# yzhang511/multi_modal_foundation_model

Hardware: AMD Instinct MI355X
Metric: pretrain samples/sec (T=100 bins/modality, d_model=256, 5+5 layers, spike+behaviour masked pretraining step) (higher is better)
Workload: dtype bf16; 1 GPU; BASELINE.json configs[1]: 1 session, ap(668 neurons)+behaviour(2), d_model=256, heads=8, mlp=512, 5 enc + 5 dec layers, T=100 (L=200 tokens), dropout 0.4/0.2, AdamW+OneCycleLR, mixed objectives; per_gpu_batch=1024, global_batch=1024, seq_len=200, parallelism=dp1

## Files before the change

include/mmfm.h:

```cpp
#ifndef MMFM_H
#define MMFM_H
#include <stdint.h>
#ifdef __cplusplus
extern "C" {
#endif

#define MMFM_VERSION 401
#define MMFM_F32 0
#define MMFM_BF16 1
#define MMFM_NULL_BIAS 1
#define MMFM_EMBED_OPTS 1
#define MMFM_MLP_GELU 0
#define MMFM_MLP_RELU 1
#define MMFM_MLP_SIGMOID 2
#define MMFM_MLP_GELU_TANH 3

typedef void* mmfm_stream;

typedef struct {
    const void* state;
    uint32_t site;
    float p;
} mmfm_dropout;

int mmfm_version(void);
const char* mmfm_last_error(void);
int mmfm_device_check(int device);
int mmfm_rng_seed(void* state, uint64_t seed, mmfm_stream stream);
int mmfm_rng_advance(void* state, mmfm_stream stream);

typedef struct {
    int dtype;
    int c_f32;
    const void* A;
    const void* B;
    void* C;
    int M, N, K;
    int lda, ldb, ldc;
    int a_kcontig, b_kcontig;
    int splits, kchunk;
    int64_t slab_stride;
    const float* bias;
    void* pre_out;
    int act;
    float act_scale;
    const void* gradmul_pre;
    mmfm_dropout drop;
    const void* residual;
    int ldr;
    float* colsum;
} mmfm_gemm_desc;
int mmfm_gemm(const mmfm_gemm_desc* d, mmfm_stream stream);
int mmfm_gemm_pair(const mmfm_gemm_desc* a, const mmfm_gemm_desc* b, mmfm_stream stream);

int mmfm_gemm_dw_tiles(int M, int N, int K);
int mmfm_reduce_slabs(float* dst, const float* src, int64_t n, int nslabs, int64_t slab_stride,
                      int accumulate, mmfm_stream stream);
typedef struct {
    float* dst;
    const float* src;
    int64_t n, slab_stride;
    int32_t nslabs, accumulate, chunk0, pad_;
} mmfm_reduce_entry;
int mmfm_reduce_slabs_multi(const mmfm_reduce_entry* table, int count, int total_chunks, mmfm_stream stream);
int64_t mmfm_colsum_workspace(int64_t R, int N);
int mmfm_colsum(int dtype, const void* x, int64_t R, int N, int ld, float* out, int accumulate,
                void* workspace, int64_t workspace_bytes, mmfm_stream stream);

int mmfm_layernorm_fwd(int dtype, const void* x, const float* gamma, const float* beta, void* y,
                       float* mean, float* rstd, int64_t R, int H, float eps,
                       int destitch_L, int destitch_T, mmfm_stream stream);
int64_t mmfm_layernorm_bwd_workspace(int64_t R, int H);
int mmfm_layernorm_bwd(int dtype, const void* dy, const void* x, const float* mean, const float* rstd,
                       const float* gamma, const void* dres, void* dx, float* dgamma, float* dbeta,
                       int accumulate, int64_t R, int H, int destitch_L, int destitch_T,
                       void* workspace, int64_t workspace_bytes, mmfm_stream stream);

int mmfm_scalenorm_fwd(int dtype, const void* x, const float* g, void* y, float* rinv, int64_t R, int H, float eps,
                       mmfm_stream stream);
int64_t mmfm_scalenorm_bwd_workspace(int64_t R, int H);
int mmfm_scalenorm_bwd(int dtype, const void* dy, const void* x, const float* rinv, const float* g, const void* dres, void* dx,
                       float* dg, int accumulate, int64_t R, int H, void* workspace, int64_t workspace_bytes,
                       mmfm_stream stream);

#define MMFM_ATTN_DIAG 1
#define MMFM_ATTN_CAUSAL 2
#define MMFM_ATTN_SEP 4
typedef struct {
    int dtype;
    int B, heads, Lq, Lk, dh;
    const void* q; const void* k; const void* v;
    int ldq, ldk, ldv;
    void* o; int ldo;
    float* lse;
    const uint8_t* keypad;
    const uint8_t* mod_id;
    int flags;
    float scale;
    mmfm_dropout drop_p, drop_o;
    const void* d_o; int lddo;
    void* dq; void* dk; void* dv;
    int lddq, lddk, lddv;
    void* keepbits;
} mmfm_attn_desc;
int mmfm_attn_fwd(const mmfm_attn_desc* d, mmfm_stream stream);
int mmfm_attn_bwd(const mmfm_attn_desc* d, mmfm_stream stream);
int64_t mmfm_attn_keepbits_bytes(int B, int heads, int Lq, int Lk);
float mmfm_attn_keep_prob(float p);

int mmfm_mask_prep(int B, int T, int M, const int64_t* const* mask_src, const int64_t* mask_stride,
                   const int64_t* attn, const int64_t* channels, uint8_t* tokmask, uint8_t* keypad,
                   uint8_t* keep0, uint8_t* mod_id, int64_t* count, mmfm_stream stream);

int mmfm_stitch_fwd(int dtype, const void* tok, const float* mod_emb_row, const float* pos_emb,
                    const int64_t* ts, const uint8_t* keep0, void* x, void* emb,
                    int B, int T, int L, int m, int H, int max_F, mmfm_stream stream);
int64_t mmfm_stitch_bwd_workspace(int dtype, int B, int T, int L, int H, int max_F);
int mmfm_stitch_bwd(int dtype, const void* dx, const void* dextra, const int64_t* ts, const uint8_t* keep0,
                    mmfm_dropout drop, void* d_tok, float* d_mod_row, float* d_pos, int acc_mod, int acc_pos,
                    int B, int T, int L, int m, int H, int max_F,
                    void* workspace, int64_t workspace_bytes, mmfm_stream stream);

int mmfm_collate_csr(int B, int max_T, int max_N, float pad_value, const uint8_t* data, const int32_t* indices,
                     const int64_t* indptr, const int64_t* indptr_off, const int64_t* nnz_off, const int32_t* T_b,
                     const int32_t* N_b, float* out, int64_t* time_mask, int64_t* space_mask, mmfm_stream stream);

#define MMFM_LOSS_KINDS 1
#define MMFM_LOSS_POISSON_LOG 0
#define MMFM_LOSS_MSE 1
#define MMFM_LOSS_POISSON_RATE 2
#define MMFM_LOSS_L1 3
#define MMFM_LOSS_SMOOTH_L1 4
#define MMFM_LOSS_HUBER 5
#define MMFM_LOSS_BCE_LOGITS 6
#define MMFM_LOSS_FULL 1
int64_t mmfm_masked_loss_workspace(int64_t R, int N);
int mmfm_masked_loss_fwd(int dtype, int kind, const void* pred, const float* target, const uint8_t* rowmask,
                         int mask_ld, int T, int64_t R, int N, float* loss_sum,
                         void* workspace, int64_t workspace_bytes, mmfm_stream stream);
int mmfm_masked_loss_kind_fwd(int dtype, int kind, float param, int flags, const void* pred, const float* target,
                              const uint8_t* rowmask, int mask_ld, int T, int64_t R, int N, float* loss_sum,
                              void* workspace, int64_t workspace_bytes, mmfm_stream stream);
int mmfm_loss_finalize(const float* loss_sum, const int64_t* count, int M, float* loss, float* inv_n,
                       mmfm_stream stream);
int mmfm_masked_loss_bwd(int dtype, int kind, const void* pred, const float* target, const uint8_t* rowmask,
                         int mask_ld, int T, int64_t R, int N, const float* grad_out, const float* inv_n,
                         void* dpred, mmfm_stream stream);
int mmfm_masked_loss_kind_bwd(int dtype, int kind, float param, int flags, const void* pred, const float* target,
                              const uint8_t* rowmask, int mask_ld, int T, int64_t R, int N, const float* grad_out,
                              const float* inv_n, void* dpred, mmfm_stream stream);

int mmfm_dropout_apply(int dtype, const void* src, void* dst, int64_t R, int N, mmfm_dropout drop,
                       mmfm_stream stream);
int mmfm_cast_f32_to_bf16(const float* src, void* dst, int64_t n, mmfm_stream stream);

int mmfm_adamw_step(float* p, const float* g, float* m, float* v, void* p_bf16, int64_t n,
                    const float* hyper, mmfm_stream stream);

int mmfm_r2_series(const float* gt, const int64_t* gt_strides, const float* pred, const int64_t* pred_strides,
                   int G, int S, int C, float* out, mmfm_stream stream);
int64_t mmfm_bits_per_spike_workspace(int64_t R, int N);
int mmfm_bits_per_spike(const float* rates, const float* spikes, int64_t R, int N, float* out,
                        void* workspace, int64_t workspace_bytes, mmfm_stream stream);
int64_t mmfm_bits_per_spike_neurons_workspace(int64_t R, int N);
int mmfm_bits_per_spike_neurons(const float* rates, const float* spikes, int64_t R, int N, float* out,
                                void* workspace, int64_t workspace_bytes, mmfm_stream stream);


typedef struct {
    const float* W;
    const float* gamma;
    const float* beta;
    const float* bias;
    void* Wp;
// ... 64 lines not shown
```

multi_modal_foundation_model_amd/_lib.py:

```python
from __future__ import annotations

import ctypes as C
import os
import re

import torch

_HERE = os.path.dirname(os.path.abspath(__file__))
LIB_PATH = os.environ.get("MMFM_LIB") or os.path.join(_HERE, "libmmfm_hip.so")
HEADER_PATH = os.path.join(os.path.dirname(_HERE), "include", "mmfm.h")

F32, BF16 = 0, 1
ATTN_DIAG, ATTN_CAUSAL, ATTN_SEP = 1, 2, 4
ACT_NONE, ACT_GELU, ACT_SOFTSIGN, ACT_GELU_GRAD, ACT_SOFTSIGN_GRAD, ACT_SOFTSIGN_GRAD_OUT = 0, 1, 2, 3, 4, 5
ACT_RELU, ACT_RELU_GRAD, ACT_SIGMOID, ACT_SIGMOID_GRAD, ACT_GELU_TANH, ACT_GELU_TANH_GRAD = 6, 7, 8, 9, 10, 11
(ACT_EMB_IDENTITY, ACT_EMB_IDENTITY_GRAD, ACT_EMB_RELU, ACT_EMB_RELU_GRAD, ACT_EMB_GELU, ACT_EMB_GELU_GRAD, ACT_EMB_SILU, ACT_EMB_SILU_GRAD,
 ACT_EMB_QUICK_GELU, ACT_EMB_QUICK_GELU_GRAD, ACT_EMB_GELU_TANH, ACT_EMB_GELU_TANH_GRAD, ACT_EMB_TANH, ACT_EMB_TANH_GRAD) = range(12, 26)
MLP_GELU, MLP_RELU, MLP_SIGMOID, MLP_GELU_TANH = 0, 1, 2, 3
LOSS_POISSON_LOG, LOSS_MSE, LOSS_POISSON_RATE, LOSS_L1, LOSS_SMOOTH_L1, LOSS_HUBER, LOSS_BCE_LOGITS = range(7)
LOSS_FULL = 1


class MmfmError(RuntimeError):
    pass


class Dropout(C.Structure):
    _fields_ = [("state", C.c_void_p), ("site", C.c_uint32), ("p", C.c_float)]


NO_DROP = Dropout(None, 0, 0.0)


class GemmDesc(C.Structure):
    _fields_ = [("dtype", C.c_int), ("c_f32", C.c_int), ("A", C.c_void_p), ("B", C.c_void_p), ("C", C.c_void_p),
                ("M", C.c_int), ("N", C.c_int), ("K", C.c_int), ("lda", C.c_int), ("ldb", C.c_int), ("ldc", C.c_int),
                ("a_kcontig", C.c_int), ("b_kcontig", C.c_int), ("splits", C.c_int), ("kchunk", C.c_int),
                ("slab_stride", C.c_int64), ("bias", C.c_void_p), ("pre_out", C.c_void_p), ("act", C.c_int),
                ("act_scale", C.c_float), ("gradmul_pre", C.c_void_p), ("drop", Dropout), ("residual", C.c_void_p),
                ("ldr", C.c_int), ("colsum", C.c_void_p)]


class AttnDesc(C.Structure):
    _fields_ = [("dtype", C.c_int), ("B", C.c_int), ("heads", C.c_int), ("Lq", C.c_int), ("Lk", C.c_int), ("dh", C.c_int),
                ("q", C.c_void_p), ("k", C.c_void_p), ("v", C.c_void_p), ("ldq", C.c_int), ("ldk", C.c_int),
                ("ldv", C.c_int), ("o", C.c_void_p), ("ldo", C.c_int), ("lse", C.c_void_p), ("keypad", C.c_void_p),
                ("mod_id", C.c_void_p), ("flags", C.c_int), ("scale", C.c_float), ("drop_p", Dropout),
                ("drop_o", Dropout), ("d_o", C.c_void_p), ("lddo", C.c_int), ("dq", C.c_void_p), ("dk", C.c_void_p),
                ("dv", C.c_void_p), ("lddq", C.c_int), ("lddk", C.c_int), ("lddv", C.c_int), ("keepbits", C.c_void_p)]


class PrepEntry(C.Structure):
    _fields_ = [("W", C.c_void_p), ("gamma", C.c_void_p), ("beta", C.c_void_p), ("bias", C.c_void_p), ("Wp", C.c_void_p),
                ("WpT", C.c_void_p), ("bp", C.c_void_p), ("N", C.c_int), ("K", C.c_int), ("tile0", C.c_int), ("scalar_gain", C.c_int),
                ("WpP", C.c_void_p), ("WpTP", C.c_void_p)]


class ReduceEntry(C.Structure):
    _fields_ = [("dst", C.c_void_p), ("src", C.c_void_p), ("n", C.c_int64), ("slab_stride", C.c_int64), ("nslabs", C.c_int32),
                ("accumulate", C.c_int32), ("chunk0", C.c_int32), ("pad_", C.c_int32)]


class RowGemmDesc(C.Structure):
    _fields_ = [("R", C.c_int64), ("K", C.c_int), ("N", C.c_int), ("x", C.c_void_p), ("ldx", C.c_int), ("w", C.c_void_p),
                ("ldw", C.c_int), ("bias", C.c_void_p), ("ln", C.c_int), ("eps", C.c_float), ("xhat", C.c_void_p),
                ("rstd", C.c_void_p), ("residual", C.c_void_p), ("ldr", C.c_int), ("y", C.c_void_p), ("ldy", C.c_int),
                ("stream_out", C.c_int), ("rotate", C.c_int), ("ln_bwd", C.c_int), ("bwd_xhat", C.c_void_p), ("bwd_rstd", C.c_void_p)]


class MlpDesc(C.Structure):
    _fields_ = [("R", C.c_int64), ("x", C.c_void_p), ("ldx", C.c_int), ("eps", C.c_float), ("w_up", C.c_void_p),
                ("b_up", C.c_void_p), ("w_down", C.c_void_p), ("b_down", C.c_void_p), ("drop", Dropout), ("y", C.c_void_p),
                ("ldy", C.c_int), ("xhat", C.c_void_p), ("rstd", C.c_void_p), ("dy", C.c_void_p), ("lddy", C.c_int),
                ("w_down_t", C.c_void_p), ("w_up_t", C.c_void_p), ("t1", C.c_void_p), ("g", C.c_void_p), ("du", C.c_void_p),
                ("dx", C.c_void_p), ("lddx", C.c_int), ("rotate", C.c_int), ("scalenorm", C.c_int),
                ("act", C.c_int), ("act_beta", C.c_float)]


_vp, _i, _i64, _f = C.c_void_p, C.c_int, C.c_int64, C.c_float
_PROTOS = {
    "mmfm_version": (C.c_int, []),
    "mmfm_last_error": (C.c_char_p, []),
    "mmfm_device_check": (C.c_int, [_i]),
    "mmfm_rng_seed": (C.c_int, [_vp, C.c_uint64, _vp]),
    "mmfm_rng_advance": (C.c_int, [_vp, _vp]),
    "mmfm_gemm": (C.c_int, [C.POINTER(GemmDesc), _vp]),
    "mmfm_gemm_pair": (C.c_int, [_vp, _vp, _vp]),
    "mmfm_gemm_dw_tiles": (C.c_int, [_i, _i, _i]),
    "mmfm_reduce_slabs": (C.c_int, [_vp, _vp, _i64, _i, _i64, _i, _vp]),
    "mmfm_reduce_slabs_multi": (C.c_int, [_vp, _i, _i, _vp]),
    "mmfm_colsum_workspace": (C.c_int64, [_i64, _i]),
    "mmfm_colsum": (C.c_int, [_i, _vp, _i64, _i, _i, _vp, _i, _vp, _i64, _vp]),
    "mmfm_layernorm_fwd": (C.c_int, [_i, _vp, _vp, _vp, _vp, _vp, _vp, _i64, _i, _f, _i, _i, _vp]),
    "mmfm_layernorm_bwd_workspace": (C.c_int64, [_i64, _i]),
    "mmfm_layernorm_bwd": (C.c_int, [_i, _vp, _vp, _vp, _vp, _vp, _vp, _vp, _vp, _vp, _i, _i64, _i, _i, _i, _vp, _i64, _vp]),
    "mmfm_scalenorm_fwd": (C.c_int, [_i, _vp, _vp, _vp, _vp, _i64, _i, _f, _vp]),
    "mmfm_scalenorm_bwd_workspace": (C.c_int64, [_i64, _i]),
    "mmfm_scalenorm_bwd": (C.c_int, [_i, _vp, _vp, _vp, _vp, _vp, _vp, _vp, _i, _i64, _i, _vp, _i64, _vp]),
    "mmfm_attn_fwd": (C.c_int, [C.POINTER(AttnDesc), _vp]),
    "mmfm_attn_bwd": (C.c_int, [C.POINTER(AttnDesc), _vp]),
    "mmfm_attn_keepbits_bytes": (C.c_int64, [_i, _i, _i, _i]),
    "mmfm_attn_keep_prob": (C.c_float, [_f]),
    "mmfm_mask_prep": (C.c_int, [_i, _i, _i, C.POINTER(_vp), C.POINTER(_i64), _vp, C.POINTER(_i64), _vp, _vp, _vp, _vp, _vp, _vp]),
    "mmfm_collate_csr": (C.c_int, [_i, _i, _i, _f, _vp, _vp, _vp, _vp, _vp, _vp, _vp, _vp, _vp, _vp, _vp]),
    "mmfm_stitch_fwd": (C.c_int, [_i, _vp, _vp, _vp, _vp, _vp, _vp, _vp, _i, _i, _i, _i, _i, _i, _vp]),
    "mmfm_stitch_bwd_workspace": (C.c_int64, [_i, _i, _i, _i, _i, _i]),
    "mmfm_stitch_bwd": (C.c_int, [_i, _vp, _vp, _vp, _vp, Dropout, _vp, _vp, _vp, _i, _i, _i, _i, _i, _i, _i, _i, _vp, _i64, _vp]),
    "mmfm_masked_loss_workspace": (C.c_int64, [_i64, _i]),
    "mmfm_masked_loss_fwd": (C.c_int, [_i, _i, _vp, _vp, _vp, _i, _i, _i64, _i, _vp, _vp, _i64, _vp]),
    "mmfm_masked_loss_kind_fwd": (C.c_int, [_i, _i, _f, _i, _vp, _vp, _vp, _i, _i, _i64, _i, _vp, _vp, _i64, _vp]),
    "mmfm_loss_finalize": (C.c_int, [_vp, _vp, _i, _vp, _vp, _vp]),
    "mmfm_masked_loss_bwd": (C.c_int, [_i, _i, _vp, _vp, _vp, _i, _i, _i64, _i, _vp, _vp, _vp, _vp]),
    "mmfm_masked_loss_kind_bwd": (C.c_int, [_i, _i, _f, _i, _vp, _vp, _vp, _i, _i, _i64, _i, _vp, _vp, _vp, _vp]),
    "mmfm_dropout_apply": (C.c_int, [_i, _vp, _vp, _i64, _i, Dropout, _vp]),
    "mmfm_cast_f32_to_bf16": (C.c_int, [_vp, _vp, _i64, _vp]),
    "mmfm_adamw_step": (C.c_int, [_vp, _vp, _vp, _vp, _vp, _i64, _vp, _vp]),
    "mmfm_prep_weights": (C.c_int, [_vp, _i, _i, _vp]),
    "mmfm_rowgemm": (C.c_int, [C.POINTER(RowGemmDesc), _vp]),
    "mmfm_mlp_fwd": (C.c_int, [C.POINTER(MlpDesc), _vp]),
    "mmfm_mlp_bwd": (C.c_int, [C.POINTER(MlpDesc), _vp]),
    "mmfm_ln_linear_grad_workspace": (C.c_int64, [_i]),
    "mmfm_ln_linear_grad": (C.c_int, [_vp, _vp, _vp, _vp, _i, _i, _vp, _vp, _vp, _vp, _i, _vp, _i64, _vp]),
    "mmfm_sn_linear_grad": (C.c_int, [_vp, _vp, _vp, _i, _i, _vp, _vp, _vp, _i, _vp, _i64, _vp]),
    "mmfm_r2_series": (C.c_int, [_vp, C.POINTER(_i64), _vp, C.POINTER(_i64), _i, _i, _i, _vp, _vp]),
    "mmfm_bits_per_spike_workspace": (C.c_int64, [_i64, _i]),
    "mmfm_bits_per_spike": (C.c_int, [_vp, _vp, _i64, _i, _vp, _vp, _i64, _vp]),
    "mmfm_bits_per_spike_neurons_workspace": (C.c_int64, [_i64, _i]),
    "mmfm_bits_per_spike_neurons": (C.c_int, [_vp, _vp, _i64, _i, _vp, _vp, _i64, _vp]),
    "mmfm_mt19937_jump": (C.c_int, [_vp, C.POINTER(C.c_int32), C.c_uint64]),
    "mmfm_mt19937_jump_reset": (C.c_int, []),
}

_lib = None


def header_symbols():
    with open(HEADER_PATH) as f:
        src = f.read()
    src = re.sub(r"/\*.*?\*/", "", src, flags=re.S)
    return sorted(set(re.findall(r"\b(mmfm_[a-z0-9_]+)\s*\(", src)))


def lib():
    global _lib
    if _lib is None:
        if not os.path.exists(LIB_PATH):
            raise ImportError(f"{LIB_PATH} is missing: the HIP extension is not built and there is no CPU "
                              "fallback.  Run `python -c 'import __graft_entry__ as g; g.build()'`.")
        l = C.CDLL(LIB_PATH)
        for name, (res, args) in _PROTOS.items():
            fn = getattr(l, name)
            fn.restype, fn.argtypes = res, args
        _lib = l
    return _lib


def check(rc, what=""):
    if rc != 0:
# ... 2 lines not shown
```

multi_modal_foundation_model_amd/csrc/common.h:

```cpp
#pragma once
#include <hip/hip_runtime.h>
#include <stdint.h>
#include <stdio.h>
#include <stdarg.h>
#include <math.h>

#include "../../include/mmfm.h"

typedef __attribute__((ext_vector_type(16))) float f32x16;
typedef __attribute__((ext_vector_type(4))) float f32x4;
typedef __attribute__((ext_vector_type(8))) short bf16x8;
typedef __bf16 bf16_t;

int mmfm_set_error(int code, const char* fmt, ...);

#define MMFM_REQUIRE(cond, ...)                      \
    do {                                             \
        if (!(cond)) return mmfm_set_error(-1, __VA_ARGS__); \
    } while (0)

#define MMFM_LAUNCH_CHECK(name)                                                         \
    do {                                                                                \
        hipError_t e__ = hipGetLastError();                                             \
        if (e__ != hipSuccess)                                                          \
            return mmfm_set_error((int)e__, "%s: launch failed: %s", name, hipGetErrorString(e__)); \
    } while (0)

int mmfm_lds_opt_in(const void* kern, size_t bytes, const char* what);

static inline int cdiv(long a, long b) { return (int)((a + b - 1) / b); }

__device__ __forceinline__ float bf2f(uint16_t v) { return __uint_as_float(((uint32_t)v) << 16); }
__device__ __forceinline__ uint16_t f2bf(float f) {
    bf16_t b = (bf16_t)f;
    return *reinterpret_cast<uint16_t*>(&b);
}

typedef __attribute__((ext_vector_type(4))) unsigned int mmfm_u32x4;
typedef __attribute__((ext_vector_type(2))) unsigned int mmfm_u32x2;
typedef __attribute__((ext_vector_type(4))) float mmfm_f32x4;
__device__ __forceinline__ void st_stream(uint4* p, uint4 v) {
    __builtin_nontemporal_store(__builtin_bit_cast(mmfm_u32x4, v), reinterpret_cast<mmfm_u32x4*>(p));
}
__device__ __forceinline__ void st_stream(uint2* p, uint2 v) {
    __builtin_nontemporal_store(__builtin_bit_cast(mmfm_u32x2, v), reinterpret_cast<mmfm_u32x2*>(p));
}
__device__ __forceinline__ void st_stream(float4* p, float4 v) {
    __builtin_nontemporal_store(__builtin_bit_cast(mmfm_f32x4, v), reinterpret_cast<mmfm_f32x4*>(p));
}

template <typename T> struct io;
template <> struct io<float> {
    static __device__ __forceinline__ float ld(const float* p) { return *p; }
    static __device__ __forceinline__ void st(float* p, float v) { *p = v; }
    static __device__ __forceinline__ float4 ld4(const float* p) { return *reinterpret_cast<const float4*>(p); }
    static __device__ __forceinline__ void st4(float* p, float4 v) { *reinterpret_cast<float4*>(p) = v; }
    static __device__ __forceinline__ void st4s(float* p, float4 v) { st_stream(reinterpret_cast<float4*>(p), v); }
};
template <> struct io<uint16_t> {
    static __device__ __forceinline__ float ld(const uint16_t* p) { return bf2f(*p); }
    static __device__ __forceinline__ void st(uint16_t* p, float v) { *p = f2bf(v); }
    static __device__ __forceinline__ float4 ld4(const uint16_t* p) {
        uint2 u = *reinterpret_cast<const uint2*>(p);
        return make_float4(__uint_as_float(u.x << 16), __uint_as_float(u.x & 0xffff0000u),
                           __uint_as_float(u.y << 16), __uint_as_float(u.y & 0xffff0000u));
    }
    static __device__ __forceinline__ void st4(uint16_t* p, float4 v) {
        uint2 u;
        u.x = (uint32_t)f2bf(v.x) | ((uint32_t)f2bf(v.y) << 16);
        u.y = (uint32_t)f2bf(v.z) | ((uint32_t)f2bf(v.w) << 16);
        *reinterpret_cast<uint2*>(p) = u;
    }
    static __device__ __forceinline__ void st4s(uint16_t* p, float4 v) {
        uint2 u;
        u.x = (uint32_t)f2bf(v.x) | ((uint32_t)f2bf(v.y) << 16);
        u.y = (uint32_t)f2bf(v.z) | ((uint32_t)f2bf(v.w) << 16);
        st_stream(reinterpret_cast<uint2*>(p), u);
    }
};

__device__ __forceinline__ uint32_t mix32(uint32_t x) {
    x ^= x >> 16; x *= 0x7feb352dU; x ^= x >> 15; x *= 0x846ca68bU; x ^= x >> 16;
    return x;
// ... 289 lines not shown
```

multi_modal_foundation_model_amd/csrc/gemm.hip:

```cpp
#include "common.h"

namespace {

constexpr int BM = 128, BN = 128, BK = 32;
constexpr int LDT = 132;
constexpr int NTHREADS = 256;

template <bool KC>
__device__ __forceinline__ void g2r(float4 (&r)[4], const float* __restrict__ base, int ld, int row0, int k0,
                                    int rows, int kend, bool vec, int t) {
    if (KC) {
        const int kq = t & 7, r0 = t >> 3;
        const int k = k0 + 4 * kq;
#pragma unroll
        for (int p = 0; p < 4; ++p) {
            const int row = row0 + r0 + 32 * p;
            float4 v = make_float4(0.f, 0.f, 0.f, 0.f);
            if (row < rows && k < kend) {
                const float* src = base + (size_t)row * ld + k;
                if (vec && k + 3 < kend) {
                    v = *reinterpret_cast<const float4*>(src);
                } else {
                    v.x = src[0];
                    if (k + 1 < kend) v.y = src[1];
// ... 218 lines not shown
    }
}

template <typename T>
__global__ __launch_bounds__(256) void colsum_kernel(const T* __restrict__ x, int64_t R, int N, int ld, float* __restrict__ part,
                                                     int64_t rows_per) {
    __shared__ float red[4][64];
    const int c = blockIdx.x * 64 + (threadIdx.x & 63), rl = threadIdx.x >> 6;
    const int64_t r0 = (int64_t)blockIdx.y * rows_per, r1 = min(R, r0 + rows_per);
    float s = 0.f;
    if (c < N)
        for (int64_t r = r0 + rl; r < r1; r += 4) s += io<T>::ld(x + (size_t)r * ld + c);
    red[rl][threadIdx.x & 63] = s;
    __syncthreads();
    if (rl == 0 && c < N)
        part[(size_t)blockIdx.y * N + c] = red[0][threadIdx.x] + red[1][threadIdx.x] + red[2][threadIdx.x] + red[3][threadIdx.x];
}

template <typename T>
__global__ __launch_bounds__(256) void colsum4_kernel(const T* __restrict__ x, int64_t R, int N, int ld, float* __restrict__ part,
                                                      int64_t rows_per) {
    __shared__ float4 red[4][64];
    const int lane = threadIdx.x & 63, wave = threadIdx.x >> 6;
    const int c = blockIdx.x * 256 + lane * 4;
    const int64_t r0 = (int64_t)blockIdx.y * rows_per, r1 = min(R, r0 + rows_per);
    float4 s = make_float4(0.f, 0.f, 0.f, 0.f);
    if (c < N) {
        int64_t r = r0 + wave;
        for (; r + 12 < r1; r += 16) {
            const float4 a = io<T>::ld4(x + (size_t)r * ld + c), b = io<T>::ld4(x + (size_t)(r + 4) * ld + c);
            const float4 e = io<T>::ld4(x + (size_t)(r + 8) * ld + c), f = io<T>::ld4(x + (size_t)(r + 12) * ld + c);
            s.x += (a.x + b.x) + (e.x + f.x); s.y += (a.y + b.y) + (e.y + f.y);
            s.z += (a.z + b.z) + (e.z + f.z); s.w += (a.w + b.w) + (e.w + f.w);
        }
        for (; r < r1; r += 4) {
            const float4 a = io<T>::ld4(x + (size_t)r * ld + c);
            s.x += a.x; s.y += a.y; s.z += a.z; s.w += a.w;
        }
    }
    red[wave][lane] = s;
    __syncthreads();
    if (wave == 0 && c < N) {
        float4 o;
        o.x = red[0][lane].x + red[1][lane].x + red[2][lane].x + red[3][lane].x;
        o.y = red[0][lane].y + red[1][lane].y + red[2][lane].y + red[3][lane].y;
        o.z = red[0][lane].z + red[1][lane].z + red[2][lane].z + red[3][lane].z;
        o.w = red[0][lane].w + red[1][lane].w + red[2][lane].w + red[3][lane].w;
        *reinterpret_cast<float4*>(part + (size_t)blockIdx.y * N + c) = o;
    }
}

}

int mmfm_gemm_bf16_launch(const mmfm_gemm_desc* d, hipStream_t st);

static int gemm_check(const mmfm_gemm_desc* dp, mmfm_gemm_desc& d) {
    MMFM_REQUIRE(dp != nullptr, "mmfm_gemm: null descriptor");
    d = *dp;
    MMFM_REQUIRE(d.dtype == MMFM_F32 || d.dtype == MMFM_BF16, "mmfm_gemm: bad dtype %d", d.dtype);
    MMFM_REQUIRE(d.M > 0 && d.N > 0 && d.K > 0, "mmfm_gemm: bad shape M=%d N=%d K=%d", d.M, d.N, d.K);
    MMFM_REQUIRE(d.A && d.B && d.C, "mmfm_gemm: null operand");
    MMFM_REQUIRE(d.lda >= (d.a_kcontig ? d.K : d.M), "mmfm_gemm: lda %d too small", d.lda);
    MMFM_REQUIRE(d.ldb >= (d.b_kcontig ? d.K : d.N), "mmfm_gemm: ldb %d too small", d.ldb);
    MMFM_REQUIRE(d.ldc >= d.N, "mmfm_gemm: ldc %d < N %d", d.ldc, d.N);
    MMFM_REQUIRE(!(d.a_kcontig == 0 && d.b_kcontig == 1), "mmfm_gemm: layout (A row-contig, B k-contig) is not built");
    MMFM_REQUIRE(d.act >= 0 && d.act <= kActEmbedLast, "mmfm_gemm: bad act %d", d.act);
    const bool grad_act = (d.act >= 3 && d.act <= 5) || (d.act >= 7 && (d.act & 1));
    MMFM_REQUIRE(!d.gradmul_pre || grad_act,
                 "mmfm_gemm: gradmul_pre needs a gradient act (3 gelu', 4 softsign', 5 softsign' from the output, 7 relu', 9 sigmoid-gate', 11 tanh-gelu', "
                 "the embedder's 13 identity', 15 relu', 17 gelu', 19 silu', 21 quick_gelu', 23 tanh-gelu', 25 tanh')");
    MMFM_REQUIRE(d.gradmul_pre || !grad_act || d.act == kActEmbedIdentityGrad, "mmfm_gemm: act %d needs gradmul_pre", d.act);
    if (d.splits <= 1) {
        d.splits = 1;
        d.kchunk = d.K;
    } else {
        MMFM_REQUIRE(d.kchunk > 0 && d.kchunk % 64 == 0, "mmfm_gemm: kchunk %d must be a positive multiple of 64", d.kchunk);
        MMFM_REQUIRE((int64_t)d.splits * d.kchunk >= d.K, "mmfm_gemm: splits*kchunk < K");
        MMFM_REQUIRE(d.slab_stride >= (int64_t)d.M * d.ldc, "mmfm_gemm: slab_stride too small");
        MMFM_REQUIRE(!d.bias && !d.pre_out && !d.act && !d.residual && d.drop.p <= 0.f,
                     "mmfm_gemm: split-K writes raw partials, no epilogue");
    }
    MMFM_REQUIRE(!d.residual || d.ldr >= d.N, "mmfm_gemm: ldr too small");
    MMFM_REQUIRE(!d.colsum || (d.dtype == MMFM_BF16 && d.a_kcontig == 0), "mmfm_gemm: colsum needs dtype bf16 and a_kcontig == 0");
    return 0;
}

int mmfm_gemm_dw_pair_launch(const mmfm_gemm_desc* a, const mmfm_gemm_desc* b, hipStream_t st);

extern "C" int mmfm_gemm(const mmfm_gemm_desc* dp, mmfm_stream stream) {
    mmfm_gemm_desc d;
    if (int rc = gemm_check(dp, d)) return rc;
    hipStream_t st = (hipStream_t)stream;
    if (d.dtype == MMFM_BF16) return mmfm_gemm_bf16_launch(&d, st);

    const int tiles = cdiv(d.M, BM) * cdiv(d.N, BN);
    const int vecA = (d.lda % 4 == 0) && ((uintptr_t)d.A % 16 == 0);
    const int vecB = (d.ldb % 4 == 0) && ((uintptr_t)d.B % 16 == 0);
    dim3 grid(tiles, d.splits), block(NTHREADS);
#define F32_LAUNCH(AKV)                                                                                            \
    if (d.a_kcontig && d.b_kcontig) hipLaunchKernelGGL((gemm_f32_kernel<true, true, AKV>), grid, block, 0, st, d, vecA, vecB);        \
    else if (d.a_kcontig && !d.b_kcontig) hipLaunchKernelGGL((gemm_f32_kernel<true, false, AKV>), grid, block, 0, st, d, vecA, vecB); \
    else hipLaunchKernelGGL((gemm_f32_kernel<false, false, AKV>), grid, block, 0, st, d, vecA, vecB);
    switch (gemm_act_kind(d.act)) {
    case MMFM_MLP_RELU: { F32_LAUNCH(MMFM_MLP_RELU) } break;
    case MMFM_MLP_SIGMOID: { F32_LAUNCH(MMFM_MLP_SIGMOID) } break;
    case MMFM_MLP_GELU_TANH: { F32_LAUNCH(MMFM_MLP_GELU_TANH) } break;
    case kActEmbed: { F32_LAUNCH(kActEmbed) } break;
    default: { F32_LAUNCH(0) }
    }
#undef F32_LAUNCH
    MMFM_LAUNCH_CHECK("mmfm_gemm(f32)");
    return 0;
}

extern "C" int mmfm_gemm_pair(const mmfm_gemm_desc* ap, const mmfm_gemm_desc* bp, mmfm_stream stream) {
    mmfm_gemm_desc a, b;
    if (int rc = gemm_check(ap, a)) return rc;
    if (int rc = gemm_check(bp, b)) return rc;
    hipStream_t st = (hipStream_t)stream;
    if (a.dtype == MMFM_BF16 && b.dtype == MMFM_BF16) {
        const int rc = mmfm_gemm_dw_pair_launch(&a, &b, st);
        if (rc != -1000) return rc;
    }
    if (int rc = mmfm_gemm(ap, stream)) return rc;
    return mmfm_gemm(bp, stream);
}

__global__ __launch_bounds__(256) void reduce_slabs_multi_kernel(const mmfm_reduce_entry* __restrict__ tab, int count) {
    int lo = 0, hi = count - 1;
    const int b = blockIdx.x;
    while (lo < hi) {
        const int mid = (lo + hi + 1) >> 1;
        if (tab[mid].chunk0 <= b) lo = mid; else hi = mid - 1;
    }
    const mmfm_reduce_entry e = tab[lo];
    const int64_t i = (int64_t)(b - e.chunk0) * 256 + threadIdx.x;
    if (i >= e.n) return;
    float s = e.accumulate ? e.dst[i] : 0.f;
    for (int k = 0; k < e.nslabs; ++k) s += e.src[(size_t)k * e.slab_stride + i];
    e.dst[i] = s;
}

extern "C" int mmfm_reduce_slabs_multi(const mmfm_reduce_entry* table, int count, int total_chunks, mmfm_stream stream) {
    MMFM_REQUIRE(table && count > 0 && total_chunks > 0, "mmfm_reduce_slabs_multi: bad arguments");
    hipLaunchKernelGGL(reduce_slabs_multi_kernel, dim3(total_chunks), dim3(256), 0, (hipStream_t)stream, table, count);
    MMFM_LAUNCH_CHECK("mmfm_reduce_slabs_multi");
    return 0;
}

extern "C" int mmfm_reduce_slabs(float* dst, const float* src_c, int64_t n, int nslabs, int64_t slab_stride,
                                 int accumulate, mmfm_stream stream) {
    MMFM_REQUIRE(dst && src_c && n > 0 && nslabs > 0 && slab_stride >= n, "mmfm_reduce_slabs: bad arguments");
    float* src = const_cast<float*>(src_c);
    hipStream_t st = (hipStream_t)stream;
    const bool vec = (n % 4 == 0) && (slab_stride % 4 == 0) && ((uintptr_t)dst % 16 == 0) && ((uintptr_t)src % 16 == 0);
    if (!vec) {
        const int blocks = (int)std::min<int64_t>(2048, (n + 255) / 256);
        hipLaunchKernelGGL(reduce_slabs_kernel, dim3(blocks), dim3(256), 0, st, dst, src, n, nslabs, slab_stride, accumulate);
        MMFM_LAUNCH_CHECK("mmfm_reduce_slabs");
        return 0;
    }
    const int chunks = (int)((n + 255) / 256);
    int group = nslabs;
    if (nslabs >= 16 && chunks < 512) {
        const int want = std::min(nslabs / 4, std::max(1, 512 / chunks));
// ... 46 lines not shown
```

multi_modal_foundation_model_amd/csrc/gemm_bf16.hip:

```cpp
#include "common.h"
#include <stdlib.h>
#include <algorithm>

namespace {

constexpr int BM = 128, BN = 128;
constexpr int NTHREADS = 256;
template <int BK> struct Geo {
    static constexpr int KC_LD = BK + 8;
    static constexpr int TILE_BYTES = 128 * KC_LD * 2;
    static constexpr int NP = BK / 16;
};

typedef __attribute__((ext_vector_type(8))) __bf16 bf16x8v;
typedef __attribute__((ext_vector_type(4))) short s16x4;
typedef __attribute__((address_space(3))) s16x4 lds_s16x4;

__device__ __forceinline__ uint4 load8(const uint16_t* __restrict__ src, int nvalid, int align) {
    uint4 v = make_uint4(0u, 0u, 0u, 0u);
    if (nvalid >= 8 && align == 8) return *reinterpret_cast<const uint4*>(src);
    if (nvalid >= 8 && align == 4) {
        const uint2 a = *reinterpret_cast<const uint2*>(src), b = *reinterpret_cast<const uint2*>(src + 4);
        return make_uint4(a.x, a.y, b.x, b.y);
    }
// ... 16 lines not shown
        for (int p = 0; p < NP; ++p) {
            const int row = row0 + r0 + RPP * p;
            r[p] = (row < rows) ? load8(base + (size_t)row * ld + k, kend - k, align) : make_uint4(0u, 0u, 0u, 0u);
        }
    } else {
        const int cq = t & 15, kk0 = t >> 4, col = row0 + 8 * cq;
#pragma unroll
        for (int p = 0; p < NP; ++p) {
            const int k = k0 + kk0 + 16 * p;
            r[p] = (k < kend) ? load8(base + (size_t)k * ld + col, rows - col, align) : make_uint4(0u, 0u, 0u, 0u);
        }
    }
}

template <bool RC, int BK>
__device__ __forceinline__ void r2s(char* __restrict__ S, const uint4 (&r)[BK / 16], int t) {
    constexpr int NP = BK / 16, LPR = BK / 8, RPP = 256 / LPR, KC_LD = Geo<BK>::KC_LD;
    if (!RC) {
        const int kq = t % LPR, r0 = t / LPR;
#pragma unroll
        for (int p = 0; p < NP; ++p) *reinterpret_cast<uint4*>(S + (r0 + RPP * p) * (KC_LD * 2) + kq * 16) = r[p];
    } else {
        const int cq = t & 15, kk0 = t >> 4;
#pragma unroll
        for (int p = 0; p < NP; ++p) {
            const int kk = kk0 + 16 * p;
            *reinterpret_cast<uint4*>(S + kk * 256 + ((cq * 16) ^ ((kk & 3) << 6))) = r[p];
        }
    }
}

template <bool RC, int BK>
__device__ __forceinline__ bf16x8v frag(const char* __restrict__ S, int rowbase, int ks, int lane) {
    if (!RC) {
        const int r = lane & 31, h = lane >> 5;
        const uint4 v = *reinterpret_cast<const uint4*>(S + (rowbase + r) * (Geo<BK>::KC_LD * 2) + ks * 32 + h * 16);
        return __builtin_bit_cast(bf16x8v, v);
    } else {
        const int g = lane >> 4, li = lane & 15, q = li >> 2, p = li & 3;
        const int col = rowbase + 16 * (g & 1) + 4 * p;
        const int kb = ks * 16 + 8 * (g >> 1);
        const int off0 = (kb + q) * 256 + ((col * 2) ^ (q << 6));
        const int off1 = (kb + 4 + q) * 256 + ((col * 2) ^ (q << 6));
        const s16x4 lo = __builtin_amdgcn_ds_read_tr16_b64_v4i16((lds_s16x4*)(S + off0));
        const s16x4 hi = __builtin_amdgcn_ds_read_tr16_b64_v4i16((lds_s16x4*)(S + off1));
        typedef __attribute__((ext_vector_type(8))) short s16x8;
        s16x8 v;
        v[0] = lo[0]; v[1] = lo[1]; v[2] = lo[2]; v[3] = lo[3]; v[4] = hi[0]; v[5] = hi[1]; v[6] = hi[2]; v[7] = hi[3];
        return __builtin_bit_cast(bf16x8v, v);
    }
}

template <typename TO, int AK = 0, int EF = 0>
__device__ __forceinline__ void epilogue_store(const mmfm_gemm_desc& d, const Drop& dr, float v, int m, int n) {
    typedef io<uint16_t> I16;
    constexpr int AKM = AK == kActEmbed ? 0 : AK;
    if (d.bias) v += d.bias[n];
    if (d.pre_out) I16::st(reinterpret_cast<uint16_t*>(d.pre_out) + (size_t)m * d.ldc + n, v);
    if constexpr (AK == kActEmbed) {
        if (!(d.act & 1)) v = embed_act1<true, EF>(v) * d.act_scale;
        else if (EF == 0) v *= d.act_scale;
        else v = embed_mul_grad1<true, EF>(v, I16::ld(reinterpret_cast<const uint16_t*>(d.gradmul_pre) + (size_t)m * d.ldc + n)) * d.act_scale;
        v = dr.apply(v, (uint64_t)m * (uint64_t)d.N + (uint64_t)n);
        if (d.residual) v += I16::ld(reinterpret_cast<const uint16_t*>(d.residual) + (size_t)m * d.ldr + n);
        io<TO>::st(reinterpret_cast<TO*>(d.C) + (size_t)m * d.ldc + n, v);
        return;
    }
    if (d.act == 1) v = gelu_poly(v);
    else if (d.act == 2) v = softsign_f(v) * d.act_scale;
    else if (AK && !(d.act & 1)) v = mlp_act1<AKM>(v, d.act_scale);
    if (d.gradmul_pre) {
        const float u = I16::ld(reinterpret_cast<const uint16_t*>(d.gradmul_pre) + (size_t)m * d.ldc + n);
        if (AK == MMFM_MLP_RELU) v = u > 0.f ? v : 0.f;
        else if (AK) v *= mlp_act_grad1<AKM>(u, d.act_scale);
        else v *= (d.act == 3) ? gelu_poly_grad(u) : (d.act == 4 ? softsign_grad(u) : softsign_grad_from_out(u, 1.f / d.act_scale)) * d.act_scale;
    }
    v = dr.apply(v, (uint64_t)m * (uint64_t)d.N + (uint64_t)n);
    if (d.residual) v += I16::ld(reinterpret_cast<const uint16_t*>(d.residual) + (size_t)m * d.ldr + n);
    io<TO>::st(reinterpret_cast<TO*>(d.C) + (size_t)m * d.ldc + n, v);
}

typedef __attribute__((ext_vector_type(8))) __bf16 bf16x8e;
__device__ __forceinline__ bf16x8e pack8f(const float* v) {
    bf16x8e o;
#pragma unroll
    for (int e = 0; e < 8; ++e) o[e] = (__bf16)v[e];
    return o;
}
__device__ __forceinline__ void unpack8(uint4 w, float* u) {
    u[0] = __uint_as_float(w.x << 16); u[1] = __uint_as_float(w.x & 0xffff0000u);
    u[2] = __uint_as_float(w.y << 16); u[3] = __uint_as_float(w.y & 0xffff0000u);
    u[4] = __uint_as_float(w.z << 16); u[5] = __uint_as_float(w.z & 0xffff0000u);
    u[6] = __uint_as_float(w.w << 16); u[7] = __uint_as_float(w.w & 0xffff0000u);
}

__device__ __forceinline__ int xcd_remap(int bid, int nwg) {
    const int q = nwg >> 3, r = nwg & 7, x = bid & 7;
    return (x < r ? x * (q + 1) : r * (q + 1) + (x - r) * q) + (bid >> 3);
}

__device__ __forceinline__ uint4 ldg8(const uint16_t* p, bool a16, bool hi, bool nt) {
    if (a16 && nt) return __builtin_bit_cast(uint4, __builtin_nontemporal_load(reinterpret_cast<const mmfm_u32x4*>(p)));
    if (a16) return *reinterpret_cast<const uint4*>(p);
    const uint2 a = *reinterpret_cast<const uint2*>(p);
    const uint2 b = hi ? *reinterpret_cast<const uint2*>(p + 4) : make_uint2(0u, 0u);
    return make_uint4(a.x, a.y, b.x, b.y);
}
__device__ __forceinline__ void stg8(uint16_t* p, uint4 v, bool a16, bool hi, bool nt) {
    if (nt) {
        if (a16) { st_stream(reinterpret_cast<uint4*>(p), v); return; }
        st_stream(reinterpret_cast<uint2*>(p), make_uint2(v.x, v.y));
        if (hi) st_stream(reinterpret_cast<uint2*>(p + 4), make_uint2(v.z, v.w));
        return;
    }
    if (a16) { *reinterpret_cast<uint4*>(p) = v; return; }
    *reinterpret_cast<uint2*>(p) = make_uint2(v.x, v.y);
    if (hi) *reinterpret_cast<uint2*>(p + 4) = make_uint2(v.z, v.w);
}

template <typename TO, bool EPI_LOADS = true, int AK = 0, int EF = 0>
__device__ __forceinline__ void epilogue_tile(const mmfm_gemm_desc& d, f32x16 (&acc)[2][2], char* smem, int m0, int n0, int z, int vec_epi,
                                              int t, int wm, int wn, int kh, int l31) {
    const bool split = d.splits > 1;
    constexpr int AKM = AK == kActEmbed ? 0 : AK;
    float* Cf = reinterpret_cast<float*>(d.C) + (split ? (size_t)z * d.slab_stride : 0);
    const Drop dr = drop_init(d.drop);
    if (vec_epi & 1) {
        float* stage = reinterpret_cast<float*>(smem);
        constexpr int SLDW = 132;
        constexpr bool BF_OUT = sizeof(TO) == 2;
        const bool bf_path = BF_OUT && !split;
        const bool a16 = !(vec_epi & 2);
        const int col = (t & 15) * 8, n = n0 + col;
        const bool n_ok = n < d.N, hi = n + 8 <= d.N;
        float bs[8];
#pragma unroll
        for (int e = 0; e < 8; ++e) bs[e] = 0.f;
        if (d.bias && n_ok && !split) {
            const float4 b0 = *reinterpret_cast<const float4*>(d.bias + n);
            const float4 b1 = hi ? *reinterpret_cast<const float4*>(d.bias + n + 4) : make_float4(0.f, 0.f, 0.f, 0.f);
            bs[0] = b0.x; bs[1] = b0.y; bs[2] = b0.z; bs[3] = b0.w; bs[4] = b1.x; bs[5] = b1.y; bs[6] = b1.z; bs[7] = b1.w;
        }
#pragma unroll 1
        for (int half = 0; half < 2; ++half) {
            uint4 gu[4], gr[4];
            if (EPI_LOADS && bf_path) {
#pragma unroll
                for (int c = 0; c < 4; ++c) {
                    const int m = m0 + half * 64 + ((t + 256 * c) >> 4);
                    gu[c] = gr[c] = make_uint4(0u, 0u, 0u, 0u);
                    if (m < d.M && n_ok) {
                        if (d.gradmul_pre) gu[c] = ldg8(reinterpret_cast<const uint16_t*>(d.gradmul_pre) + (size_t)m * d.ldc + n, a16, hi, (vec_epi & 32768) != 0);
                        if (d.residual) gr[c] = ldg8(reinterpret_cast<const uint16_t*>(d.residual) + (size_t)m * d.ldr + n, a16, hi, (vec_epi & 32768) != 0);
                    }
                }
            }
            __syncthreads();
            if (wm == half) {
#pragma unroll
                for (int i = 0; i < 2; ++i)
#pragma unroll
                    for (int j = 0; j < 2; ++j)
#pragma unroll
                        for (int r = 0; r < 16; ++r)
                            stage[(i * 32 + (r & 3) + 8 * (r >> 2) + 4 * kh) * SLDW + wn * 64 + j * 32 + l31] = acc[i][j][r];
            }
            __syncthreads();
#pragma unroll
            for (int c = 0; c < 4; ++c) {
                const int row = (t + 256 * c) >> 4;
                const int m = m0 + half * 64 + row;
                if (m >= d.M || !n_ok) continue;
                float v[8];
                const float4 s0 = *reinterpret_cast<const float4*>(stage + row * SLDW + col);
                const float4 s1 = *reinterpret_cast<const float4*>(stage + row * SLDW + col + 4);
                v[0] = s0.x; v[1] = s0.y; v[2] = s0.z; v[3] = s0.w; v[4] = s1.x; v[5] = s1.y; v[6] = s1.z; v[7] = s1.w;
                const size_t off = (size_t)m * d.ldc + n;
#pragma unroll
                for (int e = 0; e < 8; ++e) v[e] += bs[e];
                if (split || !BF_OUT) {
                    float* dst = (split ? Cf : reinterpret_cast<float*>(d.C)) + off;
                    if (vec_epi & 16384) {
                        st_stream(reinterpret_cast<float4*>(dst), make_float4(v[0], v[1], v[2], v[3]));
                        if (hi) st_stream(reinterpret_cast<float4*>(dst + 4), make_float4(v[4], v[5], v[6], v[7]));
                    } else {
                        *reinterpret_cast<float4*>(dst) = make_float4(v[0], v[1], v[2], v[3]);
                        if (hi) *reinterpret_cast<float4*>(dst + 4) = make_float4(v[4], v[5], v[6], v[7]);
                    }
                    continue;
                }
                if (d.pre_out) stg8(reinterpret_cast<uint16_t*>(d.pre_out) + off, __builtin_bit_cast(uint4, pack8f(v)), a16, hi, (vec_epi & 8192) != 0);
                if constexpr (AK == kActEmbed) {
                    if (!(d.act & 1)) embed_act_n<8, EF>(v, d.act_scale);
                    else {
                        float u[8];
                        unpack8(gu[c], u);
                        embed_mul_grad_n<8, EF>(v, u, d.act_scale);
                    }
                } else if (d.act == 1) gelu_n<8>(v);
                else if (d.act == 2) {
#pragma unroll
                    for (int e = 0; e < 8; ++e) v[e] = softsign_f(v[e]) * d.act_scale;
                } else if (AK && !(d.act & 1)) mlp_act_n<AK, 8>(v, d.act_scale);
                if (AK != kActEmbed && EPI_LOADS && d.gradmul_pre) {
                    float u[8];
                    unpack8(gu[c], u);
                    if (d.act == 3) mul_gelu_grad_n<8>(v, u);
                    else if (d.act == 4) {
#pragma unroll
                        for (int e = 0; e < 8; ++e) v[e] *= softsign_grad(u[e]) * d.act_scale;
                    } else if (AK) mul_mlp_act_grad_n<AKM, 8>(v, u, d.act_scale);
                    else {
                        const float inv_s = 1.f / d.act_scale;
#pragma unroll
                        for (int e = 0; e < 8; ++e) v[e] *= softsign_grad_from_out(u[e], inv_s) * d.act_scale;
                    }
                }
                if (dr.on()) {
                    const uint64_t base = (uint64_t)m * (uint64_t)d.N + (uint64_t)n;
#pragma unroll
                    for (int e = 0; e < 8; e += 2) dr.apply2(v[e], v[e + 1], base + e);
                }
                if (EPI_LOADS && d.residual) {
                    float u[8];
                    unpack8(gr[c], u);
#pragma unroll
                    for (int e = 0; e < 8; ++e) v[e] += u[e];
                }
                stg8(reinterpret_cast<uint16_t*>(d.C) + off, __builtin_bit_cast(uint4, pack8f(v)), a16, hi, (vec_epi & 4096) != 0);
            }
        }
        return;
    }
    if (split) {
#pragma unroll
        for (int i = 0; i < 2; ++i)
#pragma unroll
            for (int j = 0; j < 2; ++j)
#pragma unroll
                for (int r = 0; r < 16; ++r) {
                    const int m = m0 + wm * 64 + i * 32 + (r & 3) + 8 * (r >> 2) + 4 * kh;
                    const int n = n0 + wn * 64 + j * 32 + l31;
                    if (m < d.M && n < d.N) Cf[(size_t)m * d.ldc + n] = acc[i][j][r];
                }
        return;
    }
#pragma unroll
    for (int i = 0; i < 2; ++i)
#pragma unroll
        for (int j = 0; j < 2; ++j)
#pragma unroll
            for (int r = 0; r < 16; ++r) {
                const int m = m0 + wm * 64 + i * 32 + (r & 3) + 8 * (r >> 2) + 4 * kh;
                const int n = n0 + wn * 64 + j * 32 + l31;
                if (m < d.M && n < d.N) epilogue_store<TO, AK, EF>(d, dr, acc[i][j][r], m, n);
            }
}

template <bool ARC, bool BRC, typename TO, int BK, bool PERSIST = (sizeof(TO) == 4), int AK = 0>
__global__ __launch_bounds__(NTHREADS, BK == 64 ? 3 : 2) void gemm_bf16_kernel(const mmfm_gemm_desc d, const int alignA, const int alignB,
                                                                              const int vec_epi, const int total_items) {
    constexpr int TILE_BYTES = Geo<BK>::TILE_BYTES;
    __shared__ __attribute__((aligned(16))) char smem[2 * TILE_BYTES];
    char* As = smem;
    char* Bs = smem + TILE_BYTES;
    const int t = threadIdx.x, lane = t & 63, wave = t >> 6;
    const int wm = wave >> 1, wn = wave & 1, kh = lane >> 5, l31 = lane & 31;
    const int tiles_n = (d.N + BN - 1) / BN;
    const int tiles = ((d.M + BM - 1) / BM) * tiles_n;
    const uint16_t* A = reinterpret_cast<const uint16_t*>(d.A);
    const uint16_t* B = reinterpret_cast<const uint16_t*>(d.B);

    auto decode = [&](int w, int& m0, int& n0, int& z, int& kbeg, int& kend) {
        const int item = xcd_remap(w, total_items);
        z = item / tiles;
        const int tile = item - z * tiles;
        m0 = (tile / tiles_n) * BM;
        n0 = (tile % tiles_n) * BN;
        kbeg = z * d.kchunk;
        kend = min(d.K, kbeg + d.kchunk);
    };

    int m0, n0, z, kbeg, kend;
    int w = blockIdx.x;
    if (w >= total_items) return;
    decode(w, m0, n0, z, kbeg, kend);
    uint4 ra[BK / 16], rb[BK / 16];
    g2r<ARC, BK>(ra, A, d.lda, m0, kbeg, d.M, kend, alignA, t);
    g2r<BRC, BK>(rb, B, d.ldb, n0, kbeg, d.N, kend, alignB, t);
    for (;;) {
        f32x16 acc[2][2];
#pragma unroll
        for (int i = 0; i < 2; ++i)
#pragma unroll
            for (int j = 0; j < 2; ++j)
#pragma unroll
                for (int r = 0; r < 16; ++r) acc[i][j][r] = 0.f;
        const bool do_cs = ARC && d.colsum != nullptr && n0 == 0;
        float cs[8];
#pragma unroll
        for (int j = 0; j < 8; ++j) cs[j] = 0.f;
        const int wn_ = w + gridDim.x;
        const bool more = PERSIST && wn_ < total_items;
        int m0n = 0, n0n = 0, zn = 0, kbegn = 0, kendn = 0;
        if (more) decode(wn_, m0n, n0n, zn, kbegn, kendn);
        for (int k0 = kbeg; k0 < kend; k0 += BK) {
            __syncthreads();
            r2s<ARC, BK>(As, ra, t);
            r2s<BRC, BK>(Bs, rb, t);
            __syncthreads();
            {
                if (k0 + BK < kend) {
                    g2r<ARC, BK>(ra, A, d.lda, m0, k0 + BK, d.M, kend, alignA, t);
                    g2r<BRC, BK>(rb, B, d.ldb, n0, k0 + BK, d.N, kend, alignB, t);
                } else if (more) {
                    g2r<ARC, BK>(ra, A, d.lda, m0n, kbegn, d.M, kendn, alignA, t);
                    g2r<BRC, BK>(rb, B, d.ldb, n0n, kbegn, d.N, kendn, alignB, t);
                }
            }
            if (ARC && do_cs) {
                const int cq = t & 15, kk0 = t >> 4;
#pragma unroll
                for (int p = 0; p < BK / 16; ++p) {
                    const int kk = kk0 + 16 * p;
                    float u[8];
                    unpack8(*reinterpret_cast<const uint4*>(As + kk * 256 + ((cq * 16) ^ ((kk & 3) << 6))), u);
#pragma unroll
                    for (int j = 0; j < 8; ++j) cs[j] += u[j];
                }
            }
#pragma unroll
            for (int ks = 0; ks < BK / 16; ++ks) {
                const bf16x8v a0 = frag<ARC, BK>(As, wm * 64, ks, lane), a1 = frag<ARC, BK>(As, wm * 64 + 32, ks, lane);
                const bf16x8v b0 = frag<BRC, BK>(Bs, wn * 64, ks, lane), b1 = frag<BRC, BK>(Bs, wn * 64 + 32, ks, lane);
                acc[0][0] = __builtin_amdgcn_mfma_f32_32x32x16_bf16(a0, b0, acc[0][0], 0, 0, 0);
                acc[0][1] = __builtin_amdgcn_mfma_f32_32x32x16_bf16(a0, b1, acc[0][1], 0, 0, 0);
                acc[1][0] = __builtin_amdgcn_mfma_f32_32x32x16_bf16(a1, b0, acc[1][0], 0, 0, 0);
                acc[1][1] = __builtin_amdgcn_mfma_f32_32x32x16_bf16(a1, b1, acc[1][1], 0, 0, 0);
            }
        }
        if (ARC && do_cs) {
            __syncthreads();
            float* red = reinterpret_cast<float*>(smem);
            float* mine = red + (t >> 4) * 128 + (t & 15) * 8;
            *reinterpret_cast<float4*>(mine) = make_float4(cs[0], cs[1], cs[2], cs[3]);
            *reinterpret_cast<float4*>(mine + 4) = make_float4(cs[4], cs[5], cs[6], cs[7]);
            __syncthreads();
            if (t < 128 && m0 + t < d.M) {
                float sum = 0.f;
#pragma unroll
                for (int i = 0; i < 16; ++i) sum += red[i * 128 + t];
                d.colsum[(d.splits > 1 ? (size_t)z * d.slab_stride : 0) + m0 + t] = sum;
            }
        }
        if constexpr (AK == kActEmbed)
            embed_dispatch(d.act, [&](auto F) {
                epilogue_tile<TO, !(PERSIST && sizeof(TO) == 2), AK, decltype(F)::value>(d, acc, smem, m0, n0, z, vec_epi, t, wm, wn, kh, l31);
            });
        else
            epilogue_tile<TO, !(PERSIST && sizeof(TO) == 2), AK>(d, acc, smem, m0, n0, z, vec_epi, t, wm, wn, kh, l31);
        if (!more) break;
        w = wn_; m0 = m0n; n0 = n0n; z = zn; kbeg = kbegn; kend = kendn;
    }
}

int align_of(const void* p, int ld) {
    if (ld % 8 == 0 && (uintptr_t)p % 16 == 0) return 8;
    if (ld % 4 == 0 && (uintptr_t)p % 8 == 0) return 4;
    return 1;
}

}

int mmfm_gemm_big_launch(const mmfm_gemm_desc* dp, hipStream_t st);
int mmfm_gemm_dw_launch(const mmfm_gemm_desc* dp, hipStream_t st);

int mmfm_gemm_bf16_launch(const mmfm_gemm_desc* dp, hipStream_t st) {
    const mmfm_gemm_desc d = *dp;
    {
        const int rb = mmfm_gemm_big_launch(dp, st);
        if (rb != -1000) return rb;
        const int rw = mmfm_gemm_dw_launch(dp, st);
        if (rw != -1000) return rw;
    }
    MMFM_REQUIRE(d.splits == 1 || d.kchunk % 64 == 0, "mmfm_gemm(bf16): kchunk %d must be a multiple of 64", d.kchunk);
    static const int bk_env = [] { const char* e = getenv("MMFM_GEMM_BK"); return e ? atoi(e) : 0; }();
    const int kspan = d.splits > 1 ? d.kchunk : d.K;
    (void)kspan;
    const int BKsel = bk_env == 128 ? 128 : 64;
    const int tiles = cdiv(d.M, BM) * cdiv(d.N, BN);
    const int aA = align_of(d.A, d.lda), aB = align_of(d.B, d.ldb);
    const int total_items = tiles * d.splits;
    static const int wg_per_cu = [] { const char* e = getenv("MMFM_GEMM_WG_PER_CU"); const int v = e ? atoi(e) : 3; return v > 0 ? v : 3; }();
    const bool f32out = d.c_f32 || d.splits > 1;
    auto al16 = [](const void* p) { return p == nullptr || (uintptr_t)p % 16 == 0; };
    const int vec8 = (d.N % 8 == 0) && (d.ldc % 8 == 0) && al16(d.C) && al16(d.pre_out) && al16(d.gradmul_pre) && al16(d.bias) &&
                     (!d.residual || (d.ldr % 8 == 0 && al16(d.residual))) && (!d.splits || d.splits == 1 || d.slab_stride % 4 == 0);
    auto al8 = [](const void* p) { return p == nullptr || (uintptr_t)p % 8 == 0; };
    const bool f32c = d.c_f32 || d.splits > 1;
    const int vec4 = (d.N % 4 == 0) && (d.ldc % 4 == 0) && (f32c ? al16(d.C) : al8(d.C)) && al8(d.pre_out) && al8(d.gradmul_pre) && al16(d.bias) &&
                     (!d.residual || (d.ldr % 4 == 0 && al8(d.residual))) && (!d.splits || d.splits == 1 || d.slab_stride % 4 == 0);
    const int vec = vec8 ? 1 : (vec4 ? 3 : 0);
    static const int nt_env = [] { const char* e = getenv("MMFM_GEMM_NT"); return e ? atoi(e) : 3; }();
    const int vecf = vec | ((nt_env & 1) ? 4096 : 0) | ((nt_env & 2) ? 8192 : 0) | ((nt_env & 4) ? 16384 : 0) | ((nt_env & 8) ? 32768 : 0);
    static const int persist_bf16 = [] { const char* e = getenv("MMFM_GEMM_PERSIST_BF16"); return e ? atoi(e) : 1; }();
    const int ak = gemm_act_kind(d.act);
    const bool pb = !f32out && !ak && persist_bf16 && !d.gradmul_pre && !d.residual && !d.pre_out && (vec & 1) && d.K <= 768;
    dim3 grid((f32out || pb) ? std::min(total_items, 256 * wg_per_cu) : total_items), block(NTHREADS);
    static const int pad_lds = [] { const char* e = getenv("MMFM_GEMM_PAD_LDS"); return e ? atoi(e) : 0; }();
#define LAUNCH2(ARC, BRC, BKV)                                                                                    \
    if (f32out) hipLaunchKernelGGL((gemm_bf16_kernel<ARC, BRC, float, BKV>), grid, block, pad_lds, st, d, aA, aB, vecf, total_items);  \
    else if (pb) hipLaunchKernelGGL((gemm_bf16_kernel<ARC, BRC, uint16_t, BKV, true>), grid, block, pad_lds, st, d, aA, aB, vecf, total_items); \
    else hipLaunchKernelGGL((gemm_bf16_kernel<ARC, BRC, uint16_t, BKV>), grid, block, pad_lds, st, d, aA, aB, vecf, total_items);
#define LAUNCH_AK(ARC, BRC, AKV)                                                                                  \
    if (f32out) hipLaunchKernelGGL((gemm_bf16_kernel<ARC, BRC, float, 64, true, AKV>), grid, block, pad_lds, st, d, aA, aB, vecf, total_items); \
    else hipLaunchKernelGGL((gemm_bf16_kernel<ARC, BRC, uint16_t, 64, false, AKV>), grid, block, pad_lds, st, d, aA, aB, vecf, total_items);
#define LAUNCH(ARC, BRC)                                                                                          \
    if (ak == MMFM_MLP_RELU) { LAUNCH_AK(ARC, BRC, MMFM_MLP_RELU) }                                                \
    else if (ak == MMFM_MLP_SIGMOID) { LAUNCH_AK(ARC, BRC, MMFM_MLP_SIGMOID) }                                     \
    else if (ak == MMFM_MLP_GELU_TANH) { LAUNCH_AK(ARC, BRC, MMFM_MLP_GELU_TANH) }                                 \
    else if (ak == kActEmbed) { LAUNCH_AK(ARC, BRC, kActEmbed) }                                                   \
    else if (BKsel == 128) { LAUNCH2(ARC, BRC, 128) } else { LAUNCH2(ARC, BRC, 64) }
    if (d.a_kcontig && d.b_kcontig) { LAUNCH(false, false) }
    else if (d.a_kcontig && !d.b_kcontig) { LAUNCH(false, true) }
    else { LAUNCH(true, true) }
#undef LAUNCH
#undef LAUNCH_AK
#undef LAUNCH2
    MMFM_LAUNCH_CHECK("mmfm_gemm(bf16)");
    return 0;
}
```

multi_modal_foundation_model_amd/csrc/gemm_big.hip:

```cpp
#include "rowchain.h"
#include <stdlib.h>
#include <algorithm>

using namespace rowchain;

namespace {

typedef __attribute__((address_space(3))) void lds_void_t;
typedef __attribute__((address_space(1))) const void glb_void_t;

constexpr int TB = 256, BK = 64, NT = 512;
constexpr int TILE_B = TB * BK * 2;
constexpr int STG0 = 4 * TILE_B;
constexpr int LDS_ALL = STG0 + 8 * STG_BYTES;

__device__ __forceinline__ opnd tfrag(const char* tile, int row, int c) {
    return as_opnd(*reinterpret_cast<const uint4*>(tile + row * 128 + ((c ^ ((row >> 1) & 7)) << 4)));
}

__device__ __forceinline__ int xcd_order(int bid, int nwg) {
    const int q = nwg >> 3, r = nwg & 7, x = bid & 7;
    return (x < r ? x * (q + 1) : r * (q + 1) + (x - r) * q) + (bid >> 3);
}

struct BigArgs {
    mmfm_gemm_desc d;
    int tiles_n, ntiles, nk;
    int nt_c, nt_pre;
};

__device__ __forceinline__ void issue_ktile(char* buf, const uint16_t* const (&pa)[4], const uint16_t* const (&pb)[4], int koff, int wave) {
#pragma unroll
    for (int i = 0; i < 4; ++i)
        __builtin_amdgcn_global_load_lds((glb_void_t*)(pa[i] + koff), (lds_void_t*)(buf + (i * 512 + 64 * wave) * 16), 16, 0, 0);
#pragma unroll
    for (int i = 0; i < 4; ++i)
        __builtin_amdgcn_global_load_lds((glb_void_t*)(pb[i] + koff), (lds_void_t*)(buf + TILE_B + (i * 512 + 64 * wave) * 16), 16, 0, 0);
}

#define LDS_READ(dst, addr, off) asm volatile("ds_read_b128 %0, %1 offset:%2" : "=v"(dst) : "v"(addr), "n"(off))
#define LDS_WAIT(n) do { asm volatile("s_waitcnt lgkmcnt(" #n ")" ::: "memory"); __builtin_amdgcn_sched_barrier(0); } while (0)

template <int AK = 0>
__global__ __launch_bounds__(NT, 2) void gemm_big_kernel(const BigArgs a) {
    extern __shared__ __attribute__((aligned(16))) char smem[];
    const mmfm_gemm_desc& d = a.d;
    const int t = threadIdx.x, lane = t & 63, m = lane & 31, h = lane >> 5;
    const int wave = __builtin_amdgcn_readfirstlane(t >> 6);
    const int wnh = wave & 1, wmq = wave >> 1;
    char* stg = smem + STG0 + wave * STG_BYTES;
    const uint16_t* A = reinterpret_cast<const uint16_t*>(d.A);
    const uint16_t* B = reinterpret_cast<const uint16_t*>(d.B);
    const int nk = a.nk;
    const int my_tiles = blockIdx.x < a.ntiles ? (a.ntiles - 1 - (int)blockIdx.x) / (int)gridDim.x + 1 : 0;
    if (my_tiles == 0) return;
    const int G = my_tiles * nk;

    const int ldrow = t >> 3, ldc8 = 8 * ((t & 7) ^ ((t >> 4) & 7));
    const uint16_t* pa[4];
    const uint16_t* pb[4];
    auto set_rows = [&](int it) {
        const int tile = xcd_order((int)blockIdx.x + it * (int)gridDim.x, a.ntiles);
        const int m0 = (tile / a.tiles_n) * TB, n0 = (tile % a.tiles_n) * TB;
#pragma unroll
        for (int i = 0; i < 4; ++i) {
            pa[i] = A + (size_t)min(m0 + 64 * i + ldrow, d.M - 1) * d.lda + ldc8;
            pb[i] = B + (size_t)min(n0 + 64 * i + ldrow, d.N - 1) * d.ldb + ldc8;
        }
    };
    int ld_g = 0, ld_it = 0, ld_kt = 0;
    auto issue_next = [&]() {
        if (ld_g >= G) return false;
        if (ld_kt == 0) set_rows(ld_it);
        issue_ktile(smem + (ld_g & 1) * 2 * TILE_B, pa, pb, ld_kt * BK, wave);
        ++ld_g;
        if (++ld_kt == nk) { ld_kt = 0; ++ld_it; }
        return true;
    };
    issue_next();
    bool tail1 = issue_next();

    const Drop dr = drop_init(d.drop);
    const GBuf Cb = gbuf(d.C, (int64_t)d.M * d.ldc * 2), Pb = gbuf(d.pre_out, (int64_t)d.M * d.ldc * 2);
    const GBuf Gb = gbuf(d.gradmul_pre, (int64_t)d.M * d.ldc * 2), Rb = gbuf(d.residual, (int64_t)d.M * d.ldr * 2);

    const uint32_t lds0 = (uint32_t)(uintptr_t)(__attribute__((address_space(3))) char*)smem;
    const uint32_t sw = (uint32_t)((m >> 1) & 7);
    const uint32_t xrow = lds0 + (uint32_t)(64 * wmq + m) * 128u, wrow = lds0 + (uint32_t)(128 * wnh + m) * 128u;
    uint32_t coff[4];
#pragma unroll
    for (int ks = 0; ks < 4; ++ks) coff[ks] = (((uint32_t)(2 * ks + h)) ^ sw) << 4;

    f32x16 acc[4][2];
    int g = 0;
    for (int it = 0; it < my_tiles; ++it) {
        const int tile = xcd_order((int)blockIdx.x + it * (int)gridDim.x, a.ntiles);
        const int m0 = (tile / a.tiles_n) * TB, n0 = (tile % a.tiles_n) * TB;
#pragma unroll
// ... 83 lines not shown
                else if (d.act == 2) {
#pragma unroll
                    for (int e = 0; e < 2; ++e)
#pragma unroll
                        for (int r = 0; r < 16; ++r) {
                            const float v = acc[2 * ip + e][j][r];
                            acc[2 * ip + e][j][r] = v * __builtin_amdgcn_rcpf(1.f + fabsf(v)) * d.act_scale;
                        }
                } else if (AK && !(d.act & 1)) {
#pragma unroll
                    for (int e = 0; e < 2; ++e) {
                        float v[16];
#pragma unroll
                        for (int r = 0; r < 16; ++r) v[r] = acc[2 * ip + e][j][r];
                        mlp_act_n<AK, 16>(v, d.act_scale);
#pragma unroll
                        for (int r = 0; r < 16; ++r) acc[2 * ip + e][j][r] = v[r];
                    }
                } else if (d.gradmul_pre) {
                    const Lines L = fetch_lines(Gb, wrow0, ldcb, (uint32_t)ncol0 * 2u, lane);
                    stage_lines(stg, L, lane);
#pragma unroll
                    for (int e = 0; e < 2; ++e) {
                        const f32x16 u = unstage_tile(stg, e, m, h);
                        f32x16& v = acc[2 * ip + e][j];
                        if (AK) {
                            float uu[16], vv[16];
#pragma unroll
                            for (int r = 0; r < 16; ++r) { uu[r] = u[r]; vv[r] = v[r]; }
                            mul_mlp_act_grad_n<AK, 16>(vv, uu, d.act_scale);
#pragma unroll
                            for (int r = 0; r < 16; ++r) v[r] = vv[r];
                        } else if (d.act == 3) {
#pragma unroll
                            for (int r = 0; r < 16; r += 2) {
                                mmfm_f32x2 uu; uu.x = u[r]; uu.y = u[r + 1];
                                uu = gelu_grad2(uu);
                                v[r] *= uu.x; v[r + 1] *= uu.y;
                            }
                        } else if (d.act == 4) {
#pragma unroll
                            for (int r = 0; r < 16; ++r) {
                                const float rd = __builtin_amdgcn_rcpf(1.f + fabsf(u[r]));
                                v[r] *= rd * rd * d.act_scale;
                            }
                        } else {
                            const float inv_s = 1.f / d.act_scale;
#pragma unroll
                            for (int r = 0; r < 16; ++r) v[r] *= softsign_grad_from_out(u[r], inv_s) * d.act_scale;
                        }
                    }
                }
                if (dr.on()) {
#pragma unroll
                    for (int e = 0; e < 2; ++e)
#pragma unroll
                        for (int r = 0; r < 16; r += 2) {
                            float v0 = acc[2 * ip + e][j][r], v1 = acc[2 * ip + e][j][r + 1];
                            dr.apply2(v0, v1, (uint64_t)row * (uint64_t)d.N + (uint64_t)(ncol0 + 32 * e + 8 * (r >> 2) + 4 * h + (r & 3)));
                            acc[2 * ip + e][j][r] = v0; acc[2 * ip + e][j][r + 1] = v1;
                        }
                }
                if (d.residual) {
                    const Lines L = fetch_lines(Rb, wrow0, ldrb, (uint32_t)ncol0 * 2u, lane);
                    stage_lines(stg, L, lane);
#pragma unroll
                    for (int e = 0; e < 2; ++e) {
                        const f32x16 u = unstage_tile(stg, e, m, h);
#pragma unroll
                        for (int r = 0; r < 16; ++r) acc[2 * ip + e][j][r] += u[r];
                    }
                }
                stage_tile(stg, 0, m, h, acc[2 * ip][j]);
                stage_tile(stg, 1, m, h, acc[2 * ip + 1][j]);
                if (a.nt_c) flush_lines<true>(stg, Cb, wrow0, ldcb, (uint32_t)ncol0 * 2u, lane, nchunk);
                else flush_lines<false>(stg, Cb, wrow0, ldcb, (uint32_t)ncol0 * 2u, lane, nchunk);
            }
        }
        tail1 = false;
    }
}

}

int mmfm_gemm_big_launch(const mmfm_gemm_desc* dp, hipStream_t st) {
    const mmfm_gemm_desc& d = *dp;
    static const int on = [] { const char* e = getenv("MMFM_GEMM_BIG"); return e ? atoi(e) : 1; }();
    static const int kmin = [] { const char* e = getenv("MMFM_GEMM_BIG_KMIN"); return e ? atoi(e) : 512; }();
    if (!on || d.dtype != MMFM_BF16 || d.c_f32 || d.splits > 1 || !d.a_kcontig || !d.b_kcontig || d.colsum) return -1000;
    if (d.K % BK || d.K < kmin || d.N < 128 || d.M < 1024 || d.N % 8) return -1000;
    const char* mt = getenv("MMFM_GEMM_BIG_MIN_TILES");
    if (cdiv(d.M, TB) * cdiv(d.N, TB) < (mt ? atoi(mt) : 96)) return -1000;
    auto al16 = [](const void* p) { return p == nullptr || (uintptr_t)p % 16 == 0; };
    if (d.lda % 8 || d.ldb % 8 || d.ldc % 8 || (d.residual && d.ldr % 8) || !al16(d.A) || !al16(d.B) || !al16(d.C) || !al16(d.pre_out) ||
        !al16(d.gradmul_pre) || !al16(d.residual) || !al16(d.bias))
        return -1000;
    if ((int64_t)d.M * std::max(d.ldc, d.ldr) * 2 >= (int64_t)1 << 31) return -1000;
    const int ak = gemm_act_kind(d.act);
    const void* kern = ak == MMFM_MLP_RELU ? reinterpret_cast<const void*>(gemm_big_kernel<MMFM_MLP_RELU>)
                     : ak == MMFM_MLP_SIGMOID ? reinterpret_cast<const void*>(gemm_big_kernel<MMFM_MLP_SIGMOID>)
                     : ak == MMFM_MLP_GELU_TANH ? reinterpret_cast<const void*>(gemm_big_kernel<MMFM_MLP_GELU_TANH>)
                     : ak == kActEmbed ? reinterpret_cast<const void*>(gemm_big_kernel<kActEmbed>)
                     : reinterpret_cast<const void*>(gemm_big_kernel<0>);
    if (int rc = mmfm_lds_opt_in(kern, LDS_ALL, "mmfm_gemm(bf16, 256 tile)")) return rc;
    static const int nt_env = [] { const char* e = getenv("MMFM_GEMM_NT"); return e ? atoi(e) : 3; }();
    BigArgs a;
    a.d = d;
    a.tiles_n = cdiv(d.N, TB);
    a.ntiles = cdiv(d.M, TB) * a.tiles_n;
    a.nk = d.K / BK;
    a.nt_c = nt_env & 1;
    a.nt_pre = (nt_env >> 1) & 1;
    if (ak == MMFM_MLP_RELU) hipLaunchKernelGGL(gemm_big_kernel<MMFM_MLP_RELU>, dim3(std::min(a.ntiles, 256)), dim3(NT), LDS_ALL, st, a);
    else if (ak == MMFM_MLP_SIGMOID) hipLaunchKernelGGL(gemm_big_kernel<MMFM_MLP_SIGMOID>, dim3(std::min(a.ntiles, 256)), dim3(NT), LDS_ALL, st, a);
    else if (ak == MMFM_MLP_GELU_TANH) hipLaunchKernelGGL(gemm_big_kernel<MMFM_MLP_GELU_TANH>, dim3(std::min(a.ntiles, 256)), dim3(NT), LDS_ALL, st, a);
    else if (ak == kActEmbed) hipLaunchKernelGGL(gemm_big_kernel<kActEmbed>, dim3(std::min(a.ntiles, 256)), dim3(NT), LDS_ALL, st, a);
    else hipLaunchKernelGGL(gemm_big_kernel<0>, dim3(std::min(a.ntiles, 256)), dim3(NT), LDS_ALL, st, a);
    MMFM_LAUNCH_CHECK("mmfm_gemm(bf16, 256 tile)");
    return 0;
}
```

multi_modal_foundation_model_amd/csrc/gemm_dw.hip:

```cpp
#include "common.h"
#include <stdlib.h>
#include <algorithm>

namespace {

typedef __attribute__((address_space(3))) void lds_void_t;
typedef __attribute__((ext_vector_type(8))) __bf16 opnd;
typedef __attribute__((ext_vector_type(2))) unsigned int u32x2;
typedef __attribute__((ext_vector_type(4))) unsigned int u32x4;

constexpr int TM = 128, DNT = 256;
constexpr uint32_t OOB = 0x80000000u;

#ifndef MMFM_DW_LDS_KB
#define MMFM_DW_LDS_KB 160
#endif
template <int TN, int BK> struct Geo {
    static constexpr int OPA = BK * TM * 2, OPB = BK * TN * 2, STB = OPA + OPB;
    static constexpr int NST = (MMFM_DW_LDS_KB * 1024) / STB < 8 ? (MMFM_DW_LDS_KB * 1024) / STB : 8;
    static_assert(NST >= 3, "ring needs three stages");
    static constexpr int LDS = NST * STB;
    static constexpr int NA = BK / 16;
    static constexpr int NB = NA * (TN / TM);
    static constexpr int NJ = TN / 64;
};

struct DwArgs {
    mmfm_gemm_desc d;
    int tiles_n, ntiles, items;
};

__device__ __forceinline__ int xcd_order(int bid, int nwg) {
    const int q = nwg >> 3, r = nwg & 7, x = bid & 7;
    return (x < r ? x * (q + 1) : r * (q + 1) + (x - r) * q) + (bid >> 3);
}

__device__ __forceinline__ opnd mk_opnd(u32x2 lo, u32x2 hi) {
    u32x4 v;
    v[0] = lo[0]; v[1] = lo[1]; v[2] = hi[0]; v[3] = hi[1];
    return __builtin_bit_cast(opnd, v);
}

#define TR_READ(dst, addr, off) asm volatile("ds_read_b64_tr_b16 %0, %1 offset:%2" : "=v"(dst) : "v"(addr), "n"(off))
#define LDS_WAIT0 do { asm volatile("s_waitcnt lgkmcnt(0)" ::: "memory"); __builtin_amdgcn_sched_barrier(0); } while (0)
template <int N> __device__ __forceinline__ void vm_wait() { asm volatile("s_waitcnt vmcnt(%0)" :: "n"(N) : "memory"); }

struct DwPair {
    DwArgs a, b;
    int first;
};

template <int TN, int BK>
__global__ __launch_bounds__(DNT) void gemm_dw_kernel(const DwPair pr) {
    const bool second = pr.first > 0 && (int)blockIdx.x >= pr.first;
    const DwArgs& a = second ? pr.b : pr.a;
    const int w0 = second ? (int)blockIdx.x - pr.first : (int)blockIdx.x;
    const int wstep = pr.first > 0 ? (1 << 30) : (int)gridDim.x;
    typedef Geo<TN, BK> G;
    constexpr int NLW = 4;
    constexpr int NST = G::NST, NJ = G::NJ, RBB = TN * 2;
    extern __shared__ __attribute__((aligned(16))) char smem[];
    const mmfm_gemm_desc& d = a.d;
    const int t = threadIdx.x, lane = t & 63;
    const int wave = __builtin_amdgcn_readfirstlane(t >> 6);
    const int wm = wave >> 1, wn = wave & 1;
    const uint32_t ldaB = (uint32_t)d.lda * 2u, ldbB = (uint32_t)d.ldb * 2u;
    const __amdgpu_buffer_rsrc_t rsA = __builtin_amdgcn_make_buffer_rsrc(const_cast<void*>(d.A), 0, (int)((int64_t)d.K * ldaB), 0x00020000);
    const __amdgpu_buffer_rsrc_t rsB = __builtin_amdgcn_make_buffer_rsrc(const_cast<void*>(d.B), 0, (int)((int64_t)d.K * ldbB), 0x00020000);

    const int dkA = lane >> 4, dcA = (lane & 15) ^ (dkA << 2);
    constexpr int PPR = TN / 8, RPI = 64 / PPR;
    const int dkB = lane / PPR;
    const int dcB = (lane % PPR) ^ ((((RPI * wave) & 3) + dkB) << 2);
    const int g = lane >> 4, li = lane & 15, q = li >> 2, p = li & 3;
    const uint32_t lds0 = (uint32_t)(uintptr_t)(__attribute__((address_space(3))) char*)smem;
    uint32_t ra[2], rb[NJ];
#pragma unroll
    for (int i = 0; i < 2; ++i) ra[i] = lds0 + (uint32_t)((8 * (g >> 1) + q) * 256 + (((128 * wm + 64 * i) ^ (q << 6)) + 32 * (g & 1) + 8 * p));
#pragma unroll
    for (int j = 0; j < NJ; ++j)
        rb[j] = lds0 + (uint32_t)(G::OPA + (8 * (g >> 1) + q) * RBB + (((TN * wn + 64 * j) ^ (q << 6)) + 32 * (g & 1) + 8 * p));
    u32x4 ones4;
    ones4[0] = ones4[1] = ones4[2] = ones4[3] = 0x3F803F80u;
    const opnd ones = __builtin_bit_cast(opnd, ones4);

    for (int w = w0; w < a.items; w += wstep) {
        const int item = xcd_order(w, a.items);
        const int z = item / a.ntiles, tile = item - z * a.ntiles;
        const int m0 = (tile / a.tiles_n) * TM, n0 = (tile % a.tiles_n) * TN;
        const int kbeg = d.splits > 1 ? z * d.kchunk : 0;
        const int kend = d.splits > 1 ? min(d.K, kbeg + d.kchunk) : d.K;
        const int nk = (kend - kbeg + BK - 1) / BK;
        const bool do_cs = d.colsum != nullptr && n0 == 0 && wn == 0;

        const uint32_t srcA = (m0 + 8 * dcA < d.M) ? (uint32_t)dkA * ldaB + (uint32_t)(m0 + 8 * dcA) * 2u : OOB;
        const uint32_t srcB = (n0 + 8 * dcB < d.N) ? (uint32_t)dkB * ldbB + (uint32_t)(n0 + 8 * dcB) * 2u : OOB;
        auto issue = [&](int kt) {
            char* buf = smem + (kt % NST) * G::STB;
            const bool live = kt < nk;
            const uint32_t k0 = (uint32_t)(kbeg + kt * BK);
#pragma unroll
            for (int j = 0; j < G::NA; ++j) {
                const uint32_t kr = k0 + (uint32_t)(4 * (NLW * j + wave));
                const uint32_t va = live ? srcA + kr * ldaB : OOB;
                __builtin_amdgcn_raw_ptr_buffer_load_lds(rsA, (lds_void_t*)(buf + (NLW * j + wave) * 1024), 16, (int)va, 0, 0, 0);
            }
#pragma unroll
            for (int j = 0; j < G::NB; ++j) {
                const uint32_t kr = k0 + (uint32_t)(RPI * (NLW * j + wave));
                const uint32_t vb = live ? srcB + kr * ldbB : OOB;
                __builtin_amdgcn_raw_ptr_buffer_load_lds(rsB, (lds_void_t*)(buf + G::OPA + (NLW * j + wave) * 1024), 16, (int)vb, 0, 0, 0);
            }
        };
#pragma unroll
        for (int s = 0; s < NST - 1; ++s) issue(s);
// ... 46 lines not shown
            LDS_WAIT0;
            if (BK == 64) {
                READ_SET(0, 2)
                MMA_SET(1)
                LDS_WAIT0;
                READ_SET(1, 3)
                MMA_SET(0)
                LDS_WAIT0;
            }
            MMA_SET(1)
#undef READ_SET
#undef MMA_SET
        }
        asm volatile("s_waitcnt vmcnt(0)" ::: "memory");
        __builtin_amdgcn_s_barrier();

        float* Cf = reinterpret_cast<float*>(d.C) + (d.splits > 1 ? (size_t)z * d.slab_stride : 0);
        const int h = lane >> 5, l31 = lane & 31;
#pragma unroll
        for (int i = 0; i < 2; ++i)
#pragma unroll
            for (int j = 0; j < NJ; ++j) {
                const int n = n0 + (TN / 2) * wn + 32 * j + l31;
#pragma unroll
                for (int r = 0; r < 16; ++r) {
                    const int m = m0 + 64 * wm + 32 * i + (r & 3) + 8 * (r >> 2) + 4 * h;
                    if (m < d.M && n < d.N) Cf[(size_t)m * d.ldc + n] = acc[i][j][r];
                }
            }
        if (do_cs && l31 == 0) {
            float* csum = d.colsum + (d.splits > 1 ? (size_t)z * d.slab_stride : 0);
#pragma unroll
            for (int i = 0; i < 2; ++i)
#pragma unroll
                for (int r = 0; r < 16; ++r) {
                    const int m = m0 + 64 * wm + 32 * i + (r & 3) + 8 * (r >> 2) + 4 * h;
                    if (m < d.M) csum[m] = cs[i][r];
                }
        }
    }
}

template <int TN>
DwArgs make_args(const mmfm_gemm_desc& d) {
    DwArgs a;
    a.d = d;
    a.tiles_n = cdiv(d.N, TN);
    a.ntiles = cdiv(d.M, TM) * a.tiles_n;
    a.items = a.ntiles * std::max(1, d.splits);
    return a;
}

template <int TN, int BK>
int launch(const mmfm_gemm_desc& d, const mmfm_gemm_desc* d2, hipStream_t st) {
    typedef Geo<TN, BK> G;
    if (int rc = mmfm_lds_opt_in(reinterpret_cast<const void*>(gemm_dw_kernel<TN, BK>), G::LDS, "mmfm_gemm(bf16, dW stream)")) return rc;
    DwPair p;
    p.a = make_args<TN>(d);
    p.b = p.a;
    p.first = 0;
    int grid = std::min(p.a.items, 256);
    if (d2) {
        p.b = make_args<TN>(*d2);
        p.first = p.a.items;
        grid = p.a.items + p.b.items;
    }
    hipLaunchKernelGGL((gemm_dw_kernel<TN, BK>), dim3(grid), dim3(DNT), G::LDS, st, p);
    MMFM_LAUNCH_CHECK("mmfm_gemm(bf16, dW stream)");
    return 0;
}

}

static bool dw_wide(int N, int K) {
    static const int tn_env = [] { const char* e = getenv("MMFM_GEMM_DW_TN"); return e ? atoi(e) : 0; }();
    if (tn_env == 128 || N <= 128) return false;
    return tn_env == 256 || K >= 32768;
}

extern "C" int mmfm_gemm_dw_tiles(int M, int N, int K) { return cdiv(M, TM) * cdiv(N, dw_wide(N, K) ? 256 : 128); }

static bool dw_eligible(const mmfm_gemm_desc& d) {
    static const int on = [] { const char* e = getenv("MMFM_GEMM_DW"); return e ? atoi(e) : 1; }();
    const bool f32out = d.c_f32 || d.splits > 1;
    if (!on || d.dtype != MMFM_BF16 || !f32out || d.a_kcontig || d.b_kcontig) return false;
    if (d.bias || d.pre_out || d.gradmul_pre || d.residual || d.act || (d.drop.p > 0.f)) return false;
    if (d.lda % 8 || d.ldb % 8 || d.lda < (d.M + 7) / 8 * 8 || d.ldb < (d.N + 7) / 8 * 8 || ((uintptr_t)d.A & 15) || ((uintptr_t)d.B & 15) || ((uintptr_t)d.C & 3)) return false;
    if (d.splits > 1 && (d.kchunk % 64 || d.kchunk <= 0)) return false;
    if (((int64_t)d.K + 9 * 64) * std::max(d.lda, d.ldb) * 2 >= (int64_t)1 << 31) return false;
    return true;
}

int mmfm_gemm_dw_launch(const mmfm_gemm_desc* dp, hipStream_t st) {
    const mmfm_gemm_desc& d = *dp;
    if (!dw_eligible(d)) return -1000;
    return dw_wide(d.N, d.K) ? launch<256, 32>(d, nullptr, st) : launch<128, 32>(d, nullptr, st);
}

int mmfm_gemm_dw_pair_launch(const mmfm_gemm_desc* ap, const mmfm_gemm_desc* bp, hipStream_t st) {
    const mmfm_gemm_desc &a = *ap, &b = *bp;
    if (!dw_eligible(a) || !dw_eligible(b)) return -1000;
    const bool wide = dw_wide(a.N, a.K);
    if (wide != dw_wide(b.N, b.K)) return -1000;
    const int ia = mmfm_gemm_dw_tiles(a.M, a.N, a.K) * std::max(1, a.splits), ib = mmfm_gemm_dw_tiles(b.M, b.N, b.K) * std::max(1, b.splits);
    if (ia % 8 || ia + ib > 512) return -1000;
    return wide ? launch<256, 32>(a, &b, st) : launch<128, 32>(a, &b, st);
}
```

multi_modal_foundation_model_amd/csrc/stitch.hip:

```cpp
#include "common.h"
#include <algorithm>

namespace {

constexpr int MAXM = 8;
struct MaskSrc {
    const int64_t* p[MAXM];
    int64_t stride[MAXM];
    int64_t channels[MAXM];
};

__global__ void mask_prep_kernel(MaskSrc src, const int64_t* __restrict__ attn, int B, int T, int M, uint8_t* __restrict__ tokmask,
                                 uint8_t* __restrict__ keypad, uint8_t* __restrict__ keep0, uint8_t* __restrict__ mod_id,
                                 unsigned long long* __restrict__ count) {
    const int L = M * T;
    unsigned long long local[MAXM];
#pragma unroll
    for (int m = 0; m < MAXM; ++m) local[m] = 0;
    for (int64_t idx = (int64_t)blockIdx.x * blockDim.x + threadIdx.x; idx < (int64_t)B * L; idx += (int64_t)gridDim.x * blockDim.x) {
        const int b = (int)(idx / L), l = (int)(idx % L), m = l / T, t = l % T;
        const int64_t a = attn[(size_t)b * T + t];
        const int64_t v = src.p[m][((size_t)b * T + t) * src.stride[m]] & a;
        tokmask[idx] = (uint8_t)(v != 0);
        keypad[idx] = (uint8_t)(a != 0);
        if (b == 0) {
            keep0[l] = (uint8_t)(v != 1);
            mod_id[l] = (uint8_t)m;
        }
#pragma unroll
        for (int mm = 0; mm < MAXM; ++mm)
            if (mm == m) local[mm] += (unsigned long long)v * (unsigned long long)src.channels[mm];
    }
#pragma unroll
    for (int m = 0; m < MAXM; ++m) {
        if (m < M) {
            unsigned long long s = local[m];
            for (int o = 32; o > 0; o >>= 1) s += __shfl_xor(s, o);
            if ((threadIdx.x & 63) == 0 && s) atomicAdd(&count[m], s);
        }
    }
}

__global__ void zero_u64_kernel(unsigned long long* p, int n) {
    if ((int)threadIdx.x < n) p[threadIdx.x] = 0ull;
}

template <typename T>
__global__ __launch_bounds__(256) void stitch_fwd_kernel(const T* __restrict__ tok, const float* __restrict__ mod_row,
                                                         const float* __restrict__ pos, const int64_t* __restrict__ ts,
                                                         const uint8_t* __restrict__ keep0, T* __restrict__ x, T* __restrict__ emb,
                                                         int B, int Tn, int L, int m, int H, int max_F) {
    const int C4 = H / 4;
    const int64_t total = (int64_t)B * Tn * C4;
    for (int64_t idx = (int64_t)blockIdx.x * blockDim.x + threadIdx.x; idx < total; idx += (int64_t)gridDim.x * blockDim.x) {
        const int64_t r = idx / C4;
        const int c = (int)(idx % C4) * 4;
        const int b = (int)(r / Tn), t = (int)(r % Tn);
        const int l = m * Tn + t;
        const float4 mr = *reinterpret_cast<const float4*>(mod_row + c);
        float4 e = mr;
        if (pos) {
            const int tsv = (int)min((int64_t)(max_F - 1), max((int64_t)0, ts[r]));
            const float4 pr = *reinterpret_cast<const float4*>(pos + (size_t)tsv * H + c);
            e = make_float4(mr.x + pr.x, mr.y + pr.y, mr.z + pr.z, mr.w + pr.w);
        }
        const size_t o = ((size_t)b * L + l) * H + c;
        if (emb) io<T>::st4(emb + o, e);
        if (keep0[l]) {
            const float4 tv = io<T>::ld4(tok + (size_t)r * H + c);
            e.x += tv.x; e.y += tv.y; e.z += tv.z; e.w += tv.w;
        }
        io<T>::st4(x + o, e);
    }
}

template <typename T, bool POS>
__global__ void stitch_bwd_kernel(const T* __restrict__ dx, const T* __restrict__ dextra, const int64_t* __restrict__ ts,
                                  const uint8_t* __restrict__ keep0, mmfm_dropout dropa, T* __restrict__ d_tok,
                                  float* __restrict__ part, int B, int Tn, int L, int m, int H, int max_F, int bper) {
    extern __shared__ __attribute__((aligned(16))) float tab[];
    const int CW = blockDim.x, j = threadIdx.x, col = blockIdx.x * CW + j;
    const Drop dr = drop_init(dropa);
    for (int f = 0; f < max_F; ++f) tab[f * CW + j] = 0.f;
    float macc = 0.f;
    const int b0 = blockIdx.y * bper, b1 = min(B, b0 + bper);
    for (int b = b0; b < b1; ++b) {
        for (int t = 0; t < Tn; ++t) {
            const int l = m * Tn + t;
            const size_t o = ((size_t)b * L + l) * H + col;
            const float g = io<T>::ld(dx + o);
            float e = g;
            if (dextra) e += io<T>::ld(dextra + o);
            const int64_t r = (int64_t)b * Tn + t;
            if (POS) {
                const int tsv = (int)min((int64_t)(max_F - 1), max((int64_t)0, ts[r]));
                tab[tsv * CW + j] += e;
            }
            macc += e;
            if (d_tok) io<T>::st(d_tok + (size_t)r * H + col, keep0[l] ? dr.apply(g, (uint64_t)r * H + col) : 0.f);
        }
    }
    float* out = part + (size_t)blockIdx.y * (max_F + 1) * H;
    for (int f = 0; f < max_F; ++f) out[(size_t)f * H + col] = tab[f * CW + j];
    out[(size_t)max_F * H + col] = macc;
}

__global__ __launch_bounds__(256) void onehot_kernel(const int64_t* __restrict__ ts, uint16_t* __restrict__ oh, int B, int Tn, int L, int m,
                                                     int max_F, int ohc) {
    const int cpr = ohc / 8;
    const int64_t total = (int64_t)B * L * cpr;
    for (int64_t idx = (int64_t)blockIdx.x * blockDim.x + threadIdx.x; idx < total; idx += (int64_t)gridDim.x * blockDim.x) {
        const int64_t row = idx / cpr;
        const int c0 = (int)(idx % cpr) * 8;
        const int b = (int)(row / L), l = (int)(row % L), t = l - m * Tn;
        uint32_t w[4] = {0u, 0u, 0u, 0u};
        if (t >= 0 && t < Tn) {
            const int tsv = (int)min((int64_t)(max_F - 1), max((int64_t)0, ts[(int64_t)b * Tn + t]));
#pragma unroll
            for (int j = 0; j < 8; ++j)
                if (c0 + j == tsv || c0 + j == max_F) w[j >> 1] |= 0x3F80u << (16 * (j & 1));
        }
        *reinterpret_cast<uint4*>(oh + row * ohc + c0) = make_uint4(w[0], w[1], w[2], w[3]);
    }
}

__global__ __launch_bounds__(256) void stitch_modsum_kernel(const uint16_t* __restrict__ dx, const uint16_t* __restrict__ dextra,
                                                            float* __restrict__ part, int B, int Tn, int L, int m, int H, int bper) {
    __shared__ float4 red[4][64];
    const int lane = threadIdx.x & 63, rl = threadIdx.x >> 6;
    const int c = blockIdx.x * 256 + lane * 4;
    const int b0 = blockIdx.y * bper, b1 = min(B, b0 + bper);
    float4 acc = make_float4(0.f, 0.f, 0.f, 0.f);
    if (c < H) {
        for (int64_t r = (int64_t)b0 * Tn + rl; r < (int64_t)b1 * Tn; r += 4) {
            const size_t o = ((size_t)(r / Tn) * L + (size_t)m * Tn + (size_t)(r % Tn)) * H + c;
            float4 e = io<uint16_t>::ld4(dx + o);
            if (dextra) {
                const float4 x = io<uint16_t>::ld4(dextra + o);
                e.x += x.x; e.y += x.y; e.z += x.z; e.w += x.w;
            }
            acc.x += e.x; acc.y += e.y; acc.z += e.z; acc.w += e.w;
        }
    }
    red[rl][lane] = acc;
    __syncthreads();
    if (rl == 0 && c < H) {
        float4 o;
        o.x = (red[0][lane].x + red[1][lane].x) + (red[2][lane].x + red[3][lane].x);
        o.y = (red[0][lane].y + red[1][lane].y) + (red[2][lane].y + red[3][lane].y);
        o.z = (red[0][lane].z + red[1][lane].z) + (red[2][lane].z + red[3][lane].z);
        o.w = (red[0][lane].w + red[1][lane].w) + (red[2][lane].w + red[3][lane].w);
        *reinterpret_cast<float4*>(part + (size_t)blockIdx.y * H + c) = o;
    }
}

__global__ __launch_bounds__(256) void stitch_dtok_kernel(const uint16_t* __restrict__ dx, const uint8_t* __restrict__ keep0, mmfm_dropout dropa,
                                                          uint16_t* __restrict__ d_tok, int B, int Tn, int L, int m, int H) {
    const Drop dr = drop_init(dropa);
    const int C8 = H / 8;
    const int64_t total = (int64_t)B * Tn * C8;
    for (int64_t idx = (int64_t)blockIdx.x * blockDim.x + threadIdx.x; idx < total; idx += (int64_t)gridDim.x * blockDim.x) {
        const int64_t r = idx / C8;
        const int c = (int)(idx % C8) * 8;
        const int b = (int)(r / Tn), l = m * Tn + (int)(r % Tn);
        uint4 o = make_uint4(0u, 0u, 0u, 0u);
        if (keep0[l]) {
            const uint4 g = *reinterpret_cast<const uint4*>(dx + ((size_t)b * L + l) * H + c);
            if (dr.on()) {
                const uint32_t gw[4] = {g.x, g.y, g.z, g.w};
                uint32_t ow[4];
#pragma unroll
                for (int j = 0; j < 4; ++j) {
                    const float v0 = dr.apply(__uint_as_float(gw[j] << 16), (uint64_t)r * H + c + 2 * j);
                    const float v1 = dr.apply(__uint_as_float(gw[j] & 0xffff0000u), (uint64_t)r * H + c + 2 * j + 1);
                    ow[j] = (uint32_t)f2bf(v0) | ((uint32_t)f2bf(v1) << 16);
                }
                o = make_uint4(ow[0], ow[1], ow[2], ow[3]);
            } else {
                o = g;
            }
        }
        *reinterpret_cast<uint4*>(d_tok + (size_t)r * H + c) = o;
    }
}

struct CollateArgs {
    const uint8_t* data;
    const int32_t* indices;
    const int64_t* indptr;
    const int64_t* indptr_off;
    const int64_t* nnz_off;
    const int32_t* T_b;
    const int32_t* N_b;
};
__global__ __launch_bounds__(256) void collate_csr_kernel(CollateArgs a, int B, int max_T, int max_N, float pad, float* __restrict__ out,
                                                          int64_t* __restrict__ tmask, int64_t* __restrict__ smask) {
    const int lane = threadIdx.x & 63, wave = threadIdx.x >> 6;
    for (int64_t row = (int64_t)blockIdx.x * 4 + wave; row < (int64_t)B * max_T; row += (int64_t)gridDim.x * 4) {
        const int b = (int)(row / max_T), t = (int)(row % max_T);
        const int Tb = a.T_b[b], Nb = a.N_b[b];
        const bool live = t < Tb;
        const int nvalid = min(Nb, max_N);
        float* o = out + row * max_N;
        for (int n = lane; n < max_N; n += 64) o[n] = (live && n < nvalid) ? 0.f : pad;
        if (lane == 0) tmask[row] = live ? 1 : 0;
        if (t == 0)
            for (int n = lane; n < max_N; n += 64) smask[(size_t)b * max_N + n] = n < nvalid ? 1 : 0;
        if (!live) continue;
        __threadfence_block();
        __builtin_amdgcn_wave_barrier();
        const int64_t* ip = a.indptr + a.indptr_off[b];
        const int64_t z0 = ip[t], z1 = ip[t + 1], base = a.nnz_off[b];
        for (int64_t z = z0 + lane; z < z1; z += 64) {
            const int col = a.indices[base + z];
            if (col >= 0 && col < nvalid) atomicAdd(o + col, (float)a.data[base + z]);
        }
    }
}

int pick_cw(int H, int max_F) {
    for (int cw : {256, 128, 64, 32, 16, 8, 4})
        if (H % cw == 0 && (size_t)max_F * cw * 4 <= 60 * 1024) return cw;
    return 0;
}
int stitch_chunks(int B, int H, int cw) { return std::max(1, std::min(B, 512 / std::max(1, H / cw))); }
struct OhGeo { int ohc, S, kchunk; int64_t oh_bytes, slab; };
OhGeo oh_geo(int B, int L, int H, int max_F) {
    OhGeo g;
    g.ohc = (max_F + 1 + 7) & ~7;
    const int64_t K = (int64_t)B * L;
    const int tiles = ((max_F + 1 + 127) / 128) * ((H + 127) / 128);
    int S = (int)std::max<int64_t>(1, std::min<int64_t>(K / 512, (512 + tiles - 1) / tiles));
    g.kchunk = (int)(((K + S - 1) / S + 63) / 64 * 64);
    g.S = (int)((K + g.kchunk - 1) / g.kchunk);
    g.oh_bytes = ((int64_t)K * g.ohc * 2 + 255) / 256 * 256;
    g.slab = (int64_t)(max_F + 1) * H;
    return g;
}
bool oh_path(int dtype, int H) { return dtype == MMFM_BF16 && H % 8 == 0; }

}

extern "C" int mmfm_reduce_slabs(float*, const float*, int64_t, int, int64_t, int, mmfm_stream);
int mmfm_gemm_bf16_launch(const mmfm_gemm_desc* dp, hipStream_t st);

extern "C" int mmfm_mask_prep(int B, int T, int M, const int64_t* const* mask_src, const int64_t* mask_stride,
                              const int64_t* attn, const int64_t* channels, uint8_t* tokmask, uint8_t* keypad,
                              uint8_t* keep0, uint8_t* mod_id, int64_t* count, mmfm_stream stream) {
    MMFM_REQUIRE(B > 0 && T > 0 && M > 0 && M <= MAXM, "mmfm_mask_prep: bad shape B=%d T=%d M=%d (M <= %d)", B, T, M, MAXM);
    MMFM_REQUIRE(mask_src && mask_stride && attn && channels && tokmask && keypad && keep0 && mod_id && count, "mmfm_mask_prep: null pointer");
    MMFM_REQUIRE(M * T <= 65535, "mmfm_mask_prep: sequence too long");
    MaskSrc src;
    for (int m = 0; m < MAXM; ++m) {
        src.p[m] = m < M ? mask_src[m] : nullptr;
        src.stride[m] = m < M ? mask_stride[m] : 0;
        src.channels[m] = m < M ? channels[m] : 0;
        MMFM_REQUIRE(m >= M || (src.p[m] && src.stride[m] > 0), "mmfm_mask_prep: modality %d has no mask source", m);
    }
    hipStream_t st = (hipStream_t)stream;
    hipLaunchKernelGGL(zero_u64_kernel, dim3(1), dim3(64), 0, st, (unsigned long long*)count, M);
    MMFM_LAUNCH_CHECK("mmfm_mask_prep(zero)");
    const int64_t n = (int64_t)B * M * T;
    hipLaunchKernelGGL(mask_prep_kernel, dim3((int)std::min<int64_t>(256, (n + 255) / 256)), dim3(256), 0, st, src, attn, B, T, M,
                       tokmask, keypad, keep0, mod_id, (unsigned long long*)count);
    MMFM_LAUNCH_CHECK("mmfm_mask_prep");
    return 0;
}

extern "C" int mmfm_collate_csr(int B, int max_T, int max_N, float pad_value, const uint8_t* data, const int32_t* indices,
                                const int64_t* indptr, const int64_t* indptr_off, const int64_t* nnz_off, const int32_t* T_b,
                                const int32_t* N_b, float* out, int64_t* time_mask, int64_t* space_mask, mmfm_stream stream) {
    MMFM_REQUIRE(B > 0 && max_T > 0 && max_N > 0, "mmfm_collate_csr: bad shape");
    MMFM_REQUIRE(indptr && indptr_off && nnz_off && T_b && N_b && out && time_mask && space_mask, "mmfm_collate_csr: null pointer");
    CollateArgs a{data, indices, indptr, indptr_off, nnz_off, T_b, N_b};
    const int64_t rows = (int64_t)B * max_T;
    hipLaunchKernelGGL(collate_csr_kernel, dim3((int)std::min<int64_t>(4096, (rows + 3) / 4)), dim3(256), 0, (hipStream_t)stream, a, B, max_T,
                       max_N, pad_value, out, time_mask, space_mask);
    MMFM_LAUNCH_CHECK("mmfm_collate_csr");
    return 0;
}

extern "C" int mmfm_stitch_fwd(int dtype, const void* tok, const float* mod_emb_row, const float* pos_emb, const int64_t* ts,
                               const uint8_t* keep0, void* x, void* emb, int B, int T, int L, int m, int H, int max_F, mmfm_stream stream) {
    MMFM_REQUIRE(tok && mod_emb_row && (ts || !pos_emb) && keep0 && x, "mmfm_stitch_fwd: null pointer");
    MMFM_REQUIRE(B > 0 && T > 0 && H > 0 && H % 4 == 0 && m >= 0 && (m + 1) * T <= L && max_F > 0, "mmfm_stitch_fwd: bad shape");
    const int64_t n = (int64_t)B * T * (H / 4);
    dim3 grid((int)std::min<int64_t>(4096, (n + 255) / 256)), block(256);
    hipStream_t st = (hipStream_t)stream;
    if (dtype == MMFM_F32)
        hipLaunchKernelGGL(stitch_fwd_kernel<float>, grid, block, 0, st, (const float*)tok, mod_emb_row, pos_emb, ts, keep0, (float*)x, (float*)emb, B, T, L, m, H, max_F);
    else if (dtype == MMFM_BF16)
        hipLaunchKernelGGL(stitch_fwd_kernel<uint16_t>, grid, block, 0, st, (const uint16_t*)tok, mod_emb_row, pos_emb, ts, keep0, (uint16_t*)x, (uint16_t*)emb, B, T, L, m, H, max_F);
    else
        return mmfm_set_error(-1, "mmfm_stitch_fwd: bad dtype %d", dtype);
    MMFM_LAUNCH_CHECK("mmfm_stitch_fwd");
    return 0;
}

extern "C" int64_t mmfm_stitch_bwd_workspace(int dtype, int B, int T, int L, int H, int max_F) {
    (void)T;
    if (oh_path(dtype, H)) {
        const OhGeo g = oh_geo(B, L, H, max_F);
        return g.oh_bytes + 2 * (int64_t)g.S * g.slab * (int64_t)sizeof(float);
    }
    const int cw = pick_cw(H, max_F);
    if (!cw) return -1;
    return (int64_t)stitch_chunks(B, H, cw) * (max_F + 1) * H * sizeof(float);
}

extern "C" int mmfm_stitch_bwd(int dtype, const void* dx, const void* dextra, const int64_t* ts, const uint8_t* keep0,
                               mmfm_dropout drop, void* d_tok, float* d_mod_row, float* d_pos, int acc_mod, int acc_pos, int B, int T,
                               int L, int m, int H, int max_F, void* workspace, int64_t workspace_bytes, mmfm_stream stream) {
    MMFM_REQUIRE(dx && (ts || !d_pos) && keep0 && d_mod_row, "mmfm_stitch_bwd: null pointer");
    MMFM_REQUIRE(B > 0 && T > 0 && H > 0 && max_F > 0 && m >= 0 && (m + 1) * T <= L, "mmfm_stitch_bwd: bad shape");
    if (oh_path(dtype, H)) {
        const OhGeo g = oh_geo(B, L, H, max_F);
        MMFM_REQUIRE(workspace && workspace_bytes >= mmfm_stitch_bwd_workspace(dtype, B, T, L, H, max_F), "mmfm_stitch_bwd: workspace too small");
        MMFM_REQUIRE((uintptr_t)dx % 16 == 0 && (!dextra || (uintptr_t)dextra % 16 == 0) && (!d_tok || (uintptr_t)d_tok % 16 == 0) &&
                     (uintptr_t)workspace % 16 == 0, "mmfm_stitch_bwd: bf16 tensors must be 16-byte aligned");
        hipStream_t st = (hipStream_t)stream;
        if (!d_pos) {
            const int64_t room = mmfm_stitch_bwd_workspace(dtype, B, T, L, H, max_F) / ((int64_t)H * (int64_t)sizeof(float));
            const int S = (int)std::max<int64_t>(1, std::min<int64_t>(std::min<int64_t>(B, 256), room));
            const int bper = (B + S - 1) / S, nsl = (B + bper - 1) / bper;
            if (d_tok) {
                const int64_t n = (int64_t)B * T * (H / 8);
                hipLaunchKernelGGL(stitch_dtok_kernel, dim3((int)std::min<int64_t>(4096, (n + 255) / 256)), dim3(256), 0, st, (const uint16_t*)dx, keep0,
                                   drop, (uint16_t*)d_tok, B, T, L, m, H);
            }
            hipLaunchKernelGGL(stitch_modsum_kernel, dim3(cdiv(H, 256), nsl), dim3(256), 0, st, (const uint16_t*)dx, (const uint16_t*)dextra,
                               (float*)workspace, B, T, L, m, H, bper);
            MMFM_LAUNCH_CHECK("mmfm_stitch_bwd(column sum)");
            return mmfm_reduce_slabs(d_mod_row, (const float*)workspace, H, nsl, H, acc_mod, stream);
        }
        uint16_t* oh = reinterpret_cast<uint16_t*>(workspace);
        float* slabs = reinterpret_cast<float*>(reinterpret_cast<char*>(workspace) + g.oh_bytes);
        const int64_t nch = (int64_t)B * L * (g.ohc / 8);
        hipLaunchKernelGGL(onehot_kernel, dim3((int)std::min<int64_t>(4096, (nch + 255) / 256)), dim3(256), 0, st, ts, oh, B, T, L, m, max_F, g.ohc);
        if (d_tok) {
            const int64_t n = (int64_t)B * T * (H / 8);
            hipLaunchKernelGGL(stitch_dtok_kernel, dim3((int)std::min<int64_t>(4096, (n + 255) / 256)), dim3(256), 0, st, (const uint16_t*)dx, keep0,
                               drop, (uint16_t*)d_tok, B, T, L, m, H);
        }
        MMFM_LAUNCH_CHECK("mmfm_stitch_bwd(one-hot)");
        mmfm_gemm_desc gd = {};
        gd.dtype = MMFM_BF16; gd.c_f32 = 1;
        gd.A = oh; gd.lda = g.ohc; gd.a_kcontig = 0;
        gd.ldb = H; gd.b_kcontig = 0;
        gd.M = max_F + 1; gd.N = H; gd.K = B * L; gd.ldc = H;
        gd.splits = g.S; gd.kchunk = g.kchunk; gd.slab_stride = g.slab;
        gd.act_scale = 1.f;
        int nsl = 0;
        for (const void* src : {dx, dextra}) {
            if (!src) continue;
            gd.B = src;
            gd.C = slabs + (int64_t)nsl * g.slab;
            if (int rc = mmfm_gemm_bf16_launch(&gd, st)) return rc;
            nsl += g.S;
        }
        if (int rc = mmfm_reduce_slabs(d_pos, slabs, (int64_t)max_F * H, nsl, g.slab, acc_pos, stream)) return rc;
        return mmfm_reduce_slabs(d_mod_row, slabs + (int64_t)max_F * H, H, nsl, g.slab, acc_mod, stream);
    }
    const int cw = pick_cw(H, max_F);
    MMFM_REQUIRE(cw > 0, "mmfm_stitch_bwd: no column slab fits LDS for H=%d max_F=%d", H, max_F);
    const int nch = stitch_chunks(B, H, cw);
    MMFM_REQUIRE(workspace && workspace_bytes >= mmfm_stitch_bwd_workspace(dtype, B, T, L, H, max_F), "mmfm_stitch_bwd: workspace too small");
    const int bper = (B + nch - 1) / nch;
    dim3 grid(H / cw, nch), block(cw);
    const size_t lds = (size_t)max_F * cw * sizeof(float);
    hipStream_t st = (hipStream_t)stream;
    MMFM_REQUIRE(dtype == MMFM_F32 || dtype == MMFM_BF16, "mmfm_stitch_bwd: bad dtype %d", dtype);
    if (!d_pos) {
        if (dtype == MMFM_F32)
            hipLaunchKernelGGL((stitch_bwd_kernel<float, false>), grid, block, 0, st, (const float*)dx, (const float*)dextra, ts, keep0, drop,
                               (float*)d_tok, (float*)workspace, B, T, L, m, H, 0, bper);
        else
            hipLaunchKernelGGL((stitch_bwd_kernel<uint16_t, false>), grid, block, 0, st, (const uint16_t*)dx, (const uint16_t*)dextra, ts, keep0, drop,
                               (uint16_t*)d_tok, (float*)workspace, B, T, L, m, H, 0, bper);
        MMFM_LAUNCH_CHECK("mmfm_stitch_bwd(no table)");
        return mmfm_reduce_slabs(d_mod_row, (const float*)workspace, H, nch, H, acc_mod, stream);
    }
    if (dtype == MMFM_F32)
        hipLaunchKernelGGL((stitch_bwd_kernel<float, true>), grid, block, lds, st, (const float*)dx, (const float*)dextra, ts, keep0, drop, (float*)d_tok,
                           (float*)workspace, B, T, L, m, H, max_F, bper);
    else
        hipLaunchKernelGGL((stitch_bwd_kernel<uint16_t, true>), grid, block, lds, st, (const uint16_t*)dx, (const uint16_t*)dextra, ts, keep0, drop,
                           (uint16_t*)d_tok, (float*)workspace, B, T, L, m, H, max_F, bper);
    MMFM_LAUNCH_CHECK("mmfm_stitch_bwd");
    const int64_t stride = (int64_t)(max_F + 1) * H;
    if (int rc = mmfm_reduce_slabs(d_pos, (const float*)workspace, (int64_t)max_F * H, nch, stride, acc_pos, stream)) return rc;
    return mmfm_reduce_slabs(d_mod_row, (const float*)workspace + (size_t)max_F * H, H, nch, stride, acc_mod, stream);
}
```

multi_modal_foundation_model_amd/ops.py:

```python
from __future__ import annotations

import ctypes as C

import torch

from . import _lib as L


def _stream():
    return torch.cuda.current_stream().cuda_stream


def run_plan(plan, stream=None):
    st = _stream() if stream is None else stream
    for fn, args, _keep in plan:
        rc = fn(*args, st)
        if rc:
            L.check(rc, fn.__name__)


def _emit(plan, fn, args, keep=()):
    if plan is None:
        L.check(fn(*args, _stream()), fn.__name__)
    else:
        plan.append((fn, args, keep))


def P(t):
    return None if t is None else t.data_ptr()


def dt(t):
    if t.dtype == torch.float32:
        return L.F32
    if t.dtype == torch.bfloat16:
        return L.BF16
    raise TypeError(f"unsupported dtype {t.dtype}")


def dropout(state, site, p):
    if state is None or p <= 0:
        return L.NO_DROP
    return L.Dropout(state.data_ptr(), site, float(p))


def gemm_desc(A, B, Cout, M, N, K, *, lda, ldb, ldc, a_kcontig=1, b_kcontig=1, bias=None, pre_out=None, act=0,
              act_scale=1.0, gradmul_pre=None, drop=None, residual=None, ldr=0, splits=1, kchunk=0, slab_stride=0,
              dtype=None, c_f32=0, colsum=None):
    d = L.GemmDesc()
    d.dtype = dt(A) if dtype is None else dtype
    d.c_f32 = c_f32
    d.A, d.B, d.C = P(A), P(B), P(Cout)
    d.M, d.N, d.K, d.lda, d.ldb, d.ldc = M, N, K, lda, ldb, ldc
    d.a_kcontig, d.b_kcontig = a_kcontig, b_kcontig
    d.splits, d.kchunk, d.slab_stride = splits, kchunk, slab_stride
    d.bias, d.pre_out, d.act, d.act_scale, d.gradmul_pre = P(bias), P(pre_out), act, act_scale, P(gradmul_pre)
    d.drop = drop if drop is not None else L.NO_DROP
    d.residual, d.ldr = P(residual), ldr
    d.colsum = colsum if isinstance(colsum, int) else P(colsum)
    return d


def gemm(A, B, Cout, M, N, K, *, plan=None, **kw):
    d = gemm_desc(A, B, Cout, M, N, K, **kw)
    _emit(plan, L.lib().mmfm_gemm, (C.byref(d),), keep=(d,))


def gemm_pair(da, db, plan=None):
    _emit(plan, L.lib().mmfm_gemm_pair, (C.byref(da), C.byref(db)), keep=(da, db))


def reduce_slabs(dst, src, n, nslabs, stride, accumulate=False, plan=None):
    _emit(plan, L.lib().mmfm_reduce_slabs, (P(dst), P(src), n, nslabs, stride, int(accumulate)))


def reduce_slabs_multi(items, device, plan=None):
    import numpy as np
    arr = (L.ReduceEntry * len(items))()
    chunk0 = 0
    for a, (dst, src, n, nslabs, stride, acc) in zip(arr, items):
        a.dst, a.src, a.n, a.slab_stride, a.nslabs, a.accumulate, a.chunk0 = P(dst), P(src), n, stride, nslabs, int(acc), chunk0
        chunk0 += (n + 255) // 256
    table = torch.from_numpy(np.frombuffer(bytes(arr), dtype=np.uint8).copy()).to(device)
    _emit(plan, L.lib().mmfm_reduce_slabs_multi, (P(table), len(items), chunk0), keep=(table,))


def colsum(x, R, N, ld, out, ws, accumulate=False, plan=None):
    _emit(plan, L.lib().mmfm_colsum, (dt(x), P(x), R, N, ld, P(out), int(accumulate), P(ws), ws.numel() * ws.element_size()))


def layernorm_fwd(x, gamma, beta, y, mean, rstd, R, H, eps=1e-5, ds_L=0, ds_T=0, plan=None):
    _emit(plan, L.lib().mmfm_layernorm_fwd, (dt(x), P(x), P(gamma), P(beta), P(y), P(mean), P(rstd), R, H, eps, ds_L, ds_T))


def layernorm_bwd(dy, x, mean, rstd, gamma, dres, dx, dgamma, dbeta, R, H, ws, accumulate=False, ds_L=0, ds_T=0, plan=None):
    _emit(plan, L.lib().mmfm_layernorm_bwd, (dt(x), P(dy), P(x), P(mean), P(rstd), P(gamma), P(dres), P(dx), P(dgamma),
                                             P(dbeta), int(accumulate), R, H, ds_L, ds_T, P(ws), ws.numel() * ws.element_size()))


def scalenorm_fwd(x, g, y, rinv, R, H, eps=1e-5, plan=None):
    _emit(plan, L.lib().mmfm_scalenorm_fwd, (dt(x), P(x), P(g), P(y), P(rinv), R, H, eps))


def scalenorm_bwd_workspace(R, H):
    return int(L.lib().mmfm_scalenorm_bwd_workspace(R, H))


def scalenorm_bwd(dy, x, rinv, g, dres, dx, dg, R, H, ws, accumulate=False, plan=None):
    _emit(plan, L.lib().mmfm_scalenorm_bwd, (dt(x), P(dy), P(x), P(rinv), P(g), P(dres), P(dx), P(dg), int(accumulate), R, H, P(ws),
                                             ws.numel() * ws.element_size()))


def attn_desc(dtype, B, heads, Lq, Lk, dh, q, k, v, ldq, ldk, ldv, o, ldo, lse, keypad, mod_id, flags, scale,
              drop_p=None, drop_o=None, d_o=None, lddo=0, dq=None, dk=None, dv=None, lddq=0, lddk=0, lddv=0, keepbits=None):
    d = L.AttnDesc()
    d.dtype, d.B, d.heads, d.Lq, d.Lk, d.dh = dtype, B, heads, Lq, Lk, dh
    d.q, d.k, d.v, d.ldq, d.ldk, d.ldv = q, k, v, ldq, ldk, ldv
    d.o, d.ldo, d.lse, d.keypad, d.mod_id, d.flags, d.scale = o, ldo, P(lse), P(keypad), P(mod_id), flags, scale
    d.drop_p = drop_p if drop_p is not None else L.NO_DROP
    d.drop_o = drop_o if drop_o is not None else L.NO_DROP
    d.d_o, d.lddo, d.dq, d.dk, d.dv, d.lddq, d.lddk, d.lddv = d_o, lddo, dq, dk, dv, lddq, lddk, lddv
    d.keepbits = P(keepbits)
    return d


def attn_keepbits_bytes(B, heads, Lq, Lk):
    return int(L.lib().mmfm_attn_keepbits_bytes(B, heads, Lq, Lk))


def attn_keep_prob(p):
    return float(L.lib().mmfm_attn_keep_prob(float(p)))


def attn_fwd(desc, plan=None):
    _emit(plan, L.lib().mmfm_attn_fwd, (C.byref(desc),), keep=(desc,))


def attn_bwd(desc, plan=None):
    _emit(plan, L.lib().mmfm_attn_bwd, (C.byref(desc),), keep=(desc,))


def mask_prep(B, T, masks, strides, attn, channels, tokmask, keypad, keep0, mod_id, count, plan=None):
    M = len(masks)
    src = (C.c_void_p * M)(*[m.data_ptr() for m in masks])
    st = (C.c_int64 * M)(*strides)
    ch = (C.c_int64 * M)(*channels)
    _emit(plan, L.lib().mmfm_mask_prep, (B, T, M, src, st, P(attn), ch, P(tokmask), P(keypad), P(keep0), P(mod_id), P(count)),
          keep=(src, st, ch))


def stitch_fwd(tok, mod_row, pos, ts, keep0, x, emb, B, T, Lseq, m, H, max_F, plan=None):
    _emit(plan, L.lib().mmfm_stitch_fwd, (dt(tok), P(tok), P(mod_row), P(pos), P(ts), P(keep0), P(x), P(emb), B, T, Lseq, m, H, max_F))


def stitch_bwd(dx, dextra, ts, keep0, drop, d_tok, d_mod_row, d_pos, acc_mod, acc_pos, B, T, Lseq, m, H, max_F, ws, plan=None):
    _emit(plan, L.lib().mmfm_stitch_bwd, (dt(dx), P(dx), P(dextra), P(ts), P(keep0), drop if drop is not None else L.NO_DROP,
                                          P(d_tok), P(d_mod_row), P(d_pos), int(acc_mod), int(acc_pos), B, T, Lseq, m, H, max_F, P(ws),
                                          ws.numel() * ws.element_size()))


def masked_loss_fwd(kind, pred, target, rowmask, mask_ld, T, R, N, loss_sum, ws, plan=None):
    _emit(plan, L.lib().mmfm_masked_loss_fwd, (dt(pred), kind, P(pred), P(target), P(rowmask), mask_ld, T, R, N, P(loss_sum), P(ws),
                                               ws.numel() * ws.element_size()))


def masked_loss_kind_fwd(kind, param, flags, pred, target, rowmask, mask_ld, T, R, N, loss_sum, ws, plan=None):
    _emit(plan, L.lib().mmfm_masked_loss_kind_fwd, (dt(pred), kind, float(param), flags, P(pred), P(target), P(rowmask), mask_ld, T, R, N,
                                                    P(loss_sum), P(ws), ws.numel() * ws.element_size()))


def loss_finalize(loss_sum, count, M, loss, inv_n, plan=None):
    _emit(plan, L.lib().mmfm_loss_finalize, (P(loss_sum), P(count), M, P(loss), P(inv_n)))


def masked_loss_bwd(kind, pred, target, rowmask, mask_ld, T, R, N, grad_out, inv_n, dpred, plan=None):
    _emit(plan, L.lib().mmfm_masked_loss_bwd, (dt(pred), kind, P(pred), P(target), P(rowmask), mask_ld, T, R, N, P(grad_out), P(inv_n), P(dpred)))


def masked_loss_kind_bwd(kind, param, flags, pred, target, rowmask, mask_ld, T, R, N, grad_out, inv_n, dpred, plan=None):
    _emit(plan, L.lib().mmfm_masked_loss_kind_bwd, (dt(pred), kind, float(param), flags, P(pred), P(target), P(rowmask), mask_ld, T, R, N,
                                                    P(grad_out), P(inv_n), P(dpred)))


def dropout_apply(src, dst, R, N, drop, plan=None):
    _emit(plan, L.lib().mmfm_dropout_apply, (dt(src), P(src), P(dst), R, N, drop))


def cast_bf16(src, dst, n, plan=None):
    _emit(plan, L.lib().mmfm_cast_f32_to_bf16, (P(src), P(dst), n))


def adamw_step(p, g, m, v, p_bf16, n, hyper, plan=None):
    _emit(plan, L.lib().mmfm_adamw_step, (P(p), P(g), P(m), P(v), P(p_bf16), n, P(hyper)))


def rng_seed(state, seed, plan=None):
    _emit(plan, L.lib().mmfm_rng_seed, (P(state), int(seed) & (2 ** 64 - 1)))


def rng_advance(state, plan=None):
    _emit(plan, L.lib().mmfm_rng_advance, (P(state),))


def collate_csr(B, max_T, max_N, pad_value, data, indices, indptr, indptr_off, nnz_off, T_b, N_b, out, tmask, smask, plan=None):
    _emit(plan, L.lib().mmfm_collate_csr, (B, max_T, max_N, float(pad_value), P(data), P(indices), P(indptr), P(indptr_off), P(nnz_off),
# ... 125 lines not shown
```

multi_modal_foundation_model_amd/plan.py:

```python
from __future__ import annotations

import functools
import math
import os
from collections import namedtuple

import torch

from . import _lib as L
from . import ops as K


def _align(n, a=8):
    return (n + a - 1) // a * a


Switches = namedtuple("Switches", "fused gemm_big gemm_dw batch_reduce dw_pair attn_keepbits mlp_bwd_split")


def read_switches() -> Switches:
    env, on = os.environ, lambda k: os.environ.get(k, "1") != "0"
    return Switches(fused=int(env["MMFM_FUSED"]) if "MMFM_FUSED" in env else None, gemm_big=on("MMFM_GEMM_BIG"), gemm_dw=on("MMFM_GEMM_DW"),
                    batch_reduce=on("MMFM_BATCH_REDUCE"), dw_pair=on("MMFM_DW_PAIR"), attn_keepbits=on("MMFM_ATTN_KEEPBITS"),
                    mlp_bwd_split=env.get("MMFM_MLP_BWD_SPLIT", "1") == "1")


class Side:
    def __init__(self, sc, training):
        self.heads, self.I, self.act, self.scale, self.mult, self.max_F = sc.heads, sc.inter, sc.act, sc.embed_scale, sc.mult, sc.max_F
        self.dp, self.dpe = (sc.dropout, sc.embed_dropout) if training else (0.0, 0.0)
        self.act_fwd, self.act_grad = K.GEMM_ACTS[sc.act[0]]
        self.emb_act, self.pos = sc.embed_act, sc.embed_pos
        self.emb_fwd, self.emb_grad = K.embed_act(sc.embed_act)
        self.use_keep = self.F_MLP = False


class PlanBuilder:
    def __init__(self, engine, B, T, training, grad=True):
        e, c = self.e, self.c = engine, engine.cfg
        self.B, self.T, self.training, self.grad = B, T, bool(training), bool(grad)
        self.sw = read_switches()
        self.mods_of = {side: c.side_mods(side) for side in ("encoder", "decoder")}
        self.H, self.M = c.hidden, len(self.mods_of["encoder"])
        if len(self.mods_of["decoder"]) != self.M:
            raise RuntimeError(f"engine: the encoder's sequence has {self.M * T} tokens ({self.M} modalities x {T}), the decoder's "
                               f"{len(self.mods_of['decoder']) * T}: cross-attention needs the two lengths equal")
        self.Lq, self.R, self.BT = self.M * T, B * self.M * T, B * T
        self.split_masks = [m for m, _, _ in self.mods_of["encoder"]] != [m for m, _, _ in self.mods_of["decoder"]]
        self.staged = sorted({m for side in self.mods_of.values() for m, _, _ in side})
        self.sides = {side: Side(c.side(side), training) for side in ("encoder", "decoder")}
        self.Imax, self.mult_max = max(sd.I for sd in self.sides.values()), max(sd.mult for sd in self.sides.values())
        self.code, self.es, self.buf, self.b = e.code, 4 if e.dtype == "fp32" else 2, e._buf, e.b
        self.enc_flags = L.ATTN_DIAG
        self.dec_flags = (L.ATTN_CAUSAL if c.causal_mask else 0) | (L.ATTN_SEP if c.sep_mask else 0)
        self.fwd, self.bwd, self.cur = [], [], []
        self.pend: list = []
        self.late_lng: list = []
        self.slabm_off = 0
        self.deferred: list = []
        self.used_wt: list = []
        self.stream_in = {}

    def embed_saved(self, sd):
        if sd.emb_fwd == L.ACT_EMB_IDENTITY:
            return None
        if sd.emb_fwd == L.ACT_SOFTSIGN and self.code == L.BF16:
            return "a"
        return "z"

    def mk(self, side, name):
        return "dec/" + name if self.split_masks and side == "decoder" else name

    def side(self, name):
        return self.sides["encoder" if name.startswith("enc") else "decoder"]

    @staticmethod
    def rows(t, R, N):
        return t if tuple(t.shape) == (R, N) else t.view(-1)[:R * N].view(R, N)

    def build(self):
        self.workspaces()
        self.forward()
        plan = dict(fwd=self.fwd, bwd=None, B=self.B, T=self.T, training=self.training, M=self.M, R=self.R, BT=self.BT,
                    runs=dict(fwd=0, bwd=0), graphs={}, b=self.b, count=self.mk("decoder", "count"))
        if self.grad:
            self.backward()
            plan.update(bwd=self.bwd, fused=self.fm, use_keep=any(sd.use_keep for sd in self.sides.values()))
        return plan

    def workspaces(self):
        e, c, buf, sw = self.e, self.c, self.buf, self.sw
        B, T, H, R, BT, Lq, M = self.B, self.T, self.H, self.R, self.BT, self.Lq, self.M
        f32, i64, u8 = torch.float32, torch.int64, torch.uint8
        dec = {m for m, _, _ in self.mods_of["decoder"]}
        chans = [c.mods[m][1] for m in self.staged]
        for m in self.staged:
            n = c.mods[m][1]
            buf(f"in/{m}", (BT, _align(n, 8)), zero=True); buf(f"mask/{m}", (B, T), i64)
            if m in dec:
                buf(f"tgt/{m}", (BT, n), f32)
        buf("ts", (B, T), i64); buf("attn", (B, T), i64); buf("loss_sum", (M,), f32)
        for pre in ("", "dec/") if self.split_masks else ("",):
            buf(pre + "tokmask", (B, Lq), u8); buf(pre + "keypad", (B, Lq), u8)
            buf(pre + "keep0", (Lq,), u8); buf(pre + "mod_id", (Lq,), u8); buf(pre + "count", (M,), i64)
        max_slab = 1
        for n in chans:
            for mult in sorted({sd.mult for sd in self.sides.values()}):
                for (mm, nn, ldn) in ((n * mult, n, _align(n, 8)), (H, n * mult, None), (n, H, None)):
                    max_slab = max(max_slab, e._dw_split(mm, nn, BT, ldn=ldn, sw=sw)[0] * _align(mm * nn + mm))
        for l in e.linears:
            max_slab = max(max_slab, e._dw_split(l.N, l.K, R, sw=sw)[0] * _align(l.N * l.K + l.N))
        self.slab = buf("ws/slab", (max_slab,), f32)
        self.slab2 = buf("ws/slab2", (max_slab,), f32)
        self.batch_red = R <= 8192 and sw.batch_reduce
        if self.batch_red:
            seg_max = max(end - s0 for _, s0, end in e.layout.segments)
            self.slabm = buf("ws/slabm", (max(1, min(R // 256, 15)) * (seg_max + 128 * 64),), f32)
        maxN = max([3 * H, self.Imax] + [n * self.mult_max for n in chans])
        buf("ws/col", (max(1, L.lib().mmfm_colsum_workspace(R, maxN) // 4),), f32)
        buf("ws/ln", (max(1, L.lib().mmfm_layernorm_bwd_workspace(R, H) // 4),), f32)
        buf("ws/stitch", (max(1, max(L.lib().mmfm_stitch_bwd_workspace(self.code, B, T, Lq, H, sd.max_F) for sd in self.sides.values()) // 4),), f32)
        buf("ws/loss", (max(1, L.lib().mmfm_masked_loss_workspace(BT, 1) // 4),), f32)
        self.pair_ok = self.code == L.BF16 and not self.batch_red and sw.dw_pair and sw.gemm_dw
        fm = self.fm = e._fused_mask(R, sw)
        self.F_QKV, self.F_LNL, self.F_OUT = bool(fm & 1), bool(fm & 2), bool(fm & 8)
        for name, sd in self.sides.items():
            sd.use_keep = self.code == L.BF16 and sd.dp > 0 and self.grad and sw.attn_keepbits
            sd.F_MLP = e.fused_mlp(name, fm)
        self.prep = e._build_prep() if fm else None
        if fm:
            K.prep_weights(self.prep["table"], self.prep["n"], self.prep["tiles"], plan=self.fwd)
            self.gdb = buf("ws/gdb", (max(_align(l.N * l.K + l.N) for l in e.linears if l.norm),), f32)
            if "ws/lng" not in self.b:
                self.b["ws/lng"] = K.ln_linear_grad_workspace(H, e.device)

    def slab_region(self, S, stride):
        o = self.slabm_off
        self.slabm_off = o + S * stride
        if self.slabm_off > self.slabm.numel():
            raise RuntimeError(f"engine: ws/slabm holds {self.slabm.numel()} floats, the plan's slab regions need {self.slabm_off}")
        return self.slabm[o:o + S * stride]

    def lin(self, plan, X, wname, Y, Mr, N, Kd, ldx=None, **kw):
        K.gemm(X, self.e.W(wname + ".weight"), Y, Mr, N, Kd, lda=ldx or Kd, ldb=Kd, ldc=N, bias=self.e.Pb(wname), dtype=self.code, plan=plan, **kw)

    def wgrad(self, plan, dY, X, dst, N, Kd, Mr, nb, S, kchunk, what, ldx=None, colsum=None, slab=None, paired=False):
        n = N * Kd + nb
        if S == 1 and not paired:
            out, cs, split, red = dst, colsum if colsum is not None else (dst.data_ptr() + 4 * N * Kd if nb else None), {}, None
        else:
            stride = _align(n) if nb else n
            out = self.slab_region(S, stride) if self.batch_red else slab
            if S * stride > out.numel():
                raise RuntimeError(f"engine: {what}: {S} slabs x {stride} floats exceed the {out.numel()}-float slab workspace")
            cs = out.data_ptr() + 4 * N * Kd if nb else None
            split, red = dict(splits=S, kchunk=kchunk, slab_stride=stride), (dst, out, n, S, stride)
        emit = K.gemm_desc if paired else functools.partial(K.gemm, plan=plan)
        d = emit(dY, X, out, N, Kd, Mr, lda=N, ldb=ldx or Kd, ldc=Kd, a_kcontig=0, b_kcontig=0, dtype=self.code, c_f32=1, colsum=cs, **split)
        if paired:
            return d, red
        if red is not None:
            self.reduce(plan, red)

    def reduce(self, plan, red):
        if self.batch_red:
            self.pend.append(red + (False,))
        else:
            K.reduce_slabs(*red, plan=plan)

    def pair_splits(self, Na, Ka, Nb, Kb, Mr):
        ta, tb = L.lib().mmfm_gemm_dw_tiles(Na, Ka, Mr), L.lib().mmfm_gemm_dw_tiles(Nb, Kb, Mr)
        ia = 256 * (Na + Ka) / (Na + Ka + Nb + Kb)
        Sa = max(1, int(ia) // ta)
        while Sa > 1 and (ta * Sa) % 8:
            Sa -= 1
        Sb = max(1, (256 - ta * Sa) // tb)
        out = []
        for S in (Sa, Sb):
            kchunk = _align(-(-Mr // max(1, min(S, Mr // 512))), 64)
            out += [-(-Mr // kchunk), kchunk]
        return out

    def flush_deferred(self, plan):
        if self.deferred:
            a = self.deferred.pop()
            self.dlin(plan, a["dY"], a["X"], a["wname"], a["Mr"], a["N"], a["Kd"])

    def dlin(self, plan, dY, X, wname, Mr, N, Kd, dX=None, ldx=None, defer=False, **kw):
        e, code = self.e, self.code
        S, kchunk = e._dw_split(N, Kd, Mr, ldn=ldx, sw=self.sw)
        gw, gb = e.Gv(wname + ".weight"), e.Gb(wname)
        fused = code == L.BF16 and gb is not None
        adjacent = fused and gb.data_ptr() == gw.data_ptr() + 4 * N * Kd
        if defer and self.pair_ok and S > 1 and (adjacent or gb is None) and dX is None and ldx in (None, Kd):
            self.flush_deferred(plan)
            self.deferred.append(dict(dY=dY, X=X, wname=wname, Mr=Mr, N=N, Kd=Kd, nb=N if gb is not None else 0))
            return
        self.wgrad(plan, dY, X, gw, N, Kd, Mr, N if adjacent and S > 1 else 0, S, kchunk, wname, ldx=ldx, colsum=gb if fused else None, slab=self.slab)
        if gb is not None and (not fused or (S > 1 and not adjacent)):
            K.colsum(dY, Mr, N, N, gb, self.b["ws/col"], plan=plan)
        if dX is not None:
            wT = e._w_transposed(wname, N, Kd, Mr, sw=self.sw) if code == L.BF16 else None
            if wT is not None:
                self.used_wt.append(wname)
                K.gemm(dY, wT, dX, Mr, Kd, N, lda=N, ldb=N, ldc=Kd, b_kcontig=1, dtype=code, plan=plan, **kw)
            else:
                K.gemm(dY, e.W(wname + ".weight"), dX, Mr, Kd, N, lda=N, ldb=Kd, ldc=Kd, b_kcontig=0, dtype=code, plan=plan, **kw)

    def lin_norm_grad(self, plan, Gdb, wname, lnname, N):
        e, H, ws = self.e, self.H, self.b["ws/lng"]
        if e.is_sn(lnname):
            K.sn_linear_grad(Gdb, e.Pf(wname + ".weight"), e.Pf(lnname + ".scale"), N, H, e.Gv(wname + ".weight"),
                             e.Gb(wname), e.Gv(lnname + ".scale"), ws, plan=plan)
            return
        K.ln_linear_grad(Gdb, e.Pf(wname + ".weight"), e.Pf(lnname + ".weight"), e.Pf(lnname + ".bias"), N, H,
                         e.Gv(wname + ".weight"), e.Gb(wname), e.Gv(lnname + ".weight"), e.Gv(lnname + ".bias"), ws, plan=plan)

    def dlin_ln(self, plan, dYt, tag, wname, lnname, N):
        H, R, deferred = self.H, self.R, self.deferred
        S, kchunk = self.e._dw_split(N, H, R, sw=self.sw)
        xh = self.b[tag + "/xh"]
        nb = N if (self.e.Gb(wname) is not None or not self.e.is_sn(lnname)) else 0
        if deferred and S > 1 and deferred[-1]["Mr"] == R:
            a = deferred.pop()
            Sa, kca, Sb, kcb = self.pair_splits(a["N"], a["Kd"], N, H, R)
            da, ra = self.wgrad(plan, a["dY"], a["X"], self.e.Gv(a["wname"] + ".weight"), a["N"], a["Kd"], R, a["nb"], Sa, kca, a["wname"],
                                slab=self.slab2, paired=True)
            db_, rb = self.wgrad(plan, dYt, xh, self.gdb, N, H, R, nb, Sb, kcb, wname, slab=self.slab, paired=True)
            K.gemm_pair(da, db_, plan=plan)
            self.reduce(plan, ra)
            self.reduce(plan, rb)
        elif self.batch_red and S > 1:
            g_site = self.buf(f"ws/gdb/{len(self.late_lng)}", (self.gdb.numel(),), torch.float32)
            self.wgrad(plan, dYt, xh, g_site, N, H, R, nb, S, kchunk, wname)
            self.late_lng.append((g_site, wname, lnname, N))
            return
        else:
            self.wgrad(plan, dYt, xh, self.gdb, N, H, R, nb, S, kchunk, wname, slab=self.slab)
        self.lin_norm_grad(plan, self.gdb, wname, lnname, N)

    def ln_f(self, plan, X, name, Y, tag, **kw):
        e, R, H, f32 = self.e, self.R, self.H, torch.float32
        if e.is_sn(name):
            K.scalenorm_fwd(X, e.Pf(name + ".scale"), Y, self.buf(tag + "/rstd", (R,), f32), R, H, plan=plan)
            return
        K.layernorm_fwd(X, e.Pf(name + ".weight"), e.Pf(name + ".bias"), Y, self.buf(tag + "/mean", (R,), f32),
                        self.buf(tag + "/rstd", (R,), f32), R, H, plan=plan, **kw)

    def ln_b(self, plan, dY, X, name, tag, dres, dX, **kw):
        e, b, R, H = self.e, self.b, self.R, self.H
        if e.is_sn(name):
            K.scalenorm_bwd(dY, X, b[tag + "/rstd"], e.Pf(name + ".scale"), dres, dX, e.Gv(name + ".scale"), R, H, b["ws/ln"], plan=plan)
            return
        K.layernorm_bwd(dY, X, b[tag + "/mean"], b[tag + "/rstd"], e.Pf(name + ".weight"), dres, dX,
                        e.Gv(name + ".weight"), e.Gv(name + ".bias"), R, H, b["ws/ln"], plan=plan, **kw)

    def ln_lin(self, plan, Xin, lnname, wname, Yout, N, tag, residual=None, alias=None):
        b, R, H = self.b, self.R, self.H
        pw = self.prep["v"][wname]
        xh = rs = None
# ... 24 lines not shown
    def loss(self, plan, mod, two_kind, kind_fn, *args):
        c = self.c
        kind, param, flags = c.loss_kind[mod], float(c.loss_param.get(mod, 0.0)), int(c.loss_flags.get(mod, 0))
        if kind in (L.LOSS_POISSON_LOG, L.LOSS_MSE) and flags == 0:
            two_kind(kind, *args, plan=plan)
        else:
            kind_fn(kind, param, flags, *args, plan=plan)

    def out_proj(self, plan, a, wname, Xres, Xout):
        R, H = self.R, self.H
        if self.F_OUT:
            K.rowgemm(a, self.e.W(wname + ".weight"), Xout, R, H, H, bias=self.e.Pb(wname), residual=Xres, ldr=H, plan=plan)
        else:
            self.lin(plan, a, wname, Xout, R, H, H, residual=Xres, ldr=H)

    def self_block(self, plan, X, p, tag, flags):
        buf, R, H = self.buf, self.R, self.H
        qkv, a, Xa = buf(tag + "/qkv", (R, 3 * H)), buf(tag + "/a", (R, H)), buf(tag + "/xa", (R, H))
        if self.F_QKV:
            self.ln_lin(plan, X, p + ".ln1", p + ".attn.qkv", qkv, 3 * H, tag + "/ln1")
        else:
            self.ln_f(plan, X, p + ".ln1", buf(tag + "/h1", (R, H)), tag + "/ln1")
            self.lin(plan, self.b[tag + "/h1"], p + ".attn.qkv", qkv, R, 3 * H, H)
        K.attn_fwd(self.attn_desc(tag + "/sa", qkv, 3 * H, qkv, 3 * H, H, 2 * H, a, flags), plan=plan)
        self.out_proj(plan, a, p + ".attn.out_proj", X, Xa)
        return Xa

    def mlp_block(self, plan, X, p, tag):
        e, buf, R, H, f32, sd = self.e, self.buf, self.R, self.H, torch.float32, self.side(p)
        I, dp = sd.I, sd.dp
        Xb = buf(tag + "/xb", (R, H))
        if sd.F_MLP:
            pu = self.prep["v"][p + ".mlp.up_proj"]
            d_ = K.mlp_desc(R, x=X, w_up=pu["Wp"], b_up=pu["bp"], w_down=self.prep["v"][p + ".mlp.down_proj"]["WpP"],
                            b_down=e.Pb(p + ".mlp.down_proj"), drop=e._drop(tag + "/mlpdrop", dp), y=Xb,
                            xhat=buf(tag + "/ln2/xh", (R, H)) if self.grad else None,
                            rstd=buf(tag + "/ln2/rs", (R,), f32) if self.grad else None, scalenorm=e.is_sn(p + ".ln2"),
                            act=sd.act[0], act_beta=sd.act[1])
            K.mlp_fwd(d_, plan=plan)
            return Xb
        h, u, g = buf(tag + "/h2", (R, H)), buf(tag + "/u", (R, I)), buf(tag + "/g", (R, I))
        self.ln_f(plan, X, p + ".ln2", h, tag + "/ln2")
        self.lin(plan, h, p + ".mlp.up_proj", g, R, I, H, pre_out=u, act=sd.act_fwd, act_scale=sd.act[1])
        self.lin(plan, g, p + ".mlp.down_proj", Xb, R, H, I, drop=e._drop(tag + "/mlpdrop", dp), residual=X, ldr=H)
        return Xb

    def forward(self):
        e, c, b, buf, fwd = self.e, self.c, self.b, self.buf, self.fwd
        B, T, H, R, BT, Lq, M = self.B, self.T, self.H, self.R, self.BT, self.Lq, self.M
        mk = self.mk
        for side in ("encoder", "decoder") if self.split_masks else ("encoder",):
            K.mask_prep(B, T, [b[f"mask/{m}"] for m, _, _ in self.mods_of[side]], [1] * M, b["attn"], [n for _, _, n in self.mods_of[side]],
                        b[mk(side, "tokmask")], b[mk(side, "keypad")], b[mk(side, "keep0")], b[mk(side, "mod_id")], b[mk(side, "count")], plan=fwd)
        tok_tmp = buf("tok_tmp", (BT, H))
        x_enc, emb_enc, x_dec = buf("x_enc", (R, H)), buf("emb_enc", (R, H)), buf("x_dec", (R, H))
        for side, xs, es_ in (("encoder", x_enc, emb_enc), ("decoder", x_dec, None)):
            sd = self.sides[side]
            for slot, (m, mod, n) in enumerate(self.mods_of[side]):
                p = f"{side}_embeddings.{mod}.embedder"
                n2 = n * sd.mult
                a = buf(f"{side}/a/{m}", (BT, n2))
                z = buf(f"{side}/z/{m}", (BT, n2)) if self.embed_saved(sd) == "z" else None
                self.lin(fwd, b[f"in/{m}"], p + ".token_embed", a, BT, n2, n, ldx=_align(n, 8), pre_out=z, act=sd.emb_fwd, act_scale=sd.scale)
                self.lin(fwd, a, p + ".projection", tok_tmp, BT, H, n2, drop=e._drop(f"{side}/embdrop/{m}", sd.dpe))
                mod_row = e.Pf(f"{c.mod_emb_owner(side, mod)}_embeddings.{mod}.embedder.mod_emb.weight")[m]
                pos = e.Pf(p + ".pos_embed.weight") if sd.pos else None
                K.stitch_fwd(tok_tmp, mod_row, pos, b["ts"], b[mk(side, "keep0")], xs, es_, B, T, Lq, slot, H, sd.max_F, plan=fwd)
        X = x_enc
        for i in range(c.n_enc):
            p, tag = f"encoder.{i}", f"enc{i}"
            self.stream_in[tag] = X
            X = self.mlp_block(fwd, self.self_block(fwd, X, p, tag, self.enc_flags), p, tag)
        self.enc_last = X
        enc_out, context = buf("enc_out", (R, H)), buf("context", (R, H))
        if self.F_LNL:
            self.ln_lin(fwd, X, "encoder_norm", "decoder_proj_context", context, H, "encnorm", residual=emb_enc)
        else:
            self.ln_f(fwd, X, "encoder_norm", enc_out, "encnorm")
            self.lin(fwd, enc_out, "decoder_proj_context", context, R, H, H, residual=emb_enc, ldr=H)
        Y = x_dec
        for i in range(c.n_dec):
            p, tag = f"decoder.{i}", f"dec{i}"
            self.stream_in[tag] = Y
            Ya = self.self_block(fwd, Y, p, tag, self.dec_flags)
            qc, kvc, a2, Yb = buf(tag + "/qc", (R, H)), buf(tag + "/kvc", (R, 2 * H)), buf(tag + "/a2", (R, H)), buf(tag + "/yb", (R, H))
            if self.F_LNL:
                self.ln_lin(fwd, Ya, p + ".query_norm", p + ".cross_attn.query", qc, H, tag + "/qn")
                self.ln_lin(fwd, context, p + ".context_norm", p + ".cross_attn.kv", kvc, 2 * H, tag + "/cn", alias=None if i == 0 else "dec0/cn")
            else:
                hq, hc = buf(tag + "/hq", (R, H)), buf(tag + "/hc", (R, H))
                self.ln_f(fwd, Ya, p + ".query_norm", hq, tag + "/qn")
                self.ln_f(fwd, context, p + ".context_norm", hc, tag + "/cn")
                self.lin(fwd, hq, p + ".cross_attn.query", qc, R, H, H)
                self.lin(fwd, hc, p + ".cross_attn.kv", kvc, R, 2 * H, H)
            K.attn_fwd(self.attn_desc(tag + "/xa", qc, H, kvc, 2 * H, 0, H, a2, self.enc_flags), plan=fwd)
            self.out_proj(fwd, a2, p + ".cross_attn.out_proj", Ya, Yb)
            Y = self.mlp_block(fwd, Yb, p, tag)
        self.dec_last = Y
        ydec = buf("ydec", (R, H))
        self.ln_f(fwd, Y, "decoder_norm", ydec, "decnorm", ds_L=Lq, ds_T=T)
        tokmask = b[mk("decoder", "tokmask")]
        for j, (m, mod, n) in enumerate(self.mods_of["decoder"]):
            pred = buf(f"pred/{m}", (BT, n))
            self.lin(fwd, ydec[j * BT:(j + 1) * BT], f"decoder_embeddings.{mod}.out", pred, BT, n, H)
            self.loss(fwd, mod, K.masked_loss_fwd, K.masked_loss_kind_fwd, pred, b[f"tgt/{m}"], tokmask[:, j * T:], Lq, T, BT, n,
                      b["loss_sum"][j:j + 1], b["ws/loss"])
        K.loss_finalize(b["loss_sum"], b[mk("decoder", "count")], M, b["loss"], b["inv_n"], plan=fwd)

    def close_segment(self, name):
        if self.pend:
            K.reduce_slabs_multi(list(self.pend), self.e.device, plan=self.cur)
            self.pend.clear()
        for g_site, wname, lnname, N in self.late_lng:
            self.lin_norm_grad(self.cur, g_site, wname, lnname, N)
        self.late_lng.clear()
        self.slabm_off = 0
        self.bwd.append((name, self.cur))
        self.cur = []

    def mlp_back(self, plan, dS, p, tag, X_in):
# ... 42 lines not shown
    def self_back(self, plan, dS, p, tag, flags):
        b, H = self.b, self.H
        self.out_proj_back(plan, dS, b[tag + "/a"], p + ".attn.out_proj")
        qkv, dqkv = b[tag + "/qkv"], b["d/qkv"]
        K.attn_bwd(self.attn_desc(tag + "/sa", qkv, 3 * H, qkv, 3 * H, H, 2 * H, b[tag + "/a"], flags, d_o=b["d/t2"], dq=dqkv, dkv=dqkv,
                                  lddq=3 * H, lddkv=3 * H, dkoff=H, dvoff=2 * H), plan=plan)
        self.norm_lin_back(plan, self.F_QKV, dqkv, 3 * H, tag + "/ln1", p + ".attn.qkv", p + ".ln1", tag + "/h1", self.stream_in[tag], dS, dS)

    def cross_back(self, plan, dY, p, tag, dctx_in):
        b, H, dqc, dkvc = self.b, self.H, self.b["d/qc"], self.b["d/kvc"]
        self.out_proj_back(plan, dY, b[tag + "/a2"], p + ".cross_attn.out_proj")
        K.attn_bwd(self.attn_desc(tag + "/xa", b[tag + "/qc"], H, b[tag + "/kvc"], 2 * H, 0, H, b[tag + "/a2"], self.enc_flags,
                                  d_o=b["d/t2"], dq=dqc, dkv=dkvc, lddq=H, lddkv=2 * H, dkoff=0, dvoff=H), plan=plan)
        self.norm_lin_back(plan, self.F_LNL, dqc, H, tag + "/qn", p + ".cross_attn.query", p + ".query_norm", tag + "/hq", b[tag + "/xa"], dY, dY)
        self.norm_lin_back(plan, self.F_LNL, dkvc, 2 * H, tag + "/cn", p + ".cross_attn.kv", p + ".context_norm", tag + "/hc", b["context"],
                           dctx_in, b["d/ctx"])

    def backward(self):
        e, c, b, buf = self.e, self.c, self.b, self.buf
        B, T, H, I, R, BT, Lq = self.B, self.T, self.H, self.Imax, self.R, self.BT, self.Lq
        dY, dydec = buf("d/stream", (R, H)), buf("d/ydec", (R, H))
        buf("d/t1", (R, H)); buf("d/t2", (R, H)); buf("d/h", (R, H)); buf("d/u", (R, I)); buf("d/qkv", (R, 3 * H)); dctx = buf("d/ctx", (R, H))
        ydec = b["ydec"]
        tokmask = b[self.mk("decoder", "tokmask")]
        for j, (m, mod, n) in enumerate(self.mods_of["decoder"]):
            dpred = buf(f"d/pred/{m}", (BT, n))
            self.loss(self.cur, mod, K.masked_loss_bwd, K.masked_loss_kind_bwd, b[f"pred/{m}"], b[f"tgt/{m}"], tokmask[:, j * T:],
                      Lq, T, BT, n, b["gout"], b["inv_n"], dpred)
            self.dlin(self.cur, dpred, ydec[j * BT:(j + 1) * BT], f"decoder_embeddings.{mod}.out", BT, n, H, dX=dydec[j * BT:(j + 1) * BT])
        self.ln_b(self.cur, dydec, self.dec_last, "decoder_norm", "decnorm", None, dY, ds_L=Lq, ds_T=T)
        self.close_segment("head")
        buf("d/qc", (R, H)); buf("d/kvc", (R, 2 * H))
        for i in reversed(range(c.n_dec)):
            p, tag = f"decoder.{i}", f"dec{i}"
            self.mlp_back(self.cur, dY, p, tag, b[tag + "/yb"])
            self.cross_back(self.cur, dY, p, tag, None if i == c.n_dec - 1 else dctx)
            self.self_back(self.cur, dY, p, tag, self.dec_flags)
            self.close_segment(p)
        if c.n_dec == 0:
            raise NotImplementedError("n_dec == 0")
        dX = buf("d/xstream", (R, H))
        self.norm_lin_back(self.cur, self.F_LNL, dctx, H, "encnorm", "decoder_proj_context", "encoder_norm", "enc_out", self.enc_last, None, dX)
        self.close_segment("bridge")
        for i in reversed(range(c.n_enc)):
            p, tag = f"encoder.{i}", f"enc{i}"
            self.mlp_back(self.cur, dX, p, tag, b[tag + "/xa"])
            self.self_back(self.cur, dX, p, tag, self.enc_flags)
            self.close_segment(p)
        shared = {mod for _, mod, _ in self.mods_of["decoder"] if c.mod_emb_owner("decoder", mod) == "encoder"}
        for side, dS, dextra in (("decoder", dY, None), ("encoder", dX, dctx)):
            sd = self.sides[side]
            for slot, (m, mod, n) in enumerate(self.mods_of[side]):
                pS = f"{side}_embeddings.{mod}.embedder"
                K.stitch_bwd(dS, dextra, b["ts"], b[self.mk(side, "keep0")], e._drop(f"{side}/embdrop/{m}", sd.dpe), buf(f"d/tok/{side}/{m}", (BT, H)),
                             e.Gv(f"{c.mod_emb_owner(side, mod)}_embeddings.{mod}.embedder.mod_emb.weight")[m],
                             e.Gv(pS + ".pos_embed.weight") if sd.pos else None,
                             side == "encoder" and mod in shared, False, B, T, Lq, slot, H, sd.max_F, b["ws/stitch"], plan=self.cur)
        for side in ("decoder", "encoder"):
            sd = self.sides[side]
            saved = self.embed_saved(sd)
            for m, mod, n in self.mods_of[side]:
                p = f"{side}_embeddings.{mod}.embedder"
                n2 = n * sd.mult
                dz = self.rows(buf(f"d/z/{m}", (BT, n * self.mult_max)), BT, n2)
                self.dlin(self.cur, b[f"d/tok/{side}/{m}"], b[f"{side}/a/{m}"], p + ".projection", BT, H, n2, dX=dz,
                          act=L.ACT_SOFTSIGN_GRAD_OUT if saved == "a" else sd.emb_grad, act_scale=sd.scale,
                          gradmul_pre=b[f"{side}/{saved}/{m}"] if saved else None)
                self.dlin(self.cur, dz, b[f"in/{m}"], p + ".token_embed", BT, n2, n, ldx=_align(n, 8))
        self.close_segment("embed")
        if self.used_wt:
            tw = e._wt_table()
            K.prep_weights(tw["table"], tw["n"], tw["tiles"], plan=self.fwd)
            self.fwd.insert(0, self.fwd.pop())
```

Measured before the change: 35870 samples/s.

## Compute embedding GEMMs only on live (unmasked) time bins via row compaction

Adds a live-bin record per modality built from the keep mask, gathers only live input rows, and runs the token-embed and projection GEMMs (forward and backward, including wgrad) on the compacted row count read on device. Stitch forward/backward get live-aware variants that scatter compacted tokens back into the sequence, and dropout keys use the original row index so masks are unchanged. This removes embedding work for bins that are masked out, at the cost of extra gather kernels, a device-side row-count read inside each GEMM, and more complex launch paths.

Measured after the change: 37230 samples/s (median of 6 runs). 3.8% higher.

```diff
diff --git a/include/mmfm.h b/include/mmfm.h
--- a/include/mmfm.h
+++ b/include/mmfm.h
@@ -53,6 +53,16 @@
 int mmfm_gemm(const mmfm_gemm_desc* d, mmfm_stream stream);
 int mmfm_gemm_pair(const mmfm_gemm_desc* a, const mmfm_gemm_desc* b, mmfm_stream stream);
 
+#define MMFM_LIVE_ROWS 1
+#define MMFM_LIVE_REC_INTS(T) (2 * (T) + 4)
+int mmfm_live_bins(const uint8_t* keep0, int T, int M, int32_t* rec, mmfm_stream stream);
+int mmfm_gather_live_rows(const void* src, void* dst, int B, int T, int64_t row_bytes, const int32_t* rec, mmfm_stream stream);
+typedef struct {
+    const int32_t* rec;
+    int B, T;
+} mmfm_live_rows;
+int mmfm_gemm_live(const mmfm_gemm_desc* d, const mmfm_live_rows* live, mmfm_stream stream);
+
 int mmfm_gemm_dw_tiles(int M, int N, int K);
 int mmfm_reduce_slabs(float* dst, const float* src, int64_t n, int nslabs, int64_t slab_stride,
                       int accumulate, mmfm_stream stream);
@@ -120,6 +130,13 @@
                     mmfm_dropout drop, void* d_tok, float* d_mod_row, float* d_pos, int acc_mod, int acc_pos,
                     int B, int T, int L, int m, int H, int max_F,
                     void* workspace, int64_t workspace_bytes, mmfm_stream stream);
+int mmfm_stitch_fwd_live(int dtype, const void* tok, const float* mod_emb_row, const float* pos_emb,
+                         const int64_t* ts, const uint8_t* keep0, const int32_t* rec, void* x, void* emb,
+                         int B, int T, int L, int m, int H, int max_F, mmfm_stream stream);
+int mmfm_stitch_bwd_live(int dtype, const void* dx, const void* dextra, const int64_t* ts, const uint8_t* keep0, const int32_t* rec,
+                         mmfm_dropout drop, void* d_tok, float* d_mod_row, float* d_pos, int acc_mod, int acc_pos,
+                         int B, int T, int L, int m, int H, int max_F,
+                         void* workspace, int64_t workspace_bytes, mmfm_stream stream);
 
 int mmfm_collate_csr(int B, int max_T, int max_N, float pad_value, const uint8_t* data, const int32_t* indices,
                      const int64_t* indptr, const int64_t* indptr_off, const int64_t* nnz_off, const int32_t* T_b,
diff --git a/multi_modal_foundation_model_amd/_lib.py b/multi_modal_foundation_model_amd/_lib.py
--- a/multi_modal_foundation_model_amd/_lib.py
+++ b/multi_modal_foundation_model_amd/_lib.py
@@ -39,6 +39,14 @@
                 ("slab_stride", C.c_int64), ("bias", C.c_void_p), ("pre_out", C.c_void_p), ("act", C.c_int),
                 ("act_scale", C.c_float), ("gradmul_pre", C.c_void_p), ("drop", Dropout), ("residual", C.c_void_p),
                 ("ldr", C.c_int), ("colsum", C.c_void_p)]
+
+
+class LiveRows(C.Structure):
+    _fields_ = [("rec", C.c_void_p), ("B", C.c_int), ("T", C.c_int)]
+
+
+def live_rec_ints(T):
+    return 2 * T + 4
 
 
 class AttnDesc(C.Structure):
@@ -86,6 +94,9 @@
     "mmfm_rng_advance": (C.c_int, [_vp, _vp]),
     "mmfm_gemm": (C.c_int, [C.POINTER(GemmDesc), _vp]),
     "mmfm_gemm_pair": (C.c_int, [_vp, _vp, _vp]),
+    "mmfm_gemm_live": (C.c_int, [C.POINTER(GemmDesc), C.POINTER(LiveRows), _vp]),
+    "mmfm_live_bins": (C.c_int, [_vp, _i, _i, _vp, _vp]),
+    "mmfm_gather_live_rows": (C.c_int, [_vp, _vp, _i, _i, _i64, _vp, _vp]),
     "mmfm_gemm_dw_tiles": (C.c_int, [_i, _i, _i]),
     "mmfm_reduce_slabs": (C.c_int, [_vp, _vp, _i64, _i, _i64, _i, _vp]),
     "mmfm_reduce_slabs_multi": (C.c_int, [_vp, _i, _i, _vp]),
@@ -104,6 +115,8 @@
     "mmfm_mask_prep": (C.c_int, [_i, _i, _i, C.POINTER(_vp), C.POINTER(_i64), _vp, C.POINTER(_i64), _vp, _vp, _vp, _vp, _vp, _vp]),
     "mmfm_collate_csr": (C.c_int, [_i, _i, _i, _f, _vp, _vp, _vp, _vp, _vp, _vp, _vp, _vp, _vp, _vp, _vp]),
     "mmfm_stitch_fwd": (C.c_int, [_i, _vp, _vp, _vp, _vp, _vp, _vp, _vp, _i, _i, _i, _i, _i, _i, _vp]),
+    "mmfm_stitch_fwd_live": (C.c_int, [_i, _vp, _vp, _vp, _vp, _vp, _vp, _vp, _vp, _i, _i, _i, _i, _i, _i, _vp]),
+    "mmfm_stitch_bwd_live": (C.c_int, [_i, _vp, _vp, _vp, _vp, _vp, Dropout, _vp, _vp, _vp, _i, _i, _i, _i, _i, _i, _i, _i, _vp, _i64, _vp]),
     "mmfm_stitch_bwd_workspace": (C.c_int64, [_i, _i, _i, _i, _i, _i]),
     "mmfm_stitch_bwd": (C.c_int, [_i, _vp, _vp, _vp, _vp, Dropout, _vp, _vp, _vp, _i, _i, _i, _i, _i, _i, _i, _i, _vp, _i64, _vp]),
     "mmfm_masked_loss_workspace": (C.c_int64, [_i64, _i]),
diff --git a/multi_modal_foundation_model_amd/csrc/common.h b/multi_modal_foundation_model_amd/csrc/common.h
--- a/multi_modal_foundation_model_amd/csrc/common.h
+++ b/multi_modal_foundation_model_amd/csrc/common.h
@@ -29,6 +29,27 @@
 int mmfm_lds_opt_in(const void* kern, size_t bytes, const char* what);
 
 static inline int cdiv(long a, long b) { return (int)((a + b - 1) / b); }
+
+struct LiveArg {
+    const int32_t* rec;
+    int B, T, kdim;
+};
+static const LiveArg kNoLive = {nullptr, 0, 0, 0};
+__device__ __forceinline__ void live_patch(mmfm_gemm_desc& d, const LiveArg& lv) {
+    if (!lv.rec) return;
+    const int rows = lv.B * lv.rec[0];
+    if (!lv.kdim) {
+        d.M = rows;
+    } else if (rows != d.K) {
+        d.kchunk = d.splits > 1 ? ((rows + d.splits - 1) / d.splits + 63) / 64 * 64 : rows;
+        d.K = rows;
+    }
+}
+__device__ __forceinline__ int live_orig_row(const LiveArg& lv, int m) {
+    if (!lv.rec) return m;
+    const int tl = lv.rec[0], b = m / tl;
+    return b * lv.T + lv.rec[4 + m - b * tl];
+}
 
 __device__ __forceinline__ float bf2f(uint16_t v) { return __uint_as_float(((uint32_t)v) << 16); }
 __device__ __forceinline__ uint16_t f2bf(float f) {
diff --git a/multi_modal_foundation_model_amd/csrc/gemm.hip b/multi_modal_foundation_model_amd/csrc/gemm.hip
--- a/multi_modal_foundation_model_amd/csrc/gemm.hip
+++ b/multi_modal_foundation_model_amd/csrc/gemm.hip
@@ -294,7 +294,7 @@
 
 }
 
-int mmfm_gemm_bf16_launch(const mmfm_gemm_desc* d, hipStream_t st);
+int mmfm_gemm_bf16_launch(const mmfm_gemm_desc* d, hipStream_t st, const LiveArg& lv);
 
 static int gemm_check(const mmfm_gemm_desc* dp, mmfm_gemm_desc& d) {
     MMFM_REQUIRE(dp != nullptr, "mmfm_gemm: null descriptor");
@@ -333,7 +333,7 @@
     mmfm_gemm_desc d;
     if (int rc = gemm_check(dp, d)) return rc;
     hipStream_t st = (hipStream_t)stream;
-    if (d.dtype == MMFM_BF16) return mmfm_gemm_bf16_launch(&d, st);
+    if (d.dtype == MMFM_BF16) return mmfm_gemm_bf16_launch(&d, st, kNoLive);
 
     const int tiles = cdiv(d.M, BM) * cdiv(d.N, BN);
     const int vecA = (d.lda % 4 == 0) && ((uintptr_t)d.A % 16 == 0);
@@ -353,6 +353,17 @@
 #undef F32_LAUNCH
     MMFM_LAUNCH_CHECK("mmfm_gemm(f32)");
     return 0;
+}
+
+extern "C" int mmfm_gemm_live(const mmfm_gemm_desc* dp, const mmfm_live_rows* live, mmfm_stream stream) {
+    mmfm_gemm_desc d;
+    if (int rc = gemm_check(dp, d)) return rc;
+    MMFM_REQUIRE(d.dtype == MMFM_BF16, "mmfm_gemm_live: bf16 only (the fp32 parity path keeps the full row space)");
+    MMFM_REQUIRE(live && live->rec && live->B > 0 && live->T > 0, "mmfm_gemm_live: bad live-row record");
+    const LiveArg lv = {live->rec, live->B, live->T, d.a_kcontig ? 0 : 1};
+    MMFM_REQUIRE((int64_t)live->B * live->T == (lv.kdim ? d.K : d.M), "mmfm_gemm_live: B * T = %lld is not the descriptor's %s = %d",
+                 (long long)live->B * live->T, lv.kdim ? "K" : "M", lv.kdim ? d.K : d.M);
+    return mmfm_gemm_bf16_launch(&d, (hipStream_t)stream, lv);
 }
 
 extern "C" int mmfm_gemm_pair(const mmfm_gemm_desc* ap, const mmfm_gemm_desc* bp, mmfm_stream stream) {
diff --git a/multi_modal_foundation_model_amd/csrc/gemm_bf16.hip b/multi_modal_foundation_model_amd/csrc/gemm_bf16.hip
--- a/multi_modal_foundation_model_amd/csrc/gemm_bf16.hip
+++ b/multi_modal_foundation_model_amd/csrc/gemm_bf16.hip
@@ -92,7 +92,7 @@
 }
 
 template <typename TO, int AK = 0, int EF = 0>
-__device__ __forceinline__ void epilogue_store(const mmfm_gemm_desc& d, const Drop& dr, float v, int m, int n) {
+__device__ __forceinline__ void epilogue_store(const mmfm_gemm_desc& d, const LiveArg& lv, const Drop& dr, float v, int m, int n) {
     typedef io<uint16_t> I16;
     constexpr int AKM = AK == kActEmbed ? 0 : AK;
     if (d.bias) v += d.bias[n];
@@ -101,7 +101,7 @@
         if (!(d.act & 1)) v = embed_act1<true, EF>(v) * d.act_scale;
         else if (EF == 0) v *= d.act_scale;
         else v = embed_mul_grad1<true, EF>(v, I16::ld(reinterpret_cast<const uint16_t*>(d.gradmul_pre) + (size_t)m * d.ldc + n)) * d.act_scale;
-        v = dr.apply(v, (uint64_t)m * (uint64_t)d.N + (uint64_t)n);
+        if (dr.on()) v = dr.apply(v, (uint64_t)live_orig_row(lv, m) * (uint64_t)d.N + (uint64_t)n);
         if (d.residual) v += I16::ld(reinterpret_cast<const uint16_t*>(d.residual) + (size_t)m * d.ldr + n);
         io<TO>::st(reinterpret_cast<TO*>(d.C) + (size_t)m * d.ldc + n, v);
         return;
@@ -115,7 +115,7 @@
         else if (AK) v *= mlp_act_grad1<AKM>(u, d.act_scale);
         else v *= (d.act == 3) ? gelu_poly_grad(u) : (d.act == 4 ? softsign_grad(u) : softsign_grad_from_out(u, 1.f / d.act_scale)) * d.act_scale;
     }
-    v = dr.apply(v, (uint64_t)m * (uint64_t)d.N + (uint64_t)n);
+    if (dr.on()) v = dr.apply(v, (uint64_t)live_orig_row(lv, m) * (uint64_t)d.N + (uint64_t)n);
     if (d.residual) v += I16::ld(reinterpret_cast<const uint16_t*>(d.residual) + (size_t)m * d.ldr + n);
     io<TO>::st(reinterpret_cast<TO*>(d.C) + (size_t)m * d.ldc + n, v);
 }
@@ -159,7 +159,7 @@
 }
 
 template <typename TO, bool EPI_LOADS = true, int AK = 0, int EF = 0>
-__device__ __forceinline__ void epilogue_tile(const mmfm_gemm_desc& d, f32x16 (&acc)[2][2], char* smem, int m0, int n0, int z, int vec_epi,
+__device__ __forceinline__ void epilogue_tile(const mmfm_gemm_desc& d, const LiveArg& lv, f32x16 (&acc)[2][2], char* smem, int m0, int n0, int z, int vec_epi,
                                               int t, int wm, int wn, int kh, int l31) {
     const bool split = d.splits > 1;
     constexpr int AKM = AK == kActEmbed ? 0 : AK;
@@ -257,7 +257,7 @@
                     }
                 }
                 if (dr.on()) {
-                    const uint64_t base = (uint64_t)m * (uint64_t)d.N + (uint64_t)n;
+                    const uint64_t base = (uint64_t)live_orig_row(lv, m) * (uint64_t)d.N + (uint64_t)n;
 #pragma unroll
                     for (int e = 0; e < 8; e += 2) dr.apply2(v[e], v[e + 1], base + e);
                 }
@@ -293,13 +293,16 @@
             for (int r = 0; r < 16; ++r) {
                 const int m = m0 + wm * 64 + i * 32 + (r & 3) + 8 * (r >> 2) + 4 * kh;
                 const int n = n0 + wn * 64 + j * 32 + l31;
-                if (m < d.M && n < d.N) epilogue_store<TO, AK, EF>(d, dr, acc[i][j][r], m, n);
+                if (m < d.M && n < d.N) epilogue_store<TO, AK, EF>(d, lv, dr, acc[i][j][r], m, n);
             }
 }
 
 template <bool ARC, bool BRC, typename TO, int BK, bool PERSIST = (sizeof(TO) == 4), int AK = 0>
-__global__ __launch_bounds__(NTHREADS, BK == 64 ? 3 : 2) void gemm_bf16_kernel(const mmfm_gemm_desc d, const int alignA, const int alignB,
-                                                                              const int vec_epi, const int total_items) {
+__global__ __launch_bounds__(NTHREADS, BK == 64 ? 3 : 2) void gemm_bf16_kernel(const mmfm_gemm_desc d_full, const int alignA, const int alignB,
+                                                                              const int vec_epi, const int items_full, const LiveArg lv) {
+    mmfm_gemm_desc d = d_full;
+    live_patch(d, lv);
+    const int total_items = (lv.rec && !lv.kdim) ? ((d.M + BM - 1) / BM) * ((d.N + BN - 1) / BN) : items_full;
     constexpr int TILE_BYTES = Geo<BK>::TILE_BYTES;
     __shared__ __attribute__((aligned(16))) char smem[2 * TILE_BYTES];
     char* As = smem;
@@ -395,10 +398,10 @@
         }
         if constexpr (AK == kActEmbed)
             embed_dispatch(d.act, [&](auto F) {
-                epilogue_tile<TO, !(PERSIST && sizeof(TO) == 2), AK, decltype(F)::value>(d, acc, smem, m0, n0, z, vec_epi, t, wm, wn, kh, l31);
+                epilogue_tile<TO, !(PERSIST && sizeof(TO) == 2), AK, decltype(F)::value>(d, lv, acc, smem, m0, n0, z, vec_epi, t, wm, wn, kh, l31);
             });
         else
-            epilogue_tile<TO, !(PERSIST && sizeof(TO) == 2), AK>(d, acc, smem, m0, n0, z, vec_epi, t, wm, wn, kh, l31);
+            epilogue_tile<TO, !(PERSIST && sizeof(TO) == 2), AK>(d, lv, acc, smem, m0, n0, z, vec_epi, t, wm, wn, kh, l31);
         if (!more) break;
         w = wn_; m0 = m0n; n0 = n0n; z = zn; kbeg = kbegn; kend = kendn;
     }
@@ -412,15 +415,15 @@
 
 }
 
-int mmfm_gemm_big_launch(const mmfm_gemm_desc* dp, hipStream_t st);
-int mmfm_gemm_dw_launch(const mmfm_gemm_desc* dp, hipStream_t st);
-
-int mmfm_gemm_bf16_launch(const mmfm_gemm_desc* dp, hipStream_t st) {
+int mmfm_gemm_big_launch(const mmfm_gemm_desc* dp, hipStream_t st, const LiveArg& lv);
+int mmfm_gemm_dw_launch(const mmfm_gemm_desc* dp, hipStream_t st, const LiveArg& lv);
+
+int mmfm_gemm_bf16_launch(const mmfm_gemm_desc* dp, hipStream_t st, const LiveArg& lv) {
     const mmfm_gemm_desc d = *dp;
     {
-        const int rb = mmfm_gemm_big_launch(dp, st);
+        const int rb = mmfm_gemm_big_launch(dp, st, lv);
         if (rb != -1000) return rb;
-        const int rw = mmfm_gemm_dw_launch(dp, st);
+        const int rw = mmfm_gemm_dw_launch(dp, st, lv);
         if (rw != -1000) return rw;
     }
     MMFM_REQUIRE(d.splits == 1 || d.kchunk % 64 == 0, "mmfm_gemm(bf16): kchunk %d must be a multiple of 64", d.kchunk);
@@ -449,12 +452,12 @@
     dim3 grid((f32out || pb) ? std::min(total_items, 256 * wg_per_cu) : total_items), block(NTHREADS);
     static const int pad_lds = [] { const char* e = getenv("MMFM_GEMM_PAD_LDS"); return e ? atoi(e) : 0; }();
 #define LAUNCH2(ARC, BRC, BKV)                                                                                    \
-    if (f32out) hipLaunchKernelGGL((gemm_bf16_kernel<ARC, BRC, float, BKV>), grid, block, pad_lds, st, d, aA, aB, vecf, total_items);  \
-    else if (pb) hipLaunchKernelGGL((gemm_bf16_kernel<ARC, BRC, uint16_t, BKV, true>), grid, block, pad_lds, st, d, aA, aB, vecf, total_items); \
-    else hipLaunchKernelGGL((gemm_bf16_kernel<ARC, BRC, uint16_t, BKV>), grid, block, pad_lds, st, d, aA, aB, vecf, total_items);
+    if (f32out) hipLaunchKernelGGL((gemm_bf16_kernel<ARC, BRC, float, BKV>), grid, block, pad_lds, st, d, aA, aB, vecf, total_items, lv);  \
+    else if (pb) hipLaunchKernelGGL((gemm_bf16_kernel<ARC, BRC, uint16_t, BKV, true>), grid, block, pad_lds, st, d, aA, aB, vecf, total_items, lv); \
+    else hipLaunchKernelGGL((gemm_bf16_kernel<ARC, BRC, uint16_t, BKV>), grid, block, pad_lds, st, d, aA, aB, vecf, total_items, lv);
 #define LAUNCH_AK(ARC, BRC, AKV)                                                                                  \
-    if (f32out) hipLaunchKernelGGL((gemm_bf16_kernel<ARC, BRC, float, 64, true, AKV>), grid, block, pad_lds, st, d, aA, aB, vecf, total_items); \
-    else hipLaunchKernelGGL((gemm_bf16_kernel<ARC, BRC, uint16_t, 64, false, AKV>), grid, block, pad_lds, st, d, aA, aB, vecf, total_items);
+    if (f32out) hipLaunchKernelGGL((gemm_bf16_kernel<ARC, BRC, float, 64, true, AKV>), grid, block, pad_lds, st, d, aA, aB, vecf, total_items, lv); \
+    else hipLaunchKernelGGL((gemm_bf16_kernel<ARC, BRC, uint16_t, 64, false, AKV>), grid, block, pad_lds, st, d, aA, aB, vecf, total_items, lv);
 #define LAUNCH(ARC, BRC)                                                                                          \
     if (ak == MMFM_MLP_RELU) { LAUNCH_AK(ARC, BRC, MMFM_MLP_RELU) }                                                \
     else if (ak == MMFM_MLP_SIGMOID) { LAUNCH_AK(ARC, BRC, MMFM_MLP_SIGMOID) }                                     \
diff --git a/multi_modal_foundation_model_amd/csrc/gemm_big.hip b/multi_modal_foundation_model_amd/csrc/gemm_big.hip
--- a/multi_modal_foundation_model_amd/csrc/gemm_big.hip
+++ b/multi_modal_foundation_model_amd/csrc/gemm_big.hip
@@ -42,8 +42,11 @@
 #define LDS_WAIT(n) do { asm volatile("s_waitcnt lgkmcnt(" #n ")" ::: "memory"); __builtin_amdgcn_sched_barrier(0); } while (0)
 
 template <int AK = 0>
-__global__ __launch_bounds__(NT, 2) void gemm_big_kernel(const BigArgs a) {
+__global__ __launch_bounds__(NT, 2) void gemm_big_kernel(const BigArgs a_full, const LiveArg lv) {
     extern __shared__ __attribute__((aligned(16))) char smem[];
+    BigArgs a = a_full;
+    live_patch(a.d, lv);
+    if (lv.rec) a.ntiles = ((a.d.M + TB - 1) / TB) * a.tiles_n;
     const mmfm_gemm_desc& d = a.d;
     const int t = threadIdx.x, lane = t & 63, m = lane & 31, h = lane >> 5;
     const int wave = __builtin_amdgcn_readfirstlane(t >> 6);
@@ -233,12 +236,13 @@
                     }
                 }
                 if (dr.on()) {
+                    const int drow = row < (uint32_t)d.M ? live_orig_row(lv, (int)row) : (int)row;
 #pragma unroll
                     for (int e = 0; e < 2; ++e)
 #pragma unroll
                         for (int r = 0; r < 16; r += 2) {
                             float v0 = acc[2 * ip + e][j][r], v1 = acc[2 * ip + e][j][r + 1];
-                            dr.apply2(v0, v1, (uint64_t)row * (uint64_t)d.N + (uint64_t)(ncol0 + 32 * e + 8 * (r >> 2) + 4 * h + (r & 3)));
+                            dr.apply2(v0, v1, (uint64_t)drow * (uint64_t)d.N + (uint64_t)(ncol0 + 32 * e + 8 * (r >> 2) + 4 * h + (r & 3)));
                             acc[2 * ip + e][j][r] = v0; acc[2 * ip + e][j][r + 1] = v1;
                         }
                 }
@@ -264,11 +268,11 @@
 
 }
 
-int mmfm_gemm_big_launch(const mmfm_gemm_desc* dp, hipStream_t st) {
+int mmfm_gemm_big_launch(const mmfm_gemm_desc* dp, hipStream_t st, const LiveArg& lv) {
     const mmfm_gemm_desc& d = *dp;
     static const int on = [] { const char* e = getenv("MMFM_GEMM_BIG"); return e ? atoi(e) : 1; }();
     static const int kmin = [] { const char* e = getenv("MMFM_GEMM_BIG_KMIN"); return e ? atoi(e) : 512; }();
-    if (!on || d.dtype != MMFM_BF16 || d.c_f32 || d.splits > 1 || !d.a_kcontig || !d.b_kcontig || d.colsum) return -1000;
+    if (!on || d.dtype != MMFM_BF16 || d.c_f32 || d.splits > 1 || !d.a_kcontig || !d.b_kcontig || d.colsum || (lv.rec && lv.kdim)) return -1000;
     if (d.K % BK || d.K < kmin || d.N < 128 || d.M < 1024 || d.N % 8) return -1000;
     const char* mt = getenv("MMFM_GEMM_BIG_MIN_TILES");
     if (cdiv(d.M, TB) * cdiv(d.N, TB) < (mt ? atoi(mt) : 96)) return -1000;
@@ -292,11 +296,11 @@
     a.nk = d.K / BK;
     a.nt_c = nt_env & 1;
     a.nt_pre = (nt_env >> 1) & 1;
-    if (ak == MMFM_MLP_RELU) hipLaunchKernelGGL(gemm_big_kernel<MMFM_MLP_RELU>, dim3(std::min(a.ntiles, 256)), dim3(NT), LDS_ALL, st, a);
-    else if (ak == MMFM_MLP_SIGMOID) hipLaunchKernelGGL(gemm_big_kernel<MMFM_MLP_SIGMOID>, dim3(std::min(a.ntiles, 256)), dim3(NT), LDS_ALL, st, a);
-    else if (ak == MMFM_MLP_GELU_TANH) hipLaunchKernelGGL(gemm_big_kernel<MMFM_MLP_GELU_TANH>, dim3(std::min(a.ntiles, 256)), dim3(NT), LDS_ALL, st, a);
-    else if (ak == kActEmbed) hipLaunchKernelGGL(gemm_big_kernel<kActEmbed>, dim3(std::min(a.ntiles, 256)), dim3(NT), LDS_ALL, st, a);
-    else hipLaunchKernelGGL(gemm_big_kernel<0>, dim3(std::min(a.ntiles, 256)), dim3(NT), LDS_ALL, st, a);
+    if (ak == MMFM_MLP_RELU) hipLaunchKernelGGL(gemm_big_kernel<MMFM_MLP_RELU>, dim3(std::min(a.ntiles, 256)), dim3(NT), LDS_ALL, st, a, lv);
+    else if (ak == MMFM_MLP_SIGMOID) hipLaunchKernelGGL(gemm_big_kernel<MMFM_MLP_SIGMOID>, dim3(std::min(a.ntiles, 256)), dim3(NT), LDS_ALL, st, a, lv);
+    else if (ak == MMFM_MLP_GELU_TANH) hipLaunchKernelGGL(gemm_big_kernel<MMFM_MLP_GELU_TANH>, dim3(std::min(a.ntiles, 256)), dim3(NT), LDS_ALL, st, a, lv);
+    else if (ak == kActEmbed) hipLaunchKernelGGL(gemm_big_kernel<kActEmbed>, dim3(std::min(a.ntiles, 256)), dim3(NT), LDS_ALL, st, a, lv);
+    else hipLaunchKernelGGL(gemm_big_kernel<0>, dim3(std::min(a.ntiles, 256)), dim3(NT), LDS_ALL, st, a, lv);
     MMFM_LAUNCH_CHECK("mmfm_gemm(bf16, 256 tile)");
     return 0;
 }
diff --git a/multi_modal_foundation_model_amd/csrc/gemm_dw.hip b/multi_modal_foundation_model_amd/csrc/gemm_dw.hip
--- a/multi_modal_foundation_model_amd/csrc/gemm_dw.hip
+++ b/multi_modal_foundation_model_amd/csrc/gemm_dw.hip
@@ -51,7 +51,7 @@
 };
 
 template <int TN, int BK>
-__global__ __launch_bounds__(DNT) void gemm_dw_kernel(const DwPair pr) {
+__global__ __launch_bounds__(DNT) void gemm_dw_kernel(const DwPair pr, const LiveArg lv) {
     const bool second = pr.first > 0 && (int)blockIdx.x >= pr.first;
     const DwArgs& a = second ? pr.b : pr.a;
     const int w0 = second ? (int)blockIdx.x - pr.first : (int)blockIdx.x;
@@ -60,7 +60,8 @@
     constexpr int NLW = 4;
     constexpr int NST = G::NST, NJ = G::NJ, RBB = TN * 2;
     extern __shared__ __attribute__((aligned(16))) char smem[];
-    const mmfm_gemm_desc& d = a.d;
+    mmfm_gemm_desc d = a.d;
+    live_patch(d, lv);
     const int t = threadIdx.x, lane = t & 63;
     const int wave = __builtin_amdgcn_readfirstlane(t >> 6);
     const int wm = wave >> 1, wn = wave & 1;
@@ -213,7 +214,7 @@
 }
 
 template <int TN, int BK>
-int launch(const mmfm_gemm_desc& d, const mmfm_gemm_desc* d2, hipStream_t st) {
+int launch(const mmfm_gemm_desc& d, const mmfm_gemm_desc* d2, hipStream_t st, const LiveArg& lv) {
     typedef Geo<TN, BK> G;
     if (int rc = mmfm_lds_opt_in(reinterpret_cast<const void*>(gemm_dw_kernel<TN, BK>), G::LDS, "mmfm_gemm(bf16, dW stream)")) return rc;
     DwPair p;
@@ -226,7 +227,7 @@
         p.first = p.a.items;
         grid = p.a.items + p.b.items;
     }
-    hipLaunchKernelGGL((gemm_dw_kernel<TN, BK>), dim3(grid), dim3(DNT), G::LDS, st, p);
+    hipLaunchKernelGGL((gemm_dw_kernel<TN, BK>), dim3(grid), dim3(DNT), G::LDS, st, p, lv);
     MMFM_LAUNCH_CHECK("mmfm_gemm(bf16, dW stream)");
     return 0;
 }
@@ -252,10 +253,10 @@
     return true;
 }
 
-int mmfm_gemm_dw_launch(const mmfm_gemm_desc* dp, hipStream_t st) {
+int mmfm_gemm_dw_launch(const mmfm_gemm_desc* dp, hipStream_t st, const LiveArg& lv) {
     const mmfm_gemm_desc& d = *dp;
-    if (!dw_eligible(d)) return -1000;
-    return dw_wide(d.N, d.K) ? launch<256, 32>(d, nullptr, st) : launch<128, 32>(d, nullptr, st);
+    if (!dw_eligible(d) || (lv.rec && !lv.kdim)) return -1000;
+    return dw_wide(d.N, d.K) ? launch<256, 32>(d, nullptr, st, lv) : launch<128, 32>(d, nullptr, st, lv);
 }
 
 int mmfm_gemm_dw_pair_launch(const mmfm_gemm_desc* ap, const mmfm_gemm_desc* bp, hipStream_t st) {
@@ -265,5 +266,5 @@
     if (wide != dw_wide(b.N, b.K)) return -1000;
     const int ia = mmfm_gemm_dw_tiles(a.M, a.N, a.K) * std::max(1, a.splits), ib = mmfm_gemm_dw_tiles(b.M, b.N, b.K) * std::max(1, b.splits);
     if (ia % 8 || ia + ib > 512) return -1000;
-    return wide ? launch<256, 32>(a, &b, st) : launch<128, 32>(a, &b, st);
-}
+    return wide ? launch<256, 32>(a, &b, st, kNoLive) : launch<128, 32>(a, &b, st, kNoLive);
+}
diff --git a/multi_modal_foundation_model_amd/csrc/stitch.hip b/multi_modal_foundation_model_amd/csrc/stitch.hip
--- a/multi_modal_foundation_model_amd/csrc/stitch.hip
+++ b/multi_modal_foundation_model_amd/csrc/stitch.hip
@@ -48,8 +48,8 @@
 template <typename T>
 __global__ __launch_bounds__(256) void stitch_fwd_kernel(const T* __restrict__ tok, const float* __restrict__ mod_row,
                                                          const float* __restrict__ pos, const int64_t* __restrict__ ts,
-                                                         const uint8_t* __restrict__ keep0, T* __restrict__ x, T* __restrict__ emb,
-                                                         int B, int Tn, int L, int m, int H, int max_F) {
+                                                         const uint8_t* __restrict__ keep0, const int32_t* __restrict__ rec, T* __restrict__ x,
+                                                         T* __restrict__ emb, int B, int Tn, int L, int m, int H, int max_F) {
     const int C4 = H / 4;
     const int64_t total = (int64_t)B * Tn * C4;
     for (int64_t idx = (int64_t)blockIdx.x * blockDim.x + threadIdx.x; idx < total; idx += (int64_t)gridDim.x * blockDim.x) {
@@ -67,7 +67,8 @@
         const size_t o = ((size_t)b * L + l) * H + c;
         if (emb) io<T>::st4(emb + o, e);
         if (keep0[l]) {
-            const float4 tv = io<T>::ld4(tok + (size_t)r * H + c);
+            const int64_t tr = rec ? (int64_t)b * rec[0] + rec[4 + Tn + t] : r;
+            const float4 tv = io<T>::ld4(tok + (size_t)tr * H + c);
             e.x += tv.x; e.y += tv.y; e.z += tv.z; e.w += tv.w;
         }
         io<T>::st4(x + o, e);
@@ -76,8 +77,8 @@
 
 template <typename T, bool POS>
 __global__ void stitch_bwd_kernel(const T* __restrict__ dx, const T* __restrict__ dextra, const int64_t* __restrict__ ts,
-                                  const uint8_t* __restrict__ keep0, mmfm_dropout dropa, T* __restrict__ d_tok,
-                                  float* __restrict__ part, int B, int Tn, int L, int m, int H, int max_F, int bper) {
+                                  const uint8_t* __restrict__ keep0, const int32_t* __restrict__ rec, mmfm_dropout dropa,
+                                  T* __restrict__ d_tok, float* __restrict__ part, int B, int Tn, int L, int m, int H, int max_F, int bper) {
     extern __shared__ __attribute__((aligned(16))) float tab[];
     const int CW = blockDim.x, j = threadIdx.x, col = blockIdx.x * CW + j;
     const Drop dr = drop_init(dropa);
@@ -97,7 +98,9 @@
                 tab[tsv * CW + j] += e;
             }
             macc += e;
-            if (d_tok) io<T>::st(d_tok + (size_t)r * H + col, keep0[l] ? dr.apply(g, (uint64_t)r * H + col) : 0.f);
+            if (d_tok && !rec) io<T>::st(d_tok + (size_t)r * H + col, keep0[l] ? dr.apply(g, (uint64_t)r * H + col) : 0.f);
+            else if (d_tok && keep0[l])
+                io<T>::st(d_tok + ((size_t)b * rec[0] + rec[4 + Tn + t]) * H + col, dr.apply(g, (uint64_t)r * H + col));
         }
     }
     float* out = part + (size_t)blockIdx.y * (max_F + 1) * H;
@@ -154,7 +157,8 @@
     }
 }
 
-__global__ __launch_bounds__(256) void stitch_dtok_kernel(const uint16_t* __restrict__ dx, const uint8_t* __restrict__ keep0, mmfm_dropout dropa,
+__global__ __launch_bounds__(256) void stitch_dtok_kernel(const uint16_t* __restrict__ dx, const uint8_t* __restrict__ keep0,
+                                                          const int32_t* __restrict__ rec, mmfm_dropout dropa,
                                                           uint16_t* __restrict__ d_tok, int B, int Tn, int L, int m, int H) {
     const Drop dr = drop_init(dropa);
     const int C8 = H / 8;
@@ -164,6 +168,8 @@
         const int c = (int)(idx % C8) * 8;
         const int b = (int)(r / Tn), l = m * Tn + (int)(r % Tn);
         uint4 o = make_uint4(0u, 0u, 0u, 0u);
+        if (rec && !keep0[l]) continue;
+        const int64_t orow = rec ? (int64_t)b * rec[0] + rec[4 + Tn + (int)(r % Tn)] : r;
         if (keep0[l]) {
             const uint4 g = *reinterpret_cast<const uint4*>(dx + ((size_t)b * L + l) * H + c);
             if (dr.on()) {
@@ -180,7 +186,7 @@
                 o = g;
             }
         }
-        *reinterpret_cast<uint4*>(d_tok + (size_t)r * H + c) = o;
+        *reinterpret_cast<uint4*>(d_tok + (size_t)orow * H + c) = o;
     }
 }
 
@@ -242,7 +248,7 @@
 }
 
 extern "C" int mmfm_reduce_slabs(float*, const float*, int64_t, int, int64_t, int, mmfm_stream);
-int mmfm_gemm_bf16_launch(const mmfm_gemm_desc* dp, hipStream_t st);
+int mmfm_gemm_bf16_launch(const mmfm_gemm_desc* dp, hipStream_t st, const LiveArg& lv);
 
 extern "C" int mmfm_mask_prep(int B, int T, int M, const int64_t* const* mask_src, const int64_t* mask_stride,
                               const int64_t* attn, const int64_t* channels, uint8_t* tokmask, uint8_t* keypad,
@@ -280,21 +286,32 @@
     return 0;
 }
 
-extern "C" int mmfm_stitch_fwd(int dtype, const void* tok, const float* mod_emb_row, const float* pos_emb, const int64_t* ts,
-                               const uint8_t* keep0, void* x, void* emb, int B, int T, int L, int m, int H, int max_F, mmfm_stream stream) {
+static int stitch_fwd_impl(int dtype, const void* tok, const float* mod_emb_row, const float* pos_emb, const int64_t* ts,
+                           const uint8_t* keep0, const int32_t* rec, void* x, void* emb, int B, int T, int L, int m, int H, int max_F,
+                           mmfm_stream stream) {
     MMFM_REQUIRE(tok && mod_emb_row && (ts || !pos_emb) && keep0 && x, "mmfm_stitch_fwd: null pointer");
     MMFM_REQUIRE(B > 0 && T > 0 && H > 0 && H % 4 == 0 && m >= 0 && (m + 1) * T <= L && max_F > 0, "mmfm_stitch_fwd: bad shape");
     const int64_t n = (int64_t)B * T * (H / 4);
     dim3 grid((int)std::min<int64_t>(4096, (n + 255) / 256)), block(256);
     hipStream_t st = (hipStream_t)stream;
     if (dtype == MMFM_F32)
-        hipLaunchKernelGGL(stitch_fwd_kernel<float>, grid, block, 0, st, (const float*)tok, mod_emb_row, pos_emb, ts, keep0, (float*)x, (float*)emb, B, T, L, m, H, max_F);
+        hipLaunchKernelGGL(stitch_fwd_kernel<float>, grid, block, 0, st, (const float*)tok, mod_emb_row, pos_emb, ts, keep0, rec, (float*)x, (float*)emb, B, T, L, m, H, max_F);
     else if (dtype == MMFM_BF16)
-        hipLaunchKernelGGL(stitch_fwd_kernel<uint16_t>, grid, block, 0, st, (const uint16_t*)tok, mod_emb_row, pos_emb, ts, keep0, (uint16_t*)x, (uint16_t*)emb, B, T, L, m, H, max_F);
+        hipLaunchKernelGGL(stitch_fwd_kernel<uint16_t>, grid, block, 0, st, (const uint16_t*)tok, mod_emb_row, pos_emb, ts, keep0, rec, (uint16_t*)x, (uint16_t*)emb, B, T, L, m, H, max_F);
     else
         return mmfm_set_error(-1, "mmfm_stitch_fwd: bad dtype %d", dtype);
     MMFM_LAUNCH_CHECK("mmfm_stitch_fwd");
     return 0;
+}
+extern "C" int mmfm_stitch_fwd(int dtype, const void* tok, const float* mod_emb_row, const float* pos_emb, const int64_t* ts,
+                               const uint8_t* keep0, void* x, void* emb, int B, int T, int L, int m, int H, int max_F, mmfm_stream stream) {
+    return stitch_fwd_impl(dtype, tok, mod_emb_row, pos_emb, ts, keep0, nullptr, x, emb, B, T, L, m, H, max_F, stream);
+}
+extern "C" int mmfm_stitch_fwd_live(int dtype, const void* tok, const float* mod_emb_row, const float* pos_emb, const int64_t* ts,
+                                    const uint8_t* keep0, const int32_t* rec, void* x, void* emb, int B, int T, int L, int m, int H, int max_F,
+                                    mmfm_stream stream) {
+    MMFM_REQUIRE(rec, "mmfm_stitch_fwd_live: null live-bin record");
+    return stitch_fwd_impl(dtype, tok, mod_emb_row, pos_emb, ts, keep0, rec, x, emb, B, T, L, m, H, max_F, stream);
 }
 
 extern "C" int64_t mmfm_stitch_bwd_workspace(int dtype, int B, int T, int L, int H, int max_F) {
@@ -308,9 +325,9 @@
     return (int64_t)stitch_chunks(B, H, cw) * (max_F + 1) * H * sizeof(float);
 }
 
-extern "C" int mmfm_stitch_bwd(int dtype, const void* dx, const void* dextra, const int64_t* ts, const uint8_t* keep0,
-                               mmfm_dropout drop, void* d_tok, float* d_mod_row, float* d_pos, int acc_mod, int acc_pos, int B, int T,
-                               int L, int m, int H, int max_F, void* workspace, int64_t workspace_bytes, mmfm_stream stream) {
+static int stitch_bwd_impl(int dtype, const void* dx, const void* dextra, const int64_t* ts, const uint8_t* keep0, const int32_t* rec,
+                           mmfm_dropout drop, void* d_tok, float* d_mod_row, float* d_pos, int acc_mod, int acc_pos, int B, int T,
+                           int L, int m, int H, int max_F, void* workspace, int64_t workspace_bytes, mmfm_stream stream) {
     MMFM_REQUIRE(dx && (ts || !d_pos) && keep0 && d_mod_row, "mmfm_stitch_bwd: null pointer");
     MMFM_REQUIRE(B > 0 && T > 0 && H > 0 && max_F > 0 && m >= 0 && (m + 1) * T <= L, "mmfm_stitch_bwd: bad shape");
     if (oh_path(dtype, H)) {
@@ -326,7 +343,7 @@
             if (d_tok) {
                 const int64_t n = (int64_t)B * T * (H / 8);
                 hipLaunchKernelGGL(stitch_dtok_kernel, dim3((int)std::min<int64_t>(4096, (n + 255) / 256)), dim3(256), 0, st, (const uint16_t*)dx, keep0,
-                                   drop, (uint16_t*)d_tok, B, T, L, m, H);
+                                   rec, drop, (uint16_t*)d_tok, B, T, L, m, H);
             }
             hipLaunchKernelGGL(stitch_modsum_kernel, dim3(cdiv(H, 256), nsl), dim3(256), 0, st, (const uint16_t*)dx, (const uint16_t*)dextra,
                                (float*)workspace, B, T, L, m, H, bper);
@@ -340,7 +357,7 @@
         if (d_tok) {
             const int64_t n = (int64_t)B * T * (H / 8);
             hipLaunchKernelGGL(stitch_dtok_kernel, dim3((int)std::min<int64_t>(4096, (n + 255) / 256)), dim3(256), 0, st, (const uint16_t*)dx, keep0,
-                               drop, (uint16_t*)d_tok, B, T, L, m, H);
+                               rec, drop, (uint16_t*)d_tok, B, T, L, m, H);
         }
         MMFM_LAUNCH_CHECK("mmfm_stitch_bwd(one-hot)");
         mmfm_gemm_desc gd = {};
@@ -355,7 +372,7 @@
             if (!src) continue;
             gd.B = src;
             gd.C = slabs + (int64_t)nsl * g.slab;
-            if (int rc = mmfm_gemm_bf16_launch(&gd, st)) return rc;
+            if (int rc = mmfm_gemm_bf16_launch(&gd, st, kNoLive)) return rc;
             nsl += g.S;
         }
         if (int rc = mmfm_reduce_slabs(d_pos, slabs, (int64_t)max_F * H, nsl, g.slab, acc_pos, stream)) return rc;
@@ -372,22 +389,88 @@
     MMFM_REQUIRE(dtype == MMFM_F32 || dtype == MMFM_BF16, "mmfm_stitch_bwd: bad dtype %d", dtype);
     if (!d_pos) {
         if (dtype == MMFM_F32)
-            hipLaunchKernelGGL((stitch_bwd_kernel<float, false>), grid, block, 0, st, (const float*)dx, (const float*)dextra, ts, keep0, drop,
+            hipLaunchKernelGGL((stitch_bwd_kernel<float, false>), grid, block, 0, st, (const float*)dx, (const float*)dextra, ts, keep0, rec, drop,
                                (float*)d_tok, (float*)workspace, B, T, L, m, H, 0, bper);
         else
-            hipLaunchKernelGGL((stitch_bwd_kernel<uint16_t, false>), grid, block, 0, st, (const uint16_t*)dx, (const uint16_t*)dextra, ts, keep0, drop,
+            hipLaunchKernelGGL((stitch_bwd_kernel<uint16_t, false>), grid, block, 0, st, (const uint16_t*)dx, (const uint16_t*)dextra, ts, keep0, rec, drop,
                                (uint16_t*)d_tok, (float*)workspace, B, T, L, m, H, 0, bper);
         MMFM_LAUNCH_CHECK("mmfm_stitch_bwd(no table)");
         return mmfm_reduce_slabs(d_mod_row, (const float*)workspace, H, nch, H, acc_mod, stream);
     }
     if (dtype == MMFM_F32)
-        hipLaunchKernelGGL((stitch_bwd_kernel<float, true>), grid, block, lds, st, (const float*)dx, (const float*)dextra, ts, keep0, drop, (float*)d_tok,
+        hipLaunchKernelGGL((stitch_bwd_kernel<float, true>), grid, block, lds, st, (const float*)dx, (const float*)dextra, ts, keep0, rec, drop, (float*)d_tok,
                            (float*)workspace, B, T, L, m, H, max_F, bper);
     else
-        hipLaunchKernelGGL((stitch_bwd_kernel<uint16_t, true>), grid, block, lds, st, (const uint16_t*)dx, (const uint16_t*)dextra, ts, keep0, drop,
+        hipLaunchKernelGGL((stitch_bwd_kernel<uint16_t, true>), grid, block, lds, st, (const uint16_t*)dx, (const uint16_t*)dextra, ts, keep0, rec, drop,
                            (uint16_t*)d_tok, (float*)workspace, B, T, L, m, H, max_F, bper);
     MMFM_LAUNCH_CHECK("mmfm_stitch_bwd");
     const int64_t stride = (int64_t)(max_F + 1) * H;
     if (int rc = mmfm_reduce_slabs(d_pos, (const float*)workspace, (int64_t)max_F * H, nch, stride, acc_pos, stream)) return rc;
     return mmfm_reduce_slabs(d_mod_row, (const float*)workspace + (size_t)max_F * H, H, nch, stride, acc_mod, stream);
 }
+
+extern "C" int mmfm_stitch_bwd(int dtype, const void* dx, const void* dextra, const int64_t* ts, const uint8_t* keep0,
+                               mmfm_dropout drop, void* d_tok, float* d_mod_row, float* d_pos, int acc_mod, int acc_pos, int B, int T,
+                               int L, int m, int H, int max_F, void* workspace, int64_t workspace_bytes, mmfm_stream stream) {
+    return stitch_bwd_impl(dtype, dx, dextra, ts, keep0, nullptr, drop, d_tok, d_mod_row, d_pos, acc_mod, acc_pos, B, T, L, m, H, max_F,
+                           workspace, workspace_bytes, stream);
+}
+extern "C" int mmfm_stitch_bwd_live(int dtype, const void* dx, const void* dextra, const int64_t* ts, const uint8_t* keep0, const int32_t* rec,
+                                    mmfm_dropout drop, void* d_tok, float* d_mod_row, float* d_pos, int acc_mod, int acc_pos, int B, int T,
+                                    int L, int m, int H, int max_F, void* workspace, int64_t workspace_bytes, mmfm_stream stream) {
+    MMFM_REQUIRE(rec, "mmfm_stitch_bwd_live: null live-bin record");
+    return stitch_bwd_impl(dtype, dx, dextra, ts, keep0, rec, drop, d_tok, d_mod_row, d_pos, acc_mod, acc_pos, B, T, L, m, H, max_F,
+                           workspace, workspace_bytes, stream);
+}
+
+namespace {
+__global__ __launch_bounds__(64) void live_bins_kernel(const uint8_t* __restrict__ keep0, int T, int32_t* __restrict__ rec_all) {
+    const uint8_t* k = keep0 + (size_t)blockIdx.x * T;
+    int32_t* rec = rec_all + (size_t)blockIdx.x * MMFM_LIVE_REC_INTS(T);
+    const int lane = threadIdx.x;
+    int base = 0;
+    for (int t0 = 0; t0 < T; t0 += 64) {
+        const int t = t0 + lane;
+        const bool live = t < T && k[t] != 0;
+        const unsigned long long mask = __ballot(live);
+        const int r = base + __popcll(mask & ((1ull << lane) - 1ull));
+        if (t < T) rec[4 + T + t] = live ? r : -1;
+        if (live) rec[4 + r] = t;
+        base += __popcll(mask);
+    }
+    if (lane < 4) rec[lane] = lane == 0 ? base : 0;
+}
+
+template <typename V>
+__global__ __launch_bounds__(256) void gather_live_kernel(const V* __restrict__ src, V* __restrict__ dst, int B, int T, int cpr,
+                                                          const int32_t* __restrict__ rec) {
+    const int tl = rec[0];
+    const int64_t total = (int64_t)B * tl * cpr;
+    for (int64_t idx = (int64_t)blockIdx.x * blockDim.x + threadIdx.x; idx < total; idx += (int64_t)gridDim.x * blockDim.x) {
+        const int64_t row = idx / cpr;
+        const int c = (int)(idx - row * cpr), b = (int)(row / tl), j = (int)(row - (int64_t)b * tl);
+        dst[idx] = src[((int64_t)b * T + rec[4 + j]) * cpr + c];
+    }
+}
+}
+
+extern "C" int mmfm_live_bins(const uint8_t* keep0, int T, int M, int32_t* rec, mmfm_stream stream) {
+    MMFM_REQUIRE(keep0 && rec && T > 0 && M > 0, "mmfm_live_bins: bad arguments");
+    hipLaunchKernelGGL(live_bins_kernel, dim3(M), dim3(64), 0, (hipStream_t)stream, keep0, T, rec);
+    MMFM_LAUNCH_CHECK("mmfm_live_bins");
+    return 0;
+}
+
+extern "C" int mmfm_gather_live_rows(const void* src, void* dst, int B, int T, int64_t row_bytes, const int32_t* rec, mmfm_stream stream) {
+    MMFM_REQUIRE(src && dst && rec && B > 0 && T > 0 && row_bytes > 0 && row_bytes % 4 == 0 && row_bytes < ((int64_t)1 << 30),
+                 "mmfm_gather_live_rows: bad arguments (rows of a multiple of 4 bytes)");
+    const bool v16 = row_bytes % 16 == 0 && (uintptr_t)src % 16 == 0 && (uintptr_t)dst % 16 == 0;
+    const int cpr = (int)(row_bytes / (v16 ? 16 : 4));
+    const int64_t n = (int64_t)B * T * cpr;
+    dim3 grid((int)std::min<int64_t>(4096, (n + 255) / 256)), block(256);
+    hipStream_t st = (hipStream_t)stream;
+    if (v16) hipLaunchKernelGGL(gather_live_kernel<uint4>, grid, block, 0, st, (const uint4*)src, (uint4*)dst, B, T, cpr, rec);
+    else hipLaunchKernelGGL(gather_live_kernel<uint32_t>, grid, block, 0, st, (const uint32_t*)src, (uint32_t*)dst, B, T, cpr, rec);
+    MMFM_LAUNCH_CHECK("mmfm_gather_live_rows");
+    return 0;
+}
diff --git a/multi_modal_foundation_model_amd/ops.py b/multi_modal_foundation_model_amd/ops.py
--- a/multi_modal_foundation_model_amd/ops.py
+++ b/multi_modal_foundation_model_amd/ops.py
@@ -66,6 +66,26 @@
     _emit(plan, L.lib().mmfm_gemm, (C.byref(d),), keep=(d,))
 
 
+def live_rows(rec, B, T):
+    lv = L.LiveRows()
+    lv.rec, lv.B, lv.T = P(rec), B, T
+    lv._keep = rec
+    return lv
+
+
+def gemm_live(A, B, Cout, M, N, K, *, live, plan=None, **kw):
+    d = gemm_desc(A, B, Cout, M, N, K, **kw)
+    _emit(plan, L.lib().mmfm_gemm_live, (C.byref(d), C.byref(live)), keep=(d, live))
+
+
+def live_bins(keep0, T, M, rec, plan=None):
+    _emit(plan, L.lib().mmfm_live_bins, (P(keep0), T, M, P(rec)))
+
+
+def gather_live_rows(src, dst, B, T, row_bytes, rec, plan=None):
+    _emit(plan, L.lib().mmfm_gather_live_rows, (P(src), P(dst), B, T, row_bytes, P(rec)))
+
+
 def gemm_pair(da, db, plan=None):
     _emit(plan, L.lib().mmfm_gemm_pair, (C.byref(da), C.byref(db)), keep=(da, db))
 
@@ -151,6 +171,16 @@
 
 def stitch_fwd(tok, mod_row, pos, ts, keep0, x, emb, B, T, Lseq, m, H, max_F, plan=None):
     _emit(plan, L.lib().mmfm_stitch_fwd, (dt(tok), P(tok), P(mod_row), P(pos), P(ts), P(keep0), P(x), P(emb), B, T, Lseq, m, H, max_F))
+
+
+def stitch_fwd_live(tok, mod_row, pos, ts, keep0, rec, x, emb, B, T, Lseq, m, H, max_F, plan=None):
+    _emit(plan, L.lib().mmfm_stitch_fwd_live, (dt(tok), P(tok), P(mod_row), P(pos), P(ts), P(keep0), P(rec), P(x), P(emb), B, T, Lseq, m, H, max_F))
+
+
+def stitch_bwd_live(dx, dextra, ts, keep0, rec, drop, d_tok, d_mod_row, d_pos, acc_mod, acc_pos, B, T, Lseq, m, H, max_F, ws, plan=None):
+    _emit(plan, L.lib().mmfm_stitch_bwd_live, (dt(dx), P(dx), P(dextra), P(ts), P(keep0), P(rec), drop if drop is not None else L.NO_DROP,
+                                               P(d_tok), P(d_mod_row), P(d_pos), int(acc_mod), int(acc_pos), B, T, Lseq, m, H, max_F, P(ws),
+                                               ws.numel() * ws.element_size()))
 
 
 def stitch_bwd(dx, dextra, ts, keep0, drop, d_tok, d_mod_row, d_pos, acc_mod, acc_pos, B, T, Lseq, m, H, max_F, ws, plan=None):
diff --git a/multi_modal_foundation_model_amd/plan.py b/multi_modal_foundation_model_amd/plan.py
--- a/multi_modal_foundation_model_amd/plan.py
+++ b/multi_modal_foundation_model_amd/plan.py
@@ -23,6 +23,14 @@
     return Switches(fused=int(env["MMFM_FUSED"]) if "MMFM_FUSED" in env else None, gemm_big=on("MMFM_GEMM_BIG"), gemm_dw=on("MMFM_GEMM_DW"),
                     batch_reduce=on("MMFM_BATCH_REDUCE"), dw_pair=on("MMFM_DW_PAIR"), attn_keepbits=on("MMFM_ATTN_KEEPBITS"),
                     mlp_bwd_split=env.get("MMFM_MLP_BWD_SPLIT", "1") == "1")
+
+
+LIVE_ROWS_MIN = 16384
+
+
+def live_rows_on(BT):
+    v = os.environ.get("MMFM_LIVE_ROWS")
+    return v == "1" if v in ("0", "1") else BT >= max(8192, LIVE_ROWS_MIN)
 
 
 class Side:
@@ -51,6 +59,8 @@
         self.sides = {side: Side(c.side(side), training) for side in ("encoder", "decoder")}
         self.Imax, self.mult_max = max(sd.I for sd in self.sides.values()), max(sd.mult for sd in self.sides.values())
         self.code, self.es, self.buf, self.b = e.code, 4 if e.dtype == "fp32" else 2, e._buf, e.b
+        self.live = self.code == L.BF16 and live_rows_on(self.BT) and self.live_bias_ok()
+        self.lv = {}
         self.enc_flags = L.ATTN_DIAG
         self.dec_flags = (L.ATTN_CAUSAL if c.causal_mask else 0) | (L.ATTN_SEP if c.sep_mask else 0)
         self.fwd, self.bwd, self.cur = [], [], []
@@ -67,6 +77,19 @@
         if sd.emb_fwd == L.ACT_SOFTSIGN and self.code == L.BF16:
             return "a"
         return "z"
+
+    def live_bias_ok(self):
+        if not self.grad:
+            return True
+        e = self.e
+        for side, mods in self.mods_of.items():
+            for _, mod, _ in mods:
+                for lin in ("token_embed", "projection"):
+                    w = f"{side}_embeddings.{mod}.embedder.{lin}"
+                    gw, gb = e.Gv(w + ".weight"), e.Gb(w)
+                    if gb is not None and gb.data_ptr() != gw.data_ptr() + 4 * gw.numel():
+                        return False
+        return True
 
     def mk(self, side, name):
         return "dec/" + name if self.split_masks and side == "decoder" else name
@@ -141,10 +164,11 @@
             raise RuntimeError(f"engine: ws/slabm holds {self.slabm.numel()} floats, the plan's slab regions need {self.slabm_off}")
         return self.slabm[o:o + S * stride]
 
-    def lin(self, plan, X, wname, Y, Mr, N, Kd, ldx=None, **kw):
-        K.gemm(X, self.e.W(wname + ".weight"), Y, Mr, N, Kd, lda=ldx or Kd, ldb=Kd, ldc=N, bias=self.e.Pb(wname), dtype=self.code, plan=plan, **kw)
-
-    def wgrad(self, plan, dY, X, dst, N, Kd, Mr, nb, S, kchunk, what, ldx=None, colsum=None, slab=None, paired=False):
+    def lin(self, plan, X, wname, Y, Mr, N, Kd, ldx=None, live=None, **kw):
+        gemm = K.gemm if live is None else functools.partial(K.gemm_live, live=live)
+        gemm(X, self.e.W(wname + ".weight"), Y, Mr, N, Kd, lda=ldx or Kd, ldb=Kd, ldc=N, bias=self.e.Pb(wname), dtype=self.code, plan=plan, **kw)
+
+    def wgrad(self, plan, dY, X, dst, N, Kd, Mr, nb, S, kchunk, what, ldx=None, colsum=None, slab=None, paired=False, live=None):
         n = N * Kd + nb
         if S == 1 and not paired:
             out, cs, split, red = dst, colsum if colsum is not None else (dst.data_ptr() + 4 * N * Kd if nb else None), {}, None
@@ -155,7 +179,7 @@
                 raise RuntimeError(f"engine: {what}: {S} slabs x {stride} floats exceed the {out.numel()}-float slab workspace")
             cs = out.data_ptr() + 4 * N * Kd if nb else None
             split, red = dict(splits=S, kchunk=kchunk, slab_stride=stride), (dst, out, n, S, stride)
-        emit = K.gemm_desc if paired else functools.partial(K.gemm, plan=plan)
+        emit = K.gemm_desc if paired else functools.partial(K.gemm, plan=plan) if live is None else functools.partial(K.gemm_live, live=live, plan=plan)
         d = emit(dY, X, out, N, Kd, Mr, lda=N, ldb=ldx or Kd, ldc=Kd, a_kcontig=0, b_kcontig=0, dtype=self.code, c_f32=1, colsum=cs, **split)
         if paired:
             return d, red
@@ -186,7 +210,7 @@
             a = self.deferred.pop()
             self.dlin(plan, a["dY"], a["X"], a["wname"], a["Mr"], a["N"], a["Kd"])
 
-    def dlin(self, plan, dY, X, wname, Mr, N, Kd, dX=None, ldx=None, defer=False, **kw):
+    def dlin(self, plan, dY, X, wname, Mr, N, Kd, dX=None, ldx=None, defer=False, live=None, **kw):
         e, code = self.e, self.code
         S, kchunk = e._dw_split(N, Kd, Mr, ldn=ldx, sw=self.sw)
         gw, gb = e.Gv(wname + ".weight"), e.Gb(wname)
@@ -196,16 +220,19 @@
             self.flush_deferred(plan)
             self.deferred.append(dict(dY=dY, X=X, wname=wname, Mr=Mr, N=N, Kd=Kd, nb=N if gb is not None else 0))
             return
-        self.wgrad(plan, dY, X, gw, N, Kd, Mr, N if adjacent and S > 1 else 0, S, kchunk, wname, ldx=ldx, colsum=gb if fused else None, slab=self.slab)
+        self.wgrad(plan, dY, X, gw, N, Kd, Mr, N if adjacent and S > 1 else 0, S, kchunk, wname, ldx=ldx, colsum=gb if fused else None, slab=self.slab,
+                   live=live)
         if gb is not None and (not fused or (S > 1 and not adjacent)):
+            assert live is None, wname
             K.colsum(dY, Mr, N, N, gb, self.b["ws/col"], plan=plan)
         if dX is not None:
+            gemm = K.gemm if live is None else functools.partial(K.gemm_live, live=live)
             wT = e._w_transposed(wname, N, Kd, Mr, sw=self.sw) if code == L.BF16 else None
             if wT is not None:
                 self.used_wt.append(wname)
-                K.gemm(dY, wT, dX, Mr, Kd, N, lda=N, ldb=N, ldc=Kd, b_kcontig=1, dtype=code, plan=plan, **kw)
+                gemm(dY, wT, dX, Mr, Kd, N, lda=N, ldb=N, ldc=Kd, b_kcontig=1, dtype=code, plan=plan, **kw)
             else:
-                K.gemm(dY, e.W(wname + ".weight"), dX, Mr, Kd, N, lda=N, ldb=Kd, ldc=Kd, b_kcontig=0, dtype=code, plan=plan, **kw)
+                gemm(dY, e.W(wname + ".weight"), dX, Mr, Kd, N, lda=N, ldb=Kd, ldc=Kd, b_kcontig=0, dtype=code, plan=plan, **kw)
 
     def lin_norm_grad(self, plan, Gdb, wname, lnname, N):
         e, H, ws = self.e, self.H, self.b["ws/lng"]
@@ -336,6 +363,10 @@
         for side in ("encoder", "decoder") if self.split_masks else ("encoder",):
             K.mask_prep(B, T, [b[f"mask/{m}"] for m, _, _ in self.mods_of[side]], [1] * M, b["attn"], [n for _, _, n in self.mods_of[side]],
                         b[mk(side, "tokmask")], b[mk(side, "keypad")], b[mk(side, "keep0")], b[mk(side, "mod_id")], b[mk(side, "count")], plan=fwd)
+            if self.live:
+                rec = buf(mk(side, "live"), (M, L.live_rec_ints(T)), torch.int32)
+                K.live_bins(b[mk(side, "keep0")], T, M, rec, plan=fwd)
+        gathered = set()
         tok_tmp = buf("tok_tmp", (BT, H))
         x_enc, emb_enc, x_dec = buf("x_enc", (R, H)), buf("emb_enc", (R, H)), buf("x_dec", (R, H))
         for side, xs, es_ in (("encoder", x_enc, emb_enc), ("decoder", x_dec, None)):
@@ -345,11 +376,22 @@
                 n2 = n * sd.mult
                 a = buf(f"{side}/a/{m}", (BT, n2))
                 z = buf(f"{side}/z/{m}", (BT, n2)) if self.embed_saved(sd) == "z" else None
-                self.lin(fwd, b[f"in/{m}"], p + ".token_embed", a, BT, n2, n, ldx=_align(n, 8), pre_out=z, act=sd.emb_fwd, act_scale=sd.scale)
-                self.lin(fwd, a, p + ".projection", tok_tmp, BT, H, n2, drop=e._drop(f"{side}/embdrop/{m}", sd.dpe))
+                xin, lv = b[f"in/{m}"], None
+                if self.live:
+                    rec = b[mk(side, "live")][slot]
+                    lv = self.lv[side, slot] = K.live_rows(rec, B, T)
+                    xin = buf(mk(side, f"in_live/{m}"), (BT, _align(n, 8)))
+                    if mk(side, f"in_live/{m}") not in gathered:
+                        gathered.add(mk(side, f"in_live/{m}"))
+                        K.gather_live_rows(b[f"in/{m}"], xin, B, T, _align(n, 8) * self.es, rec, plan=fwd)
+                self.lin(fwd, xin, p + ".token_embed", a, BT, n2, n, ldx=_align(n, 8), pre_out=z, act=sd.emb_fwd, act_scale=sd.scale, live=lv)
+                self.lin(fwd, a, p + ".projection", tok_tmp, BT, H, n2, drop=e._drop(f"{side}/embdrop/{m}", sd.dpe), live=lv)
                 mod_row = e.Pf(f"{c.mod_emb_owner(side, mod)}_embeddings.{mod}.embedder.mod_emb.weight")[m]
                 pos = e.Pf(p + ".pos_embed.weight") if sd.pos else None
-                K.stitch_fwd(tok_tmp, mod_row, pos, b["ts"], b[mk(side, "keep0")], xs, es_, B, T, Lq, slot, H, sd.max_F, plan=fwd)
+                if lv is not None:
+                    K.stitch_fwd_live(tok_tmp, mod_row, pos, b["ts"], b[mk(side, "keep0")], lv._keep, xs, es_, B, T, Lq, slot, H, sd.max_F, plan=fwd)
+                else:
+                    K.stitch_fwd(tok_tmp, mod_row, pos, b["ts"], b[mk(side, "keep0")], xs, es_, B, T, Lq, slot, H, sd.max_F, plan=fwd)
         X = x_enc
         for i in range(c.n_enc):
             p, tag = f"encoder.{i}", f"enc{i}"
@@ -498,21 +540,26 @@
             sd = self.sides[side]
             for slot, (m, mod, n) in enumerate(self.mods_of[side]):
                 pS = f"{side}_embeddings.{mod}.embedder"
-                K.stitch_bwd(dS, dextra, b["ts"], b[self.mk(side, "keep0")], e._drop(f"{side}/embdrop/{m}", sd.dpe), buf(f"d/tok/{side}/{m}", (BT, H)),
-                             e.Gv(f"{c.mod_emb_owner(side, mod)}_embeddings.{mod}.embedder.mod_emb.weight")[m],
-                             e.Gv(pS + ".pos_embed.weight") if sd.pos else None,
-                             side == "encoder" and mod in shared, False, B, T, Lq, slot, H, sd.max_F, b["ws/stitch"], plan=self.cur)
+                lv = self.lv.get((side, slot))
+                stitch = K.stitch_bwd if lv is None else functools.partial(K.stitch_bwd_live, rec=lv._keep)
+                stitch(dS, dextra, b["ts"], b[self.mk(side, "keep0")], drop=e._drop(f"{side}/embdrop/{m}", sd.dpe), d_tok=buf(f"d/tok/{side}/{m}", (BT, H)),
+                       d_mod_row=e.Gv(f"{c.mod_emb_owner(side, mod)}_embeddings.{mod}.embedder.mod_emb.weight")[m],
+                       d_pos=e.Gv(pS + ".pos_embed.weight") if sd.pos else None,
+                       acc_mod=side == "encoder" and mod in shared, acc_pos=False, B=B, T=T, Lseq=Lq, m=slot, H=H, max_F=sd.max_F, ws=b["ws/stitch"],
+                       plan=self.cur)
         for side in ("decoder", "encoder"):
             sd = self.sides[side]
             saved = self.embed_saved(sd)
-            for m, mod, n in self.mods_of[side]:
+            for slot, (m, mod, n) in enumerate(self.mods_of[side]):
                 p = f"{side}_embeddings.{mod}.embedder"
                 n2 = n * sd.mult
+                lv = self.lv.get((side, slot))
                 dz = self.rows(buf(f"d/z/{m}", (BT, n * self.mult_max)), BT, n2)
                 self.dlin(self.cur, b[f"d/tok/{side}/{m}"], b[f"{side}/a/{m}"], p + ".projection", BT, H, n2, dX=dz,
                           act=L.ACT_SOFTSIGN_GRAD_OUT if saved == "a" else sd.emb_grad, act_scale=sd.scale,
-                          gradmul_pre=b[f"{side}/{saved}/{m}"] if saved else None)
-                self.dlin(self.cur, dz, b[f"in/{m}"], p + ".token_embed", BT, n2, n, ldx=_align(n, 8))
+                          gradmul_pre=b[f"{side}/{saved}/{m}"] if saved else None, live=lv)
+                self.dlin(self.cur, dz, b[f"in/{m}"] if lv is None else b[self.mk(side, f"in_live/{m}")], p + ".token_embed", BT, n2, n,
+                          ldx=_align(n, 8), live=lv)
         self.close_segment("embed")
         if self.used_wt:
             tw = e._wt_table()
```
